# EvolBioInf/andi

Measured on AMD Instinct MI355X. Metric: genome-pairs/sec (ordered pairs, n^2-n) over the N x N anchor-distance loop, higher is better.
Workload: dtype u8

## Files before the change

andi_amd/csrc/api.hip:

```cpp
#include <hip/hip_runtime.h>

#include <algorithm>
#include <atomic>
#include <chrono>
#include <cstdarg>
#include <cstdio>
#include <cstdlib>
#include <cstring>
#include <mutex>
#include <string>
#include <thread>
#include <sys/mman.h>
#include <vector>

#include "api_internal.h"
#include "andi_dev.h"
#include "andi_hip.h"
#include "bootstrap.h"
#include "dev_arena.h"
#include "esa_build.h"
#include "knobs.h"
#include "sa_device.h"
#include "scan.h"

// ... 196 lines not shown
	if (hipMalloc(&p, bytes) != hipSuccess) {
		(void)hipGetLastError();
		return nullptr;
	}
	return p;
}
void scratch_put(int device, void *p, size_t bytes) {
	if (!p) return;
	{
		std::lock_guard<std::mutex> lk(state().mu);
		auto &v = state().scratch;
		bool have = false;
		for (const IdleScratch &x : v) have = have || x.device == device;
		if (!have) {
			v.push_back({device, p, bytes});
			return;
		}
	}
	(void)hipFree(p);
}
static bool any() {
	std::lock_guard<std::mutex> lk(state().mu);
	return !state().streams.empty() || !state().pinned.empty() || !state().scratch.empty() || !state().slabs.empty();
}
static size_t trim() {
	std::vector<IdleStream> st;
	std::vector<IdlePinned> pb;
	std::vector<IdleScratch> sc;
	{
		std::lock_guard<std::mutex> lk(state().mu);
		st.swap(state().streams), pb.swap(state().pinned), sc.swap(state().scratch);
		if (state().words_out == 0) {
			for (char *slab : state().slabs) pb.push_back({slab, SLAB_BYTES});
			state().slabs.clear(), state().free_words.clear();
		}
	}
	for (const IdleStream &x : st)
		if (hipSetDevice(x.device) == hipSuccess) (void)hipStreamDestroy(x.s);
	for (const IdlePinned &b : pb) (void)hipHostFree(b.p);
	size_t freed = 0;
	for (const IdleScratch &x : sc)
		if (hipSetDevice(x.device) == hipSuccess && hipFree(x.p) == hipSuccess) freed += x.bytes;
	return freed;
}
}

int andi_hip_abi_version(void) {
	return ANDI_HIP_ABI_VERSION;
}

size_t andi_hip_trim(void) {
	if (!andi_arena::any_chunks() && !host_pool::any()) return 0;
	int ndev = 0, cur = 0;
	if (hipGetDeviceCount(&ndev) != hipSuccess) {
		(void)hipGetLastError();
		return 0;
	}
	(void)hipGetDevice(&cur);
	size_t freed = 0;
	for (int d = 0; d < ndev && d < 64; ++d) {
		if (!andi_arena::has_chunks(d)) continue;
		if (hipSetDevice(d) != hipSuccess) continue;
		freed += andi_arena::trim(d);
	}
	freed += host_pool::trim();
	(void)hipSetDevice(cur);
	return freed;
}

void andi_hip_default_opts(andi_hip_opts *o) {
	if (!o) return;
	memset(o, 0, sizeof *o);
	o->p_value = 0.025;
	o->model = ANDI_M_JC;
	o->device = 0;
	o->host_threads = 0;
	o->low_memory = 0;
	o->segment = 0;
	o->sa_on_host = 0;
	o->num_gpus = 1;
	o->devices = NULL;
}

int andi_hip_device_count(void) {
	int count = 0;
	return hipGetDeviceCount(&count) == hipSuccess && count > 0 ? count : 0;
}

int ctx_create(andi_hip_ctx **out, int device, char *errbuf, size_t errlen, bool high_priority) {
	if (!out) return 1;
	*out = nullptr;
	int count = 0;
	hipError_t e = hipGetDeviceCount(&count);
	if (e != hipSuccess || count <= 0) {
		set_err(errbuf, errlen, "no HIP device available (%s); the anchor-distance engine has no CPU path",
				e != hipSuccess ? hipGetErrorString(e) : "device count 0");
		return 1;
	}
	if (device < 0 || device >= count) {
		set_err(errbuf, errlen, "HIP device %d out of range (have %d)", device, count);
		return 1;
	}
	e = hipSetDevice(device);
	if (e != hipSuccess) {
		set_err(errbuf, errlen, "hipSetDevice(%d): %s", device, hipGetErrorString(e));
		return 1;
	}
	auto *ctx = new andi_hip_ctx;
	ctx->device = device;
	andi_arena::retain(device);
	int prio = 0;
	if (high_priority) {
		int least = 0, greatest = 0;
		if (hipDeviceGetStreamPriorityRange(&least, &greatest) == hipSuccess) prio = greatest;
	}
	ctx->stream_prio = prio;
	e = host_pool::stream_get(&ctx->stream, device, prio);
	if (e == hipSuccess) e = hipEventCreateWithFlags(&ctx->side_fork, hipEventDisableTiming);
	if (e == hipSuccess) e = hipEventCreateWithFlags(&ctx->side_join, hipEventDisableTiming);
	if (e == hipSuccess) e = hipEventCreateWithFlags(&ctx->desc_done, hipEventDisableTiming);
	if (e == hipSuccess) e = hipEventCreateWithFlags(&ctx->built, hipEventDisableTiming);
	if (e == hipSuccess) e = hipMalloc((void **)&ctx->d_fixups, sizeof(unsigned long long));
	if (e == hipSuccess) e = hipMemset(ctx->d_fixups, 0, sizeof(unsigned long long));
	if (e == hipSuccess && !(ctx->h_quad_waves = (uint32_t *)host_pool::word_get())) e = hipErrorOutOfMemory;
	if (e == hipSuccess) e = hipEventCreateWithFlags(&ctx->coop_fork, hipEventDisableTiming);
	if (e == hipSuccess) e = hipEventCreateWithFlags(&ctx->coop_join, hipEventDisableTiming);
	if (e == hipSuccess) e = hipEventCreateWithFlags(&ctx->l2_fork, hipEventDisableTiming);
	if (e == hipSuccess) e = hipEventCreateWithFlags(&ctx->l2_join, hipEventDisableTiming);
	if (e == hipSuccess && !(ctx->h_any_left = (uint32_t *)host_pool::word_get())) e = hipErrorOutOfMemory;
	if (e == hipSuccess) e = hipMalloc((void **)&ctx->d_route, 4 * sizeof(unsigned long long));
	if (e == hipSuccess) e = hipMemset(ctx->d_route, 0, 4 * sizeof(unsigned long long));
	if (e != hipSuccess) {
		set_err(errbuf, errlen, "context setup: %s", hipGetErrorString(e));
		andi_hip_ctx_destroy(ctx);
		return 1;
	}
	*out = ctx;
	return 0;
}

int andi_hip_ctx_create(andi_hip_ctx **out, int device, char *errbuf, size_t errlen) {
	return ctx_create(out, device, errbuf, errlen, false);
}

void andi_hip_ctx_expect_queries(andi_hip_ctx *ctx, size_t queries) {
	if (ctx) ctx->queries_hint = queries;
}

void andi_hip_ctx_destroy(andi_hip_ctx *ctx) {
	if (!ctx) return;
	(void)hipSetDevice(ctx->device);
	if (ctx->stream) (void)hipStreamSynchronize(ctx->stream);
	resolve_events(ctx);
	if (ctx->scratch) (void)andi_arena::dev_free(ctx->scratch);
	if (ctx->desc_dev) (void)andi_arena::dev_free(ctx->desc_dev);
	if (ctx->desc_host) host_pool::pinned_put(ctx->desc_host, ctx->desc_bytes);
	if (ctx->d_fixups) (void)andi_arena::dev_free(ctx->d_fixups);
	if (ctx->ib_dev) (void)andi_arena::dev_free(ctx->ib_dev);
	if (ctx->ib_host) host_pool::pinned_put(ctx->ib_host, ctx->ib_cap * sizeof(AndiIndexBatchItem));
	if (ctx->ib_done) (void)hipEventDestroy(ctx->ib_done);
	if (ctx->built) (void)hipEventDestroy(ctx->built);
	if (ctx->sa_ws) (void)andi_arena::dev_free(ctx->sa_ws);
	host_pool::word_put(ctx->sa_pinned);
	host_pool::word_put(ctx->h_quad_waves);
	if (ctx->d_route) (void)andi_arena::dev_free(ctx->d_route);
	if (ctx->scratch2) (void)andi_arena::dev_free(ctx->scratch2);
	if (ctx->pool_scratch) {
		(void)hipDeviceSynchronize();
		host_pool::scratch_put(ctx->device, ctx->pool_scratch, ctx->pool_bytes + 4096);
	}
	host_pool::word_put(ctx->h_any_left);
	if (ctx->coop_stream) {
		(void)hipStreamSynchronize(ctx->coop_stream);
		host_pool::stream_put(ctx->coop_stream, ctx->device, 0);
	}
	if (ctx->coop_fork) (void)hipEventDestroy(ctx->coop_fork);
	if (ctx->coop_join) (void)hipEventDestroy(ctx->coop_join);
	if (ctx->l2_fork) (void)hipEventDestroy(ctx->l2_fork);
	if (ctx->l2_join) (void)hipEventDestroy(ctx->l2_join);
	if (ctx->desc_done) (void)hipEventDestroy(ctx->desc_done);
	if (ctx->side_stream) {
		(void)hipStreamSynchronize(ctx->side_stream);
		host_pool::stream_put(ctx->side_stream, ctx->device, ctx->stream_prio);
	}
	if (ctx->side_fork) (void)hipEventDestroy(ctx->side_fork);
	if (ctx->side_join) (void)hipEventDestroy(ctx->side_join);
	if (ctx->stream) {
		(void)hipStreamSynchronize(ctx->stream);
		host_pool::stream_put(ctx->stream, ctx->device, ctx->stream_prio);
	}
	andi_arena::release(ctx->device);
	delete ctx;
}

const char *andi_hip_last_error(const andi_hip_ctx *ctx) {
	return ctx ? ctx->err.c_str() : "no context";
}

int andi_hip_sync(andi_hip_ctx *ctx) {
	if (!ctx) return 1;
	HIP_TRY(ctx, hipStreamSynchronize(ctx->stream));
	return 0;
}

int andi_hip_dev_alloc(andi_hip_ctx *ctx, size_t bytes, void **dptr) {
	if (!ctx || !dptr) return 1;
	HIP_TRY(ctx, hipSetDevice(ctx->device));
	HIP_TRY(ctx, hipMalloc(dptr, bytes ? bytes : 1));
	return 0;
}

void andi_hip_dev_free(andi_hip_ctx *ctx, void *dptr) {
	if (!ctx || !dptr) return;
	(void)hipSetDevice(ctx->device);
	(void)andi_arena::dev_free(dptr);
}

int andi_hip_copy_to_host(andi_hip_ctx *ctx, void *dst, const void *src, size_t bytes) {
	if (!ctx) return 1;
	HIP_TRY(ctx, hipMemcpyAsync(dst, src, bytes, hipMemcpyDeviceToHost, ctx->stream));
	HIP_TRY(ctx, hipStreamSynchronize(ctx->stream));
	return 0;
}

int esa_reserve(andi_hip_ctx *ctx, size_t cap, andi_hip_esa **out) {
	auto *e = new andi_hip_esa;
	e->cap = cap;
	hipError_t err = hipSuccess;
	auto chk = [&](hipError_t x) {
		if (err == hipSuccess) err = x;
	};
	e->deepK_cap = pick_deep_k(cap, ctx->queries_hint);
	const size_t deep_entries = (size_t)1 << (2 * e->deepK_cap);
	chk(dmalloc(&e->S, cap + 1 + ANDI_PAD));
	chk(dmalloc(&e->SA, cap + 8));
	chk(dmalloc(&e->deep, deep_entries + 2));
	const size_t nib_part = (cap / 2 + 1 + ANDI_NIB_BACK + 255) & ~(size_t)255;
	chk(dmalloc(&e->Nraw, 2 * (ANDI_NIB_FRONT + nib_part)));
	if (err == hipSuccess) {
		e->N0 = e->Nraw + ANDI_NIB_FRONT, e->N1 = e->Nraw + ANDI_NIB_FRONT + nib_part + ANDI_NIB_FRONT;
		chk(hipMemsetAsync(e->Nraw, 0x77, 2 * (ANDI_NIB_FRONT + nib_part), ctx->stream));
	}
	{
		const size_t blocks = (cap + 1 + 4096) / 32 + 4;
		chk(dmalloc(&e->Praw, 3 * blocks));
		if (err == hipSuccess) {
			e->P = e->Praw + 3;
			chk(hipMemsetAsync(e->Praw, 0xff, 3 * blocks * sizeof(uint32_t), ctx->stream));
		}
	}
	if (!(e->h_flags = (int32_t *)host_pool::word_get())) chk(hipErrorOutOfMemory);
	if (err == hipSuccess) chk(hipHostGetDevicePointer((void **)&e->flags, e->h_flags, 0));
	e->bytes = (cap + 1 + ANDI_PAD) + 4 * cap + 8 * deep_entries + 80 +
			   2 * (ANDI_NIB_FRONT + nib_part);
	if (err != hipSuccess) {
		andi_hip_esa_free(ctx, e);
		return fail(ctx, "allocating a subject", err);
	}
	*out = e;
	return 0;
}

int esa_upload(andi_hip_ctx *ctx, andi_hip_esa *e, const char *RS, const int32_t *SA, size_t n,
					  size_t threshold, hipEvent_t done) {
	if (n > e->cap) {
		ctx->err = "subject does not fit its slot";
		return 1;
	}
	e->n = (int32_t)n;
	e->thr = (int32_t)threshold;
	e->deepK = std::min(pick_deep_k(n, ctx->queries_hint), e->deepK_cap);
	e->ref_built = e->index_built = false;
	e->rec_valid = false;
	hipError_t err = done ? hipSuccess : hipStreamSynchronize(ctx->stream);
	memset(e->h_flags, 0, 4 * sizeof(int32_t));
	if (err == hipSuccess) err = hipMemsetAsync(e->S + n, 0, 1 + ANDI_PAD, ctx->stream);
	if (err == hipSuccess) err = hipMemcpyAsync(e->S, RS, n, hipMemcpyHostToDevice, ctx->stream);
	if (err == hipSuccess && SA)
		err = hipMemcpyAsync(e->SA, SA, n * sizeof(int32_t), hipMemcpyHostToDevice, ctx->stream);
	if (err == hipSuccess) err = done ? hipEventRecord(done, ctx->stream) : hipStreamSynchronize(ctx->stream);
	if (err != hipSuccess) return fail(ctx, "uploading a subject", err);
	return 0;
}

int esa_from_query(andi_hip_ctx *ctx, andi_hip_esa *e, const andi_hip_queries *Q, size_t i, size_t threshold) {
	const size_t len = Q->len[i], n = 2 * len + 1;
	if (n > e->cap) {
		ctx->err = "subject does not fit its slot";
		return 1;
	}
	e->n = (int32_t)n;
	e->thr = (int32_t)threshold;
	e->deepK = std::min(pick_deep_k(n, ctx->queries_hint), e->deepK_cap);
	e->ref_built = e->index_built = false;
	e->rec_valid = false;
	memset(e->h_flags, 0, 4 * sizeof(int32_t));
	hipError_t err = hipMemsetAsync(e->S + (n & ~(size_t)3), 0, (n & 3) + 1 + ANDI_PAD, ctx->stream);
	if (err == hipSuccess) err = andi_launch_rs_from_query(e->S, Q->pool + Q->off[i], (uint32_t)len, ctx->stream);
	if (err != hipSuccess) return fail(ctx, "writing a subject from its resident sequence", err);
	return 0;
}

int queries_gc_counts(andi_hip_ctx *ctx, const andi_hip_queries *Q, std::vector<unsigned long long> &out) {
	HIP_TRY(ctx, hipSetDevice(ctx->device));
	unsigned long long *d = nullptr;
	HIP_TRY(ctx, dmalloc(&d, Q->nq));
// ... 92 lines not shown
	const size_t tab_entries = (size_t)1 << (2 * ANDI_CACHE_K);
	const size_t mins = andi_min_tree_entries((int32_t)n);
	hipError_t err = hipSuccess;
	auto chk = [&](hipError_t x) {
		if (err == hipSuccess) err = x;
	};
	chk(dmalloc(&e->LCP, n + 1));
	chk(dmalloc(&e->CLD, n + 1));
	chk(dmalloc(&e->FVC, n + ANDI_PAD));
	chk(dmalloc(&e->tab, tab_entries));
	chk(dmalloc(&e->min_scratch, mins));
	if (err != hipSuccess) return fail(ctx, "allocating the reference arrays", err);
	e->bytes += 8 * (n + 1) + n + ANDI_PAD + 16 * tab_entries + 4 * mins;
	return 0;
}

int andi_hip_esa_build(andi_hip_ctx *ctx, andi_hip_esa *e) {
	if (!ctx || !e) return 1;
	HIP_TRY(ctx, hipSetDevice(ctx->device));
	if (ensure_reference_buffers(ctx, e)) return 1;
	Timed t(ctx, 0);
	hipError_t err = andi_launch_esa_build(build_args(e), ctx->stream);
	t.stop();
	if (err == hipSuccess) err = hipEventRecord(ctx->built, ctx->stream);
	if (err != hipSuccess) return fail(ctx, "andi_hip_esa_build", err);
	e->ref_built = true, ctx->builds_pending = true;
	return 0;
}

int andi_hip_esa_build_index(andi_hip_ctx *ctx, andi_hip_esa *e) {
	if (!ctx || !e) return 1;
	HIP_TRY(ctx, hipSetDevice(ctx->device));
	Timed t(ctx, 0);
	const int ext = andi_index_single_ext(ctx->queries_hint, e->rec_valid);
	hipError_t err = andi_launch_index_build(build_args(e), ext, ctx->stream);
	t.stop();
	if (err == hipSuccess) err = hipEventRecord(ctx->built, ctx->stream);
	if (err != hipSuccess) return fail(ctx, "andi_hip_esa_build_index", err);
	e->index_built = true, e->deep_ext = (ext == 2 && !e->rec_valid) ? 0 : ext, ctx->builds_pending = true;
	return 0;
}

int andi_hip_esa_build_index_batch(andi_hip_ctx *ctx, andi_hip_esa *const *esas, size_t count) {
	if (!ctx || !esas || count == 0 || count > 65535) {
		if (ctx) ctx->err = "andi_hip_esa_build_index_batch: bad arguments";
		return 1;
	}
	HIP_TRY(ctx, hipSetDevice(ctx->device));
	if (ctx->ib_cap < count) {
		HIP_TRY(ctx, hipStreamSynchronize(ctx->stream));
		if (ctx->ib_dev) (void)andi_arena::dev_free(ctx->ib_dev);
		if (ctx->ib_host) host_pool::pinned_put(ctx->ib_host, ctx->ib_cap * sizeof(AndiIndexBatchItem));
		ctx->ib_dev = ctx->ib_host = nullptr, ctx->ib_cap = 0;
		const size_t cap = std::max<size_t>(count, 64);
		HIP_TRY(ctx, andi_arena::dev_malloc(&ctx->ib_dev, cap * sizeof(AndiIndexBatchItem)));
		HIP_TRY(ctx, host_pool::pinned_get(&ctx->ib_host, cap * sizeof(AndiIndexBatchItem)));
		if (!ctx->ib_done) HIP_TRY(ctx, hipEventCreateWithFlags(&ctx->ib_done, hipEventDisableTiming));
		ctx->ib_cap = cap;
	} else {
		HIP_TRY(ctx, hipEventSynchronize(ctx->ib_done));
	}
	auto *items = (AndiIndexBatchItem *)ctx->ib_host;
	int32_t max_n = 0, max_n_shallow = 0;
	for (size_t k = 0; k < count; ++k) {
		andi_hip_esa *e = esas[k];
		if (!e) {
			ctx->err = "andi_hip_esa_build_index_batch: null subject";
			return 1;
		}
		items[k].S = e->S, items[k].SA = e->SA, items[k].deep = e->deep, items[k].N0 = e->N0, items[k].N1 = e->N1, items[k].P = e->P;
		items[k].flags = e->flags, items[k].n = e->n, items[k].deepK = e->deepK;
		items[k].rec = e->rec_valid ? e->rec : nullptr;
		items[k].rec2 = e->rec_valid ? e->rec2 : nullptr;
		items[k].single_ext = andi_index_single_ext(ctx->queries_hint, e->rec_valid);
		max_n = std::max(max_n, e->n);
		if (e->deepK < ANDI_CLOSED_RUN_K) max_n_shallow = std::max(max_n_shallow, e->n);
	}
	Timed t(ctx, 0);
	hipError_t err = hipMemcpyAsync(ctx->ib_dev, ctx->ib_host, count * sizeof(AndiIndexBatchItem), hipMemcpyHostToDevice, ctx->stream);
	if (err == hipSuccess) err = hipEventRecord(ctx->ib_done, ctx->stream);
	if (err == hipSuccess) err = andi_launch_index_build_batch((const AndiIndexBatchItem *)ctx->ib_dev, (uint32_t)count, max_n, max_n_shallow, ctx->stream);
	t.stop();
	if (err == hipSuccess) err = hipEventRecord(ctx->built, ctx->stream);
	if (err != hipSuccess) return fail(ctx, "andi_hip_esa_build_index_batch", err);
	for (size_t k = 0; k < count; ++k) {
		const int ext = items[k].single_ext;
		esas[k]->index_built = true, esas[k]->deep_ext = (ext == 2 && !esas[k]->rec_valid) ? 0 : ext;
	}
	ctx->builds_pending = true;
	return 0;
}

int andi_hip_esa_flags(andi_hip_ctx *ctx, const andi_hip_esa *e, int32_t *out4) {
	if (!ctx || !e || !out4) return 1;
	HIP_TRY(ctx, hipStreamSynchronize(ctx->stream));
	memcpy(out4, e->h_flags, 4 * sizeof(int32_t));
	return 0;
}

int andi_hip_esa_download(andi_hip_ctx *ctx, const andi_hip_esa *e, int32_t *LCP, int32_t *CLD,
						  uint8_t *FVC, andi_hip_interval *cache) {
	if (!ctx || !e) return 1;
	if (!e->ref_built) {
		ctx->err = "andi_hip_esa_download: reference arrays not built (call andi_hip_esa_build)";
		return 1;
	}
	const size_t n = (size_t)e->n;
	HIP_TRY(ctx, hipStreamSynchronize(ctx->stream));
	if (LCP) HIP_TRY(ctx, hipMemcpy(LCP, e->LCP, (n + 1) * 4, hipMemcpyDeviceToHost));
	if (CLD) HIP_TRY(ctx, hipMemcpy(CLD, e->CLD, (n + 1) * 4, hipMemcpyDeviceToHost));
	if (FVC) HIP_TRY(ctx, hipMemcpy(FVC, e->FVC, n, hipMemcpyDeviceToHost));
	if (cache)
		HIP_TRY(ctx, hipMemcpy(cache, e->tab, ((size_t)16 << (2 * ANDI_CACHE_K)), hipMemcpyDeviceToHost));
	return 0;
}

int andi_hip_esa_download_index(andi_hip_ctx *ctx, const andi_hip_esa *e, uint32_t *table, int *K) {
	if (!ctx || !e) return 1;
	if (!e->index_built) {
		ctx->err = "andi_hip_esa_download_index: scan index not built (call andi_hip_esa_build_index)";
		return 1;
	}
	if (K) *K = e->deepK;
	HIP_TRY(ctx, hipStreamSynchronize(ctx->stream));
	if (table) HIP_TRY(ctx, hipMemcpy(table, e->deep, (size_t)8 << (2 * e->deepK), hipMemcpyDeviceToHost));
	return 0;
}

#ifdef ANDI_TEST_HOOKS
extern "C" int andi_hip_test_download_text(andi_hip_ctx *ctx, const andi_hip_esa *e, uint8_t *N0, uint8_t *N1, size_t nib_bytes, uint32_t *P,
										   size_t p_words) {
	if (!ctx || !e) return 1;
	if (nib_bytes > e->cap / 2 + 1 + ANDI_NIB_BACK || p_words > 3 * ((e->cap + 1 + 4096) / 32 + 4)) {
		ctx->err = "andi_hip_test_download_text: more than the buffers hold";
		return 1;
	}
	HIP_TRY(ctx, hipStreamSynchronize(ctx->stream));
	if (N0) HIP_TRY(ctx, hipMemcpy(N0, e->N0, nib_bytes, hipMemcpyDeviceToHost));
	if (N1) HIP_TRY(ctx, hipMemcpy(N1, e->N1, nib_bytes, hipMemcpyDeviceToHost));
	if (P) HIP_TRY(ctx, hipMemcpy(P, e->Praw, p_words * sizeof(uint32_t), hipMemcpyDeviceToHost));
	return 0;
}
extern "C" int andi_hip_test_coop_items(andi_hip_ctx *ctx, uint32_t *items, size_t items_cap, uint8_t *pair_class, uint8_t *pair_cost, size_t pairs_cap,
										uint32_t *info) {
	if (!ctx) return 1;
	const auto &l = ctx->last_items;
	HIP_TRY(ctx, hipSetDevice(ctx->device));
	HIP_TRY(ctx, hipStreamSynchronize(ctx->stream));
	if (info) info[0] = l.n_items, info[1] = l.pairs, info[2] = l.total_segs, info[3] = l.items ? 1u : 0u;
	const size_t ni = std::min<size_t>(items_cap, l.n_items), np = std::min<size_t>(pairs_cap, l.pairs);
	if (items && l.items && ni) HIP_TRY(ctx, hipMemcpy(items, l.items, ni * sizeof(uint32_t), hipMemcpyDeviceToHost));
	if (pair_class && l.pair_class && np) HIP_TRY(ctx, hipMemcpy(pair_class, l.pair_class, np, hipMemcpyDeviceToHost));
	if (pair_cost && l.pair_cost && np) HIP_TRY(ctx, hipMemcpy(pair_cost, l.pair_cost, np, hipMemcpyDeviceToHost));
	return 0;
}
extern "C" int andi_hip_test_stitch_slots(andi_hip_ctx *ctx, ChainState *cold_exit, ChainState *true_exit, ChainState *used_entry, uint32_t *cold_counts,
										  uint32_t *owned, ColdMark *marks, size_t slots, uint32_t *restitch_count, uint32_t *info) {
	if (!ctx) return 1;
	const auto &l = ctx->last_slots;
	const bool have = l.cold_exit != nullptr;
	if (info) info[0] = l.nsub, info[1] = l.total_segs, info[2] = l.seg, info[3] = have ? 1u : 0u;
	const bool wants = cold_exit || true_exit || used_entry || cold_counts || owned || marks || restitch_count;
	if (!wants) return 0;
	if (!have || slots > (size_t)l.nsub * l.total_segs) {
		ctx->err = have ? "andi_hip_test_stitch_slots: more slots than the call had" : "andi_hip_test_stitch_slots: no scan call with one segment length on record";
		return 1;
	}
	HIP_TRY(ctx, hipSetDevice(ctx->device));
	HIP_TRY(ctx, hipStreamSynchronize(ctx->stream));
	if (cold_exit && slots) HIP_TRY(ctx, hipMemcpy(cold_exit, l.cold_exit, slots * sizeof(ChainState), hipMemcpyDeviceToHost));
	if (true_exit && slots) HIP_TRY(ctx, hipMemcpy(true_exit, l.true_exit, slots * sizeof(ChainState), hipMemcpyDeviceToHost));
	if (used_entry && slots) HIP_TRY(ctx, hipMemcpy(used_entry, l.used_entry, slots * sizeof(ChainState), hipMemcpyDeviceToHost));
	if (cold_counts && slots) HIP_TRY(ctx, hipMemcpy(cold_counts, l.cold_counts, slots * 16 * sizeof(uint32_t), hipMemcpyDeviceToHost));
	if (owned && slots) HIP_TRY(ctx, hipMemcpy(owned, l.owned, slots * 16 * sizeof(uint32_t), hipMemcpyDeviceToHost));
	if (marks && slots) HIP_TRY(ctx, hipMemcpy(marks, l.marks, slots * ANDI_COLD_MARKS * sizeof(ColdMark), hipMemcpyDeviceToHost));
	if (restitch_count) HIP_TRY(ctx, hipMemcpy(restitch_count, l.restitch_count, 16 * sizeof(uint32_t), hipMemcpyDeviceToHost));
	return 0;
}
extern "C" int andi_hip_test_pack_text(andi_hip_ctx *ctx, andi_hip_esa *e, int forms) {
	if (!ctx || !e) return 1;
	HIP_TRY(ctx, hipSetDevice(ctx->device));
	HIP_TRY(ctx, andi_launch_pack_text(e->S, (size_t)e->n + 1 + 64, e->N0, (forms & 1) ? e->N1 : nullptr, (forms & 2) ? e->P : nullptr, e->flags + 1,
									   ctx->stream));
	return 0;
}
extern "C" int andi_hip_test_query_codes(andi_hip_ctx *ctx, const andi_hip_queries *q, size_t qidx, uint32_t *out, size_t words) {
	if (!ctx || !q || !out || qidx >= q->nq || !q->codes || words > 2 * (((size_t)q->len[qidx] + 1 + 255) / 256 * 8)) {
		if (ctx) ctx->err = "andi_hip_test_query_codes: bad arguments, or more than the query's blocks hold";
		return 1;
	}
	HIP_TRY(ctx, hipSetDevice(ctx->device));
	HIP_TRY(ctx, hipStreamSynchronize(ctx->stream));
	if (words) HIP_TRY(ctx, hipMemcpy(out, q->codes + 2 * (q->off[qidx] / 32), words * sizeof(uint32_t), hipMemcpyDeviceToHost));
	return 0;
}
#endif

int andi_hip_esa_single_form(const andi_hip_esa *e) { return e && e->index_built ? e->deep_ext : 0; }

void andi_hip_esa_free(andi_hip_ctx *ctx, andi_hip_esa *e) {
	if (!e) return;
	if (ctx) (void)hipSetDevice(ctx->device);
	(void)hipDeviceSynchronize();
	void *bufs[] = {e->S, e->SA, e->LCP, e->CLD, e->FVC, e->tab, e->deep, e->Nraw, e->Praw, e->rec, e->rec2, e->min_scratch};
	for (void *b : bufs) (void)andi_arena::dev_free(b, false);
	host_pool::word_put(e->h_flags);
	delete e;
}

size_t andi_hip_esa_bytes(const andi_hip_esa *e) {
	return e ? e->bytes : 0;
}

static hipError_t queries_count_separators(andi_hip_ctx *ctx, andi_hip_queries *q) {
	hipError_t err = dmalloc(&q->d_sep, q->nq);
	if (err != hipSuccess) return err;
	uint32_t longest = 0;
	for (uint32_t l : q->len) longest = std::max(longest, l);
	err = hipMemsetAsync(q->d_sep, 0, q->nq * sizeof(uint32_t), ctx->stream);
	if (err == hipSuccess) err = andi_launch_sep_counts(q->pool, q->d_off, q->d_len, (uint32_t)q->nq, longest, q->d_sep, ctx->stream);
	return err;
}

int andi_hip_queries_stage(andi_hip_ctx *ctx, const andi_hip_seq *seqs, size_t n,
						   andi_hip_queries **out) {
	if (!ctx || !seqs || !out || n == 0 || n >= (size_t)UINT32_MAX) {
		if (ctx) ctx->err = "andi_hip_queries_stage: bad arguments";
		return 1;
	}
	HIP_TRY(ctx, hipSetDevice(ctx->device));
	auto *q = new andi_hip_queries;
	q->nq = n;
	q->off.resize(n);
	q->len.resize(n);
	uint64_t cursor = 0;
	for (size_t i = 0; i < n; ++i) {
		if (!seqs[i].seq || seqs[i].len == 0 || seqs[i].len > (size_t)(INT32_MAX - 1) / 2) {
			ctx->err = "andi_hip_queries_stage: empty or oversized sequence";
			delete q;
			return 1;
		}
		q->off[i] = cursor;
		q->len[i] = (uint32_t)seqs[i].len;
		q->total_nt += seqs[i].len;
		cursor += (seqs[i].len + 1 + 255) & ~(uint64_t)255;
	}
	const size_t pool_bytes = cursor + ANDI_PAD;
	hipError_t err = hipSuccess;
	auto chk = [&](hipError_t x) {
		if (err == hipSuccess) err = x;
	};
	chk(dmalloc(&q->pool, pool_bytes));
	chk(dmalloc(&q->nib, pool_bytes / 2 + 64));
	chk(dmalloc(&q->planes, 3 * (pool_bytes / 32) + 16));
	chk(dmalloc(&q->codes, 2 * (pool_bytes / 32) + 16));
	if (!(q->h_foreign = (int32_t *)host_pool::word_get())) chk(hipErrorOutOfMemory);
	int32_t *d_foreign = nullptr;
	chk(dmalloc(&d_foreign, 1));
	chk(dmalloc(&q->d_off, n));
	chk(dmalloc(&q->d_len, n));
	if (err == hipSuccess) err = hipMemsetAsync(q->pool, 0, pool_bytes, ctx->stream);
	uint64_t threaded_from = (uint64_t)1 << 31;
	if (const char *um = andi_knob(KNOB_UPLOAD_MIN_MB))
		if (atoi(um) >= 0) threaded_from = (uint64_t)atoi(um) << 20;
	if (err == hipSuccess && q->total_nt >= threaded_from) {
		err = hipStreamSynchronize(ctx->stream);
		constexpr size_t CHUNK = (size_t)8 << 20;
		const int nt = 4;
		std::atomic<size_t> next_seq{0};
		std::atomic<int> bad{0};
		auto work = [&]() {
			(void)hipSetDevice(ctx->device);
			hipStream_t st = nullptr;
			void *pin = nullptr;
			hipEvent_t ev[2] = {nullptr, nullptr};
			bool ok = host_pool::stream_get(&st, ctx->device, 0) == hipSuccess && host_pool::pinned_get(&pin, 2 * CHUNK) == hipSuccess &&
					  hipEventCreateWithFlags(&ev[0], hipEventDisableTiming) == hipSuccess && hipEventCreateWithFlags(&ev[1], hipEventDisableTiming) == hipSuccess;
			size_t k = 0;
			while (ok && !bad.load()) {
				const size_t i = next_seq.fetch_add(1);
				if (i >= n) break;
				for (size_t o = 0; o < seqs[i].len && ok; o += CHUNK, ++k) {
					const size_t len = std::min(CHUNK, seqs[i].len - o);
					char *buf = (char *)pin + (k & 1) * CHUNK;
					if (k >= 2) ok = hipEventSynchronize(ev[k & 1]) == hipSuccess;
					memcpy(buf, seqs[i].seq + o, len);
					ok = ok && hipMemcpyAsync(q->pool + q->off[i] + o, buf, len, hipMemcpyHostToDevice, st) == hipSuccess && hipEventRecord(ev[k & 1], st) == hipSuccess;
				}
			}
			if (st) ok = hipStreamSynchronize(st) == hipSuccess && ok;
			if (!ok) bad.store(1);
			for (hipEvent_t e : ev)
				if (e) (void)hipEventDestroy(e);
			if (pin) host_pool::pinned_put(pin, 2 * CHUNK);
			if (st) host_pool::stream_put(st, ctx->device, 0);
		};
		std::vector<std::thread> ts;
		for (int t = 1; t < nt; ++t) ts.emplace_back(work);
		work();
		for (auto &t : ts) t.join();
		if (bad.load() && err == hipSuccess) err = hipErrorUnknown;
	} else {
		for (size_t i = 0; i < n && err == hipSuccess; ++i)
			err = hipMemcpyAsync(q->pool + q->off[i], seqs[i].seq, seqs[i].len, hipMemcpyHostToDevice,
								 ctx->stream);
	}
// ... 316 lines not shown
```

andi_amd/csrc/api_internal.h:

```cpp
#pragma once
#include <hip/hip_runtime.h>

#include <atomic>
#include <cstdarg>
#include <cstdio>
#include <cstdlib>
#include <cstdint>
#include <string>
#include <vector>

#include "andi_dev.h"
#include "andi_hip.h"
#include "dev_arena.h"
#include "esa_build.h"
#include "knobs.h"
#include "scan.h"

#define ANDI_SLOT_BYTES (3 * sizeof(ChainState) + 2 * 16 * sizeof(uint32_t) + ANDI_COLD_MARKS * sizeof(ColdMark) + 4 + 8 + 8)

struct EventPair {
	hipEvent_t a, b;
	int kind;
};

struct andi_hip_ctx {
	int device = 0;
	size_t queries_hint = 0;
	hipStream_t stream = nullptr;
	hipStream_t side_stream = nullptr;
	hipEvent_t side_fork = nullptr, side_join = nullptr;
	std::string err;
	void *scratch = nullptr;
	size_t scratch_bytes = 0;
	void *desc_host = nullptr;
	void *desc_dev = nullptr;
	size_t desc_bytes = 0;
	hipEvent_t desc_done = nullptr;
	unsigned long long *d_fixups = nullptr;
	void *ib_host = nullptr, *ib_dev = nullptr;
	size_t ib_cap = 0;
	hipEvent_t ib_done = nullptr;
	hipEvent_t built = nullptr;
	bool builds_pending = false;
	void *sa_ws = nullptr;
	size_t sa_ws_bytes = 0;
	int32_t *sa_pinned = nullptr;
	int stream_prio = 0;
	uint32_t *h_quad_waves = nullptr;
	hipStream_t coop_stream = nullptr;
	hipEvent_t coop_fork = nullptr, coop_join = nullptr, l2_fork = nullptr, l2_join = nullptr;
	uint32_t *h_any_left = nullptr;
	void *pool_scratch = nullptr;
	size_t pool_bytes = 0;
	uint32_t pool_waves = 0;
	bool pool_failed = false;
	void *scratch2 = nullptr;
	size_t scratch2_bytes = 0;
	uint32_t round_waves = 0;
	struct {
		const uint32_t *items = nullptr;
		const uint8_t *pair_class = nullptr, *pair_cost = nullptr;
		uint32_t n_items = 0, pairs = 0, total_segs = 0;
	} last_items;
	unsigned long long *d_route = nullptr;
	std::vector<EventPair> pending;
	andi_hip_timings acc{};
#ifdef ANDI_TEST_HOOKS
	struct {
		const ChainState *cold_exit = nullptr, *true_exit = nullptr, *used_entry = nullptr;
		const uint32_t *cold_counts = nullptr, *owned = nullptr, *restitch_count = nullptr;
		const ColdMark *marks = nullptr;
		uint32_t nsub = 0, total_segs = 0, seg = 0;
	} last_slots;
#endif
};

struct andi_hip_esa {
	uint8_t *S = nullptr;
	int32_t *SA = nullptr, *LCP = nullptr, *CLD = nullptr;
	uint8_t *FVC = nullptr;
	int4 *tab = nullptr;
	int32_t *min_scratch = nullptr;
	uint2 *deep = nullptr;
	uint8_t *Nraw = nullptr;
	uint8_t *N0 = nullptr, *N1 = nullptr;
	uint32_t *Praw = nullptr, *P = nullptr;
	uint32_t *rec = nullptr;
	bool rec_valid = false;
	uint16_t *rec2 = nullptr;
	int32_t *flags = nullptr;
	int32_t *h_flags = nullptr;
	int32_t deepK = 0;
	int32_t deepK_cap = 0;
	int32_t n = 0;
	int32_t thr = 0;
	size_t cap = 0;
	size_t ref_cap = 0;
	bool ref_built = false;
	bool index_built = false;
	int deep_ext = 0;
	size_t bytes = 0;
};

struct andi_hip_queries {
	bool owns_pool = true;
	uint8_t *pool = nullptr;
	uint8_t *nib = nullptr;
	uint32_t *planes = nullptr;
	uint32_t *codes = nullptr;
	int32_t *h_foreign = nullptr;
	uint64_t *d_off = nullptr;
	uint32_t *d_len = nullptr;
	uint32_t *d_sep = nullptr;
	std::vector<uint64_t> off;
	std::vector<uint32_t> len;
	size_t nq = 0;
	uint64_t total_nt = 0;
	uint32_t seg = 0;
	uint32_t *d_qseg_start = nullptr;
	uint32_t *d_seg2query = nullptr;
	uint32_t total_segs = 0;
	uint32_t c_seg = 0;
	uint32_t *c_qseg_start = nullptr;
	uint32_t *c_seg2query = nullptr;
	uint32_t c_total_segs = 0;
};

namespace {

void set_err(char *buf, size_t len, const char *fmt, ...) {
	if (!buf || !len) return;
	va_list ap;
	va_start(ap, fmt);
	vsnprintf(buf, len, fmt, ap);
	va_end(ap);
}

int fail(andi_hip_ctx *ctx, const char *what, hipError_t e) {
	if (ctx) {
		ctx->err = std::string(what) + ": " + hipGetErrorString(e);
	}
	return 1;
}

#define HIP_TRY(ctx, call)                                                                         \
	do {                                                                                           \
		hipError_t e__ = (call);                                                                   \
		if (e__ != hipSuccess) return fail((ctx), #call, e__);                                     \
	} while (0)

template <typename T>
hipError_t dmalloc(T **p, size_t count) {
	return andi_arena::dev_malloc((void **)p, count * sizeof(T));
}

struct DevScope {
	hipStream_t stream;
	hipError_t err = hipSuccess;
	std::vector<void *> held;
	explicit DevScope(hipStream_t st) : stream(st) {}
	template <typename T>
	void alloc(T **p, size_t count) {
		if (err == hipSuccess && (err = dmalloc(p, count)) == hipSuccess) held.push_back(*p);
	}
	void release() {
		(void)hipStreamSynchronize(stream);
		for (void *p : held) (void)andi_arena::dev_free(p, false);
		held.clear();
		err = hipSuccess;
	}
	~DevScope() { release(); }
	DevScope(const DevScope &) = delete;
	DevScope &operator=(const DevScope &) = delete;
};

size_t nj_group_size(AndiKnob knob, size_t max, size_t budget, size_t each) {
	size_t G = budget / each;
	if (const char *v = andi_knob(knob))
		if (atoll(v) >= 1) G = (size_t)atoll(v);
	return G < 1 ? 1 : G > max ? max : G;
}

void resolve_events(andi_hip_ctx *ctx) {
	for (auto &ev : ctx->pending) {
		float ms = 0.f;
		if (hipEventSynchronize(ev.b) == hipSuccess && hipEventElapsedTime(&ms, ev.a, ev.b) == hipSuccess) {
			if (ev.kind == 0) {
				ctx->acc.build_ms += ms;
				ctx->acc.build_launches++;
			} else if (ev.kind == 1) {
				ctx->acc.scan_ms += ms;
				ctx->acc.scan_launches++;
			} else {
				ctx->acc.stitch_ms += ms;
				ctx->acc.stitch_launches++;
			}
		}
		(void)hipEventDestroy(ev.a);
		(void)hipEventDestroy(ev.b);
	}
	ctx->pending.clear();
}

struct Timed {
	andi_hip_ctx *ctx;
	EventPair ev;
	bool ok;
	Timed(andi_hip_ctx *c, int kind) : ctx(c), ok(false) {
		ev.kind = kind;
		if (hipEventCreate(&ev.a) != hipSuccess) return;
		if (hipEventCreate(&ev.b) != hipSuccess) {
			(void)hipEventDestroy(ev.a);
			return;
		}
		ok = hipEventRecord(ev.a, c->stream) == hipSuccess;
	}
	void stop() {
		if (!ok) return;
		(void)hipEventRecord(ev.b, ctx->stream);
		ctx->pending.push_back(ev);
		ok = false;
		if (ctx->pending.size() > 256) resolve_events(ctx);
	}
	~Timed() {
		if (!ok) return;
		(void)hipEventDestroy(ev.a);
		(void)hipEventDestroy(ev.b);
	}
	Timed(const Timed &) = delete;
	Timed &operator=(const Timed &) = delete;
};

}

struct PackedQueries {
	std::vector<uint64_t> off;
	std::vector<uint32_t> len;
	uint64_t total_nt = 0;
	size_t pool_bytes = 0;
	uint8_t *nib = nullptr;
	int foreign = 0;
	std::string err;
	std::atomic<int> users{0};
	void release() {
		free(nib);
		nib = nullptr;
	}
	~PackedQueries() { release(); }
};

#pragma GCC visibility push(hidden)

EsaDev esa_view(const andi_hip_esa *e, int mode);
int pick_deep_k(size_t n, size_t queries);
int ctx_create(andi_hip_ctx **out, int device, char *errbuf, size_t errlen, bool high_priority);
int esa_reserve(andi_hip_ctx *ctx, size_t cap, andi_hip_esa **out);
int esa_upload(andi_hip_ctx *ctx, andi_hip_esa *e, const char *RS, const int32_t *SA, size_t n,
			   size_t threshold, hipEvent_t done = nullptr);
int esa_from_query(andi_hip_ctx *ctx, andi_hip_esa *e, const andi_hip_queries *Q, size_t i, size_t threshold);
int queries_gc_counts(andi_hip_ctx *ctx, const andi_hip_queries *Q, std::vector<unsigned long long> &out);
int esa_sort_suffixes(andi_hip_ctx *ctx, andi_hip_esa *e);

int pack_queries_host(const andi_hip_seq *seqs, size_t n, int threads, PackedQueries &P);
int queries_stage_packed(andi_hip_ctx *ctx, const PackedQueries &P, andi_hip_queries **out);

namespace host_pool {
hipError_t stream_get(hipStream_t *out, int device, int prio);
void stream_put(hipStream_t s, int device, int prio);
hipError_t pinned_get(void **out, size_t bytes);
void pinned_put(void *p, size_t bytes);
void *word_get();
void word_put(void *p);
void *scratch_get(int device, size_t bytes);
void scratch_put(int device, void *p, size_t bytes);
}

#pragma GCC visibility pop
```

andi_amd/csrc/scan.h:

```cpp
#pragma once
#include <hip/hip_runtime.h>
#include <stdint.h>

#include "andi_dev.h"
#include "andi_hip.h"

struct __attribute__((aligned(16))) ChainState {
	uint32_t p;
	uint32_t lastS;
	uint32_t lastQ;
	uint32_t lastLen;
	uint32_t lwra;
	uint32_t pad[3];
};
#define ANDI_ANCHORS_UNKNOWN 0xffffffffu

#define ANDI_COLD_MARKS 1
struct __attribute__((aligned(16))) ColdMark {
	ChainState st;
	uint32_t counts[16];
	uint32_t first[4];
};

struct ScanArgs {
	const EsaDev *subjects;
	const int64_t *self;
	uint32_t nsub;
	const uint8_t *qpool;
	const uint8_t *qnib;
	const uint32_t *qplanes;
	const uint32_t *qcodes;
	const uint64_t *qoff;
	const uint32_t *qlen;
	const uint32_t *qsep;
	uint32_t nq;
	const uint32_t *qseg_start;
	const uint32_t *seg2query;
	uint32_t total_segs;
	uint32_t seg;
	ChainState *cold_exit;
	uint32_t *exit_p;
	uint32_t *cold_counts;
	ColdMark *marks;
	ChainState *true_exit;
	ChainState *used_entry;
	uint32_t *restitch_count;
	uint32_t restitch_round;
	uint32_t stitch_lanes;
	unsigned long long *defer_list;
	uint32_t *defer_count;
	uint32_t defer_base;
	unsigned long long *first_pub;
	uint8_t *stretch_bad;
	uint32_t *owned;
	andi_hip_model *M;
	unsigned long long *fixups;
	int exact_equal;
	int any_reference;
	int adaptive;
	uint32_t seg0;
	uint32_t seg_factor;
	uint32_t max_class;
	uint8_t *pair_class;
	uint32_t *pair_waves;
	uint32_t *pair_wave0;
	uint32_t *pair_bsum;
	uint32_t max_waves;
	uint8_t *pair_cost;
	uint32_t *coop_items;
	uint32_t n_items;
	uint32_t *item_hist;
	uint32_t items_order;
	const uint32_t *layout_count;
	float *sub_cost;
	uint32_t *sub_order;
	uint32_t quad_min_match;
	uint32_t quad_listed;
	uint32_t *h_quad_waves;
	hipStream_t side_stream;
	hipEvent_t side_fork, side_join;
	int route;
	uint32_t route_seg;
	uint32_t reduce_threads;
	uint32_t route_all_few;
	uint32_t route_giveup;
	unsigned long long *route_nt;
	int coop;
	void *pool_scratch;
	uint32_t *pool_ticket;
	uint32_t pool_waves;
	size_t pool_bytes;
	uint32_t pool_maxchunks, pool_hc;
	uint32_t pool_match;
	int pool_use;
	uint32_t pool_first;
	uint32_t knock;
};

hipError_t andi_launch_unpack_symbols(const uint8_t *N0, size_t bytes, uint8_t *dst, hipStream_t st);
hipError_t andi_launch_pack_symbols(const uint8_t *src, size_t bytes, uint8_t *N0, uint8_t *N1,
									int32_t *foreign, hipStream_t st);
hipError_t andi_launch_pack_planes(const uint8_t *N0, size_t symbols, uint32_t *planes, uint32_t *codes, hipStream_t st);
hipError_t andi_launch_pair_layout(const ScanArgs &a, hipStream_t st);
hipError_t andi_launch_pair_leftover(const ScanArgs &a2, hipStream_t st);
hipError_t andi_launch_route_count(const ScanArgs &a, hipStream_t st);
hipError_t andi_launch_coop_items(const ScanArgs &b, hipStream_t st);
hipError_t andi_launch_lane_cold(const ScanArgs &a, hipStream_t st);
int andi_coop_enabled(void);
hipError_t andi_launch_coop_cold(const ScanArgs &a, hipStream_t st);
int andi_coop_wants_pool(const ScanArgs &a);
int andi_coop_will_pool(const ScanArgs &a);
size_t andi_pool_scratch_bytes(int device, uint32_t *waves);
hipError_t andi_launch_lane_stitch(const ScanArgs &a, hipStream_t st);
hipError_t andi_launch_lane_quad_small(const ScanArgs &a, uint32_t count, hipStream_t st);
#ifndef ANDI_RESTITCH_ROUNDS
#define ANDI_RESTITCH_ROUNDS 3
#endif
#ifndef ANDI_STITCH_FIRST
#define ANDI_STITCH_FIRST 12
#endif
#ifndef ANDI_STITCH_FEW
#define ANDI_STITCH_FEW 12
#endif
#ifndef ANDI_STITCH_MANY
#define ANDI_STITCH_MANY 4096
#endif
static_assert(ANDI_RESTITCH_ROUNDS < 8, "restitch_count[]: rounds 0 .. ROUNDS at the front, defer_count at 8, ANDI_ROUTE_ANY_LEFT at 11, ANDI_STRAGGLERS at 12, ANDI_QUAD_WAVES at 13, ANDI_SPARSE_WAVES at 14, ANDI_ALL_WAVES at 15");
#define ANDI_ROUTE_COOP 0x40u
#define ANDI_ROUTE_LEFT 0x20u
#define ANDI_ROUTE_SOFT 0x10u
#define ANDI_ROUTE_GUESS 0x04u
#define ANDI_ROUTE_L2 0x08u
#define ANDI_ROUTE_POOLCAND 0x08u
#define ANDI_STRUCT_WAVES 4
#define ANDI_POOL_SEGS 6
#define ANDI_COOP_SEGS 7
#define ANDI_COST_CLASSES 64u
#define ANDI_ITEMS_ROUNDS 8u
#define ANDI_ITEMS_GRID 0
#define ANDI_ITEMS_HEAVY 1
#define ANDI_ITEMS_LIGHT 2
#define ANDI_LAYOUT_LANES 1
#define ANDI_LAYOUT_LANES2 2
#define ANDI_LAYOUT_COOP 3
#define ANDI_ROUTE_ANY_LEFT 11
#define ANDI_ROUTE_MIN_QLEN 8192u
#define ANDI_HARD_WAVES 9
#define ANDI_ISLAND_WAVES 11
#define ANDI_LANE_WAVES 10
#define ANDI_ALL_WAVES 15
#define ANDI_QUAD_WAVES 13
#define ANDI_SPARSE_WAVES 14
#define ANDI_SPARSE_MATCH 19u
#define ANDI_STRAGGLERS 12
#ifndef ANDI_STITCH_BUDGET
#define ANDI_STITCH_BUDGET 48
#endif
#ifndef ANDI_LISTED_LANES
#define ANDI_LISTED_LANES 2
#endif
#ifndef ANDI_LISTED_BLOCKS
#define ANDI_LISTED_BLOCKS 1024
#endif
#ifndef ANDI_STITCH_TOGETHER
#define ANDI_STITCH_TOGETHER 40
#endif
hipError_t andi_launch_scan_cold(const ScanArgs &a, hipStream_t st);
hipError_t andi_launch_scan_stitch(const ScanArgs &a, hipStream_t st);
hipError_t andi_launch_scan_reduce(const ScanArgs &a, hipStream_t st);
hipError_t andi_launch_match_positions(const EsaDev &E, const uint8_t *q, uint32_t qlen,
									   uint32_t first, uint32_t count, int cached,
									   andi_hip_interval *out, hipStream_t st);
```

andi_amd/csrc/scan.hip:

```cpp
#include "scan_dev.h"
#include "knobs.h"

#include <cstdlib>

template <int G>
struct Window {
	uint32_t q0, s0;
	uint32_t qc;
	uint32_t mask;
	uint4 sb;
};

__device__ __forceinline__ uint32_t diff_bits4(uint32_t x) {
	x |= x >> 4;
	x |= x >> 2;
	x |= x >> 1;
	x &= 0x01010101u;
	return ((x * 0x01020408u) >> 24) & 0xfu;
}

__device__ __forceinline__ void codes16(uint4 v, uint32_t &code, uint32_t &valid) {
	auto pack4 = [](uint32_t x) {
		x &= 0x06060606u;
		x ^= x >> 1;
// ... 322 lines not shown
	for (uint32_t t = lane; t < 16; t += G) a.owned[slot * 16 + t] = histT[t * hist_stride<G>()];
}

__global__ __launch_bounds__(BLOCK) void k_scan_reduce(ScanArgs a) {
	__shared__ uint32_t s_hist[3][16];
	const uint32_t sub = blockIdx.y, qidx = blockIdx.x;
	const uint32_t lane = __lane_id();
	andi_hip_model *out = a.M + (size_t)sub * a.nq + qidx;

	if (a.self[sub] == (int64_t)qidx) {
		if (threadIdx.x < 17) {
			uint32_t *o = (uint32_t *)out;
			o[threadIdx.x] = (threadIdx.x == 0 || threadIdx.x == 16) ? 9u : 0u;
		}
		return;
	}

	if (a.route) {
		const uint32_t cls = a.pair_class[sub * a.nq + qidx];
		const bool mine = a.route == ANDI_LAYOUT_COOP ? (cls & (ANDI_ROUTE_COOP | ANDI_ROUTE_LEFT)) == ANDI_ROUTE_COOP
						: a.route == ANDI_LAYOUT_LANES2 ? (cls & ANDI_ROUTE_L2) != 0
						: !(cls & (ANDI_ROUTE_COOP | ANDI_ROUTE_L2));
		if (!mine) return;
	}
	uint32_t *total = s_hist[0];
	uint32_t *histT = s_hist[1], *histC = s_hist[2];
	if (threadIdx.x < 16) total[threadIdx.x] = 0;
	__syncthreads();

	uint32_t nseg, seg;
	size_t row;
	if (a.adaptive) {
		const PairGeom g = pair_geometry(a, sub, qidx);
		nseg = g.nseg, seg = g.seg, row = g.slot0;
	} else {
		const uint32_t base = a.qseg_start[qidx];
		nseg = a.qseg_start[qidx + 1] - base, seg = a.seg;
		row = (size_t)sub * a.total_segs + base;
	}
	PairCtx c = make_ctx(a, sub, qidx);

	bool ok = true;
	for (uint32_t k = 1 + threadIdx.x; k < nseg; k += blockDim.x)
		ok = ok && same_state(a.true_exit[row + k - 1], a.used_entry[row + k]);
	const bool all_ok = __syncthreads_and(ok);
	{
		uint32_t sum[16];
#pragma unroll
		for (int t = 0; t < 16; ++t) sum[t] = 0;
		for (uint32_t k = threadIdx.x; k < nseg; k += blockDim.x) {
			const uint4 *o = (const uint4 *)(a.owned + (row + k) * 16);
#pragma unroll
			for (int t = 0; t < 4; ++t) {
				const uint4 v = o[t];
				sum[4 * t] += v.x, sum[4 * t + 1] += v.y, sum[4 * t + 2] += v.z, sum[4 * t + 3] += v.w;
			}
		}
#pragma unroll
		for (int t = 0; t < 16; ++t) {
			uint32_t v = sum[t];
			for (int d = 32; d; d >>= 1) v += (uint32_t)__shfl_xor((int)v, d);
			if (lane == 0) atomicAdd(&total[t], v);
		}
	}
	__syncthreads();
	if (threadIdx.x >= 64) return;
	ChainState fin = a.true_exit[row + nseg - 1];
	if (!all_ok) {
		uint32_t next = 1;
		for (uint32_t base = 1; base < nseg; base += 64) {
			const uint32_t kk = base + lane;
			uint64_t bad = __ballot(kk < nseg && !same_state(a.true_exit[row + kk - 1], a.used_entry[row + kk]));
			for (; bad; bad &= bad - 1) {
				uint32_t k = base + (uint32_t)__builtin_ctzll(bad);
				if (k < next) continue;
				ChainState st = a.true_exit[row + k - 1];
				while (k < nseg && !same_state(st, a.used_entry[row + k])) {
					if (lane == 0) atomicAdd(a.fixups, 1ull);
					const uint32_t start = k * seg, e = start + seg, end = e < c.qlen ? e : c.qlen;
					if (c.E.mode == ANDI_MODE_REFERENCE) {
						if (c.exact)
							stitch_segment<64, ANDI_MODE_REFERENCE, true>(c, st, start, end, a.cold_exit[row + k],
																		  a.cold_counts + (row + k) * 16, histT, histC);
						else
							stitch_segment<64, ANDI_MODE_REFERENCE, false>(c, st, start, end, a.cold_exit[row + k],
																		   a.cold_counts + (row + k) * 16, histT, histC);
					} else {
						if (c.exact)
							stitch_segment<64, ANDI_MODE_PROBE, true>(c, st, start, end, a.cold_exit[row + k],
																	  a.cold_counts + (row + k) * 16, histT, histC);
						else
							stitch_segment<64, ANDI_MODE_PROBE, false>(c, st, start, end, a.cold_exit[row + k],
																	   a.cold_counts + (row + k) * 16, histT, histC);
					}
					if (lane < 16) total[lane] += histT[lane] - a.owned[(row + k) * 16 + lane];
					++k;
				}
				if (k == nseg) fin = st;
				next = k + 1;
			}
		}
	}

	Tally last;
	last.hist = (lds_u32 *)total, last.hs = 1, last.quarter = 0, last.rest = 0;
	last.same[0] = last.same[1] = last.same[2] = last.same[3] = 0;
	if (fin.lastLen >= c.qlen || fin.lwra || fin.lastLen >= 2 * c.thr) {
		const bool whole = fin.lastLen >= c.qlen;
		const uint32_t from = whole ? 0u : fin.lastQ, len = whole ? c.qlen : fin.lastLen;
		if (c.exact)
			count_anchor<64, true>(c, last, from, len);
		else
			count_anchor<64, false>(c, last, from, len);
	}
	tally_finish<64>(last);
	if (lane < 16) out->counts[lane] = total[lane];
	if (lane == 0) out->seq_len = c.qlen;
}

__global__ __launch_bounds__(256) void k_match_positions(EsaDev Ed, const uint8_t *qd, uint32_t qlen,
														 uint32_t first, uint32_t count, int cached,
														 andi_hip_interval *out) {
	uint32_t k = blockIdx.x * blockDim.x + threadIdx.x;
	if (k >= count) return;
	const EsaG E = esa_global(Ed);
	g_u8p q = (g_u8p)qd;
	uint32_t pos = first + k;
	Ival r = cached ? esa_match_cached<1>(E, q + pos, qlen - pos)
					: esa_match<1>(E, q + pos, qlen - pos);
	andi_hip_interval o;
	o.l = r.l, o.i = r.i, o.j = r.j;
	o.m = r.i >= 0 ? E.SA[r.i] : -1;
	out[k] = o;
}

template <bool EXACT>
static hipError_t launch_reference(const ScanArgs &a, hipStream_t st, bool stitch) {
	const uint32_t per_block = BLOCK / SCAN_G;
	dim3 grid((a.total_segs + per_block - 1) / per_block, a.nsub);
	if (stitch)
		k_scan_stitch<SCAN_G, ANDI_MODE_REFERENCE, EXACT><<<grid, BLOCK, 0, st>>>(a);
	else
		k_scan_cold<SCAN_G, ANDI_MODE_REFERENCE, EXACT><<<grid, BLOCK, 0, st>>>(a);
	CHECK_LAUNCH();
	return hipSuccess;
}

hipError_t andi_launch_scan_cold(const ScanArgs &a, hipStream_t st) {
	hipError_t e = a.coop ? andi_launch_coop_cold(a, st) : andi_launch_lane_cold(a, st);
	if (e != hipSuccess || !a.any_reference) return e;
	return a.exact_equal ? launch_reference<true>(a, st, false) : launch_reference<false>(a, st, false);
}

hipError_t andi_launch_scan_stitch(const ScanArgs &a, hipStream_t st) {
	hipError_t e = andi_launch_lane_stitch(a, st);
	if (e != hipSuccess || !a.any_reference) return e;
	return a.exact_equal ? launch_reference<true>(a, st, true) : launch_reference<false>(a, st, true);
}

hipError_t andi_launch_scan_reduce(const ScanArgs &a, hipStream_t st) {
	dim3 grid(a.nq, a.nsub);
	k_scan_reduce<<<grid, a.reduce_threads == 64 ? 64 : BLOCK, 0, st>>>(a);
	CHECK_LAUNCH();
	return hipSuccess;
}

hipError_t andi_launch_match_positions(const EsaDev &E, const uint8_t *q, uint32_t qlen,
									   uint32_t first, uint32_t count, int cached,
									   andi_hip_interval *out, hipStream_t st) {
	if (count == 0) return hipSuccess;
	k_match_positions<<<(count + 255) / 256, 256, 0, st>>>(E, q, qlen, first, count, cached, out);
	CHECK_LAUNCH();
	return hipSuccess;
}
```

andi_amd/csrc/scan_call.hip:

```cpp
#include <hip/hip_runtime.h>

#include <algorithm>
#include <cstdio>
#include <cstdlib>
#include <vector>

#include "api_internal.h"

#define ANDI_MIN_SEGMENT 4096u
#define ANDI_MAX_SEGMENT 65536u
#define ANDI_TARGET_CHAINS (1u << 22)
#define ANDI_MIN_CHAINS (1u << 19)
#define ANDI_ADAPTIVE_MAX_PAIRS (1u << 22)
#define ANDI_ROUTE_MIN_NT (1u << 18)
#define ANDI_ROUTE_TINY_NT (1u << 25)
#define ANDI_ROUTE_SMALL_NT (1ull << 30)

static int ensure_segmentation(andi_hip_ctx *ctx, andi_hip_queries *q, uint32_t seg, bool coop = false) {
	uint32_t &have = coop ? q->c_seg : q->seg, &total_out = coop ? q->c_total_segs : q->total_segs;
	uint32_t *&d_start = coop ? q->c_qseg_start : q->d_qseg_start, *&d_s2q = coop ? q->c_seg2query : q->d_seg2query;
	if (have == seg && d_start) return 0;
	HIP_TRY(ctx, hipStreamSynchronize(ctx->stream));
	(void)andi_arena::dev_free(d_start);
	(void)andi_arena::dev_free(d_s2q);
// ... 33 lines not shown
	int coop = 0;
	bool want_adaptive = false;
	bool adaptive = false;
	uint32_t segment = 0;
	uint32_t coop_seg = 0;
	uint32_t seg0 = 0;
	uint32_t max_class = 0;
	uint64_t max_waves = 0;
	uint32_t seg_factor = 0, quad_min_match = 0, knock = 0, pool_match = 0, route_all_few = 0, route_giveup = 0;
	uint32_t items_order = ANDI_ITEMS_HEAVY;
	uint32_t longest_q = 0, reduce_threads = 0, coop_reduce_threads = 0;
	int exact_equal = 0;
	bool force_reference = false, force_adaptive = false;
};

uint32_t reduce_threads(uint32_t longest_q, uint32_t seg) { return (longest_q + seg - 1) / seg <= 64 ? 64u : 0u; }

ScanPlan plan_call(andi_hip_esa *const *subjects, size_t nsub, const andi_hip_queries *q, int model, uint32_t segment) {
	ScanPlan P;
	P.force_reference = andi_knob(KNOB_FORCE_REFERENCE) != nullptr;
	P.force_adaptive = andi_knob(KNOB_FORCE_ADAPTIVE) != nullptr;
	const bool uniform = andi_knob(KNOB_UNIFORM_SEGMENTS) != nullptr;
	const int coop_mode = andi_coop_enabled();
	int coop_ok = coop_mode != 0 && !P.force_reference;
	for (size_t s = 0; s < nsub && coop_ok; ++s)
		if (!subjects[s] || subjects[s]->thr < 2 || subjects[s]->thr > 30) coop_ok = 0;
	const uint64_t call_nt = q->total_nt * (uint64_t)nsub;
	const bool engine = coop_ok && coop_mode < 0 && segment == 0 && call_nt >= ANDI_ROUTE_MIN_NT && !uniform && !P.force_adaptive;
	const int tiny_log = knob_int(KNOB_ROUTE_TINY, 1, 62, 0);
	bool tiny = engine && call_nt < (tiny_log ? 1ull << tiny_log : ANDI_ROUTE_TINY_NT);
	uint32_t coop_seg = 524288;
	while (coop_seg > 32768 && call_nt / coop_seg < 24576) coop_seg /= 2;
	while (coop_seg > 2048 && call_nt / coop_seg < 12000u) coop_seg /= 2;
	P.coop_seg = coop_seg = (uint32_t)knob_int(KNOB_COOP_SEG, 64, INT32_MAX, (int)coop_seg);
	bool routed = engine && nsub * q->nq <= ANDI_ADAPTIVE_MAX_PAIRS;
	if (routed || tiny) {
		uint64_t cand_nt = 0;
		for (size_t i = 0; i < q->nq; ++i)
			if (q->len[i] >= std::min(coop_seg, ANDI_ROUTE_MIN_QLEN)) cand_nt += q->len[i];
		if (2 * cand_nt < q->total_nt) routed = tiny = false;
	}
	P.routed = routed && !tiny;
	P.coop = coop_ok && (coop_mode > 0 || tiny);
	P.want_adaptive = !P.coop && segment == 0 && nsub * q->nq <= ANDI_ADAPTIVE_MAX_PAIRS && !uniform;
	if (segment == 0 && P.coop) segment = coop_seg;
	if (segment == 0) {
		segment = ANDI_MIN_SEGMENT;
		while (segment < ANDI_MAX_SEGMENT && call_nt / segment > ANDI_TARGET_CHAINS) segment *= 2;
	}
	P.segment = segment;
	P.seg0 = (uint32_t)knob_int(KNOB_SEG0, 64, INT32_MAX, (int)(segment / 2));
	P.seg_factor = (uint32_t)knob_int(KNOB_SEG_FACTOR, 1, INT32_MAX, 16);
	P.quad_min_match = (uint32_t)knob_int(KNOB_QUAD_MATCH, INT32_MIN, INT32_MAX, 128);
	P.knock = (uint32_t)knob_int(KNOB_KNOCK, INT32_MIN, INT32_MAX, 0);
	P.pool_match = (uint32_t)knob_int(KNOB_POOL_MATCH, 0, INT32_MAX, 48);
	const int small_log = knob_int(KNOB_ROUTE_SMALL, 1, 62, 0);
	P.route_all_few = call_nt < (small_log ? 1ull << small_log : ANDI_ROUTE_SMALL_NT) ? 1u : 0u;
	P.route_giveup = (uint32_t)knob_int(KNOB_COOP_GIVEUP, 1, INT32_MAX, P.route_all_few ? 256 : 1024);
	if (const char *o = andi_knob(KNOB_COOP_ORDER)) P.items_order = o[0] == 'G' ? ANDI_ITEMS_GRID : o[0] == 'R' ? ANDI_ITEMS_LIGHT : ANDI_ITEMS_HEAVY;
	for (size_t i = 0; i < q->nq; ++i) P.longest_q = std::max(P.longest_q, (uint32_t)q->len[i]);
	P.coop_reduce_threads = reduce_threads(P.longest_q, coop_seg);
	P.exact_equal = (model == ANDI_M_LOGDET || model == ANDI_M_ANI) ? 1 : 0;
	return P;
}

void plan_layout(andi_hip_ctx *ctx, ScanPlan &P, const int64_t *h_self, size_t nsub, const andi_hip_queries *q,
				 int any_reference, uint64_t nt) {
	if (any_reference) P.routed = false;
	P.adaptive = P.want_adaptive && !any_reference;
	if (P.adaptive) {
		for (size_t s = 0; s < nsub; ++s)
			for (size_t i = 0; i < q->nq; ++i) {
				if (h_self[s] == (int64_t)i) continue;
				P.max_waves += ((q->len[i] + (uint64_t)P.seg0 - 1) / P.seg0 + 63) / 64;
			}
		uint64_t used = 0;
		for (size_t i = 0; i < q->nq; ++i) used += (q->len[i] + (uint64_t)P.seg0 - 1) / P.seg0;
		used *= nsub;
		size_t free_b = 0, total_b = 0;
		const size_t want_b = (size_t)64 * P.max_waves * ANDI_SLOT_BYTES * (P.routed ? 2 : 1);
		const bool fits = P.max_waves < (1u << 26) &&
						  (want_b <= ctx->scratch_bytes || hipMemGetInfo(&free_b, &total_b) != hipSuccess || want_b < free_b / 2 + ctx->scratch_bytes);
		if (!fits || (10 * used < 7 * 64 * P.max_waves && !P.force_adaptive)) P.adaptive = false, P.max_waves = 0;
	}
	P.max_class = 0;
	while (P.max_class < 3 && nt / ((uint64_t)P.seg0 << (P.max_class + 1)) >= ANDI_MIN_CHAINS) P.max_class++;
	P.reduce_threads = reduce_threads(P.longest_q, P.adaptive ? P.seg0 : P.segment);
}

size_t carve_layout(ScanArgs &x, char *base, size_t off, size_t n, size_t pairs, bool cls, size_t nsub, size_t items = 0) {
	uintptr_t p = (uintptr_t)base + off;
	auto take = [&p](size_t bytes, size_t align = 1) {
		p = (p + align - 1) & ~(uintptr_t)(align - 1);
		const uintptr_t at = p;
		p += bytes;
		return (void *)at;
	};
	x.cold_exit = (ChainState *)take(n * sizeof(ChainState));
	x.true_exit = (ChainState *)take(n * sizeof(ChainState));
	x.used_entry = (ChainState *)take(n * sizeof(ChainState));
	x.cold_counts = (uint32_t *)take(n * 16 * sizeof(uint32_t));
	x.owned = (uint32_t *)take(n * 16 * sizeof(uint32_t));
	x.marks = (ColdMark *)take(n * ANDI_COLD_MARKS * sizeof(ColdMark));
	x.exit_p = (uint32_t *)take(n * sizeof(uint32_t));
	x.restitch_count = (uint32_t *)take(64, 16);
	x.restitch_round = 0;
	x.defer_count = x.restitch_count + 8;
	x.defer_list = (unsigned long long *)take(n * sizeof(unsigned long long));
	x.first_pub = (unsigned long long *)take(n * sizeof(unsigned long long));
	x.stretch_bad = (uint8_t *)x.first_pub;
	if (pairs) {
		x.pair_waves = (uint32_t *)take(pairs * sizeof(uint32_t));
		x.pair_wave0 = (uint32_t *)take((pairs + 1) * sizeof(uint32_t));
		x.pair_bsum = (uint32_t *)take((pairs / 1024 + 2) * sizeof(uint32_t));
		if (cls) x.pair_class = (uint8_t *)take(pairs);
	}
	if (nsub) {
		x.sub_cost = (float *)take(nsub * sizeof(float), 16);
		x.sub_order = (uint32_t *)take(nsub * sizeof(uint32_t));
	}
	if (items) {
		x.pair_cost = (uint8_t *)take(pairs);
		x.item_hist = (uint32_t *)take(ANDI_COST_CLASSES * ((pairs + 1023) / 1024) * sizeof(uint32_t), 16);
		x.coop_items = (uint32_t *)take(items * sizeof(uint32_t));
	}
	return (size_t)(p - (uintptr_t)base);
}

int carve_scratch(andi_hip_ctx *ctx, const ScanPlan &P, ScanArgs &a, size_t slots, size_t slots2, size_t nsub, size_t pairs_all, size_t *b_off) {
	const size_t pairs = P.adaptive || P.routed ? pairs_all : 0, subs = P.routed ? nsub : 0;
	if (!ctx->round_waves) {
		int cus = 0;
		if (hipDeviceGetAttribute(&cus, hipDeviceAttributeMultiprocessorCount, ctx->device) != hipSuccess || cus <= 0) cus = 256;
		ctx->round_waves = (uint32_t)cus * 4u * 8u;
	}
	const bool listed = P.routed && !P.route_all_few && P.items_order != ANDI_ITEMS_GRID && slots2 <= (size_t)ANDI_ITEMS_ROUNDS * ctx->round_waves;
	const size_t items = listed ? slots2 : 0;
	ScanArgs m = a;
	*b_off = (carve_layout(m, nullptr, 0, slots, pairs, true, subs, items) + 15) & ~(size_t)15;
	const size_t need = (P.routed ? carve_layout(m, nullptr, *b_off, slots2, 0, false, 0) : *b_off) + 256;
	if (ctx->scratch_bytes < need) {
		HIP_TRY(ctx, hipStreamSynchronize(ctx->stream));
		if (ctx->scratch) (void)andi_arena::dev_free(ctx->scratch);
		ctx->scratch = nullptr;
		ctx->scratch_bytes = 0;
		HIP_TRY(ctx, andi_arena::dev_malloc(&ctx->scratch, need));
		ctx->scratch_bytes = need;
	}
	carve_layout(a, (char *)ctx->scratch, 0, slots, pairs, true, subs, items);
	return 0;
}

int upload_descriptors(andi_hip_ctx *ctx, andi_hip_esa *const *subjects, const int64_t *self, size_t nsub, const andi_hip_queries *q,
					   bool force_reference, int &any_reference, uint64_t &pairs, uint64_t &nt) {
	const size_t desc_need = nsub * (sizeof(EsaDev) + sizeof(int64_t));
	if (ctx->desc_bytes < desc_need) {
		HIP_TRY(ctx, hipStreamSynchronize(ctx->stream));
		if (ctx->desc_dev) (void)andi_arena::dev_free(ctx->desc_dev);
		if (ctx->desc_host) host_pool::pinned_put(ctx->desc_host, ctx->desc_bytes);
		ctx->desc_dev = ctx->desc_host = nullptr;
		ctx->desc_bytes = 0;
		const size_t desc_cap = std::max<size_t>(desc_need, 4096);
		HIP_TRY(ctx, andi_arena::dev_malloc(&ctx->desc_dev, desc_cap));
		HIP_TRY(ctx, host_pool::pinned_get(&ctx->desc_host, desc_cap));
		ctx->desc_bytes = desc_cap;
	} else {
		HIP_TRY(ctx, hipEventSynchronize(ctx->desc_done));
	}
	auto *h_esa = (EsaDev *)ctx->desc_host;
	auto *h_self = (int64_t *)(h_esa + nsub);
	pairs = 0, nt = 0, any_reference = 0;
	if (ctx->builds_pending) {
		HIP_TRY(ctx, hipEventSynchronize(ctx->built));
		ctx->builds_pending = false;
	}
	for (size_t s = 0; s < nsub; ++s) {
		andi_hip_esa *e = subjects[s];
		if (!e || (!e->index_built && !e->ref_built)) {
			ctx->err = "andi_hip_scan_rows: subject index not built";
			return 1;
		}
		int mode = ANDI_MODE_PROBE;
		if (!e->index_built || e->h_flags[0] != 0 || force_reference) {
			mode = ANDI_MODE_REFERENCE;
			if (!e->ref_built && andi_hip_esa_build(ctx, e)) return 1;
			ctx->acc.reference_subjects++;
			any_reference = 1;
		}
		if (e->index_built && e->h_flags[1]) {
			ctx->err = "andi_hip_scan_rows: a subject holds a byte outside {A,C,G,T,!,;,#}";
			return 1;
		}
		h_esa[s] = esa_view(e, mode);
		h_self[s] = self ? self[s] : -1;
		bool has_self = h_self[s] >= 0 && (size_t)h_self[s] < q->nq;
		pairs += q->nq - (has_self ? 1 : 0);
		nt += q->total_nt - (has_self ? q->len[(size_t)h_self[s]] : 0);
	}
	HIP_TRY(ctx, hipMemcpyAsync(ctx->desc_dev, ctx->desc_host, desc_need, hipMemcpyHostToDevice,
								ctx->stream));
	HIP_TRY(ctx, hipEventRecord(ctx->desc_done, ctx->stream));
	return 0;
}

ScanArgs scan_args(andi_hip_ctx *ctx, const ScanPlan &P, size_t nsub, const andi_hip_queries *q, andi_hip_model *M_dev, int any_reference) {
	ScanArgs a;
	a.subjects = (const EsaDev *)ctx->desc_dev;
	a.self = (const int64_t *)((const EsaDev *)ctx->desc_dev + nsub);
	a.nsub = (uint32_t)nsub;
	a.qpool = q->pool, a.qnib = q->nib, a.qplanes = q->planes, a.qcodes = q->codes, a.qoff = q->d_off, a.qlen = q->d_len, a.qsep = q->d_sep, a.nq = (uint32_t)q->nq;
	a.qseg_start = q->d_qseg_start, a.seg2query = q->d_seg2query;
	a.total_segs = q->total_segs, a.seg = P.segment;
	a.adaptive = P.adaptive ? 1 : 0;
	a.seg0 = P.seg0, a.max_waves = (uint32_t)P.max_waves, a.max_class = P.max_class;
	a.pair_waves = a.pair_wave0 = a.pair_bsum = nullptr, a.pair_class = nullptr;
	a.sub_cost = nullptr, a.sub_order = nullptr;
	a.pair_cost = nullptr, a.coop_items = nullptr, a.item_hist = nullptr, a.layout_count = nullptr;
	a.n_items = 0, a.items_order = ANDI_ITEMS_GRID;
	a.seg_factor = P.seg_factor;
	a.M = M_dev;
	a.fixups = ctx->d_fixups;
	a.any_reference = any_reference;
	a.quad_min_match = P.quad_min_match;
	a.quad_listed = 0;
	a.side_stream = ctx->side_stream, a.side_fork = ctx->side_fork, a.side_join = ctx->side_join;
	a.h_quad_waves = ctx->h_quad_waves;
	a.knock = P.knock;
	a.coop = P.coop && !a.adaptive;
	a.pool_scratch = nullptr, a.pool_ticket = nullptr, a.pool_waves = 0, a.pool_bytes = 0;
	a.pool_maxchunks = a.pool_hc = 0, a.pool_first = 0, a.pool_use = 0;
	a.pool_match = P.pool_match;
	a.route = P.routed ? ANDI_LAYOUT_LANES : 0, a.route_seg = P.coop_seg, a.route_nt = ctx->d_route;
	a.reduce_threads = P.reduce_threads;
	a.route_all_few = P.route_all_few;
	a.route_giveup = P.route_giveup;
	a.exact_equal = P.exact_equal;
	return a;
}

void give_pool_scratch(andi_hip_ctx *ctx, ScanArgs &x) {
	if (!andi_coop_wants_pool(x)) return;
	if (!ctx->pool_scratch && !ctx->pool_failed) {
		uint32_t waves = 0;
		const size_t bytes = andi_pool_scratch_bytes(ctx->device, &waves);
		if (bytes && (ctx->pool_scratch = host_pool::scratch_get(ctx->device, bytes)))
			ctx->pool_waves = waves, ctx->pool_bytes = bytes - 4096;
		else
			ctx->pool_failed = true;
	}
	if (!ctx->pool_scratch) return;
	x.pool_ticket = (uint32_t *)ctx->pool_scratch, x.pool_scratch = (char *)ctx->pool_scratch + 4096, x.pool_waves = ctx->pool_waves, x.pool_bytes = ctx->pool_bytes;
}

hipError_t launch_direct(andi_hip_ctx *ctx, ScanArgs &a, const char *&what) {
	hipError_t e = hipSuccess;
	if (a.adaptive) {
		Timed t(ctx, 2);
		e = andi_launch_pair_layout(a, ctx->stream);
		t.stop();
		if (e != hipSuccess) return what = "scan layout", e;
	}
	give_pool_scratch(ctx, a);
	{
		Timed t(ctx, 1);
		e = andi_launch_scan_cold(a, ctx->stream);
		t.stop();
		if (e != hipSuccess) return what = "scan pass A", e;
		if (a.coop) ctx->acc.coop_calls++;
		if (a.coop && andi_coop_will_pool(a)) ctx->acc.pool_calls++;
	}
	Timed t(ctx, 2);
	e = andi_launch_scan_stitch(a, ctx->stream);
	if (e == hipSuccess) e = andi_launch_scan_reduce(a, ctx->stream);
	t.stop();
	if (e != hipSuccess) what = "scan passes B/C";
#ifdef ANDI_TEST_HOOKS
	if (e == hipSuccess && !a.adaptive) {
		auto &l = ctx->last_slots;
		l.cold_exit = a.cold_exit, l.true_exit = a.true_exit, l.used_entry = a.used_entry, l.cold_counts = a.cold_counts, l.owned = a.owned;
		l.marks = a.marks, l.restitch_count = a.restitch_count, l.nsub = a.nsub, l.total_segs = a.total_segs, l.seg = a.seg;
	}
#endif
	return e;
}

hipError_t launch_routed(andi_hip_ctx *ctx, const ScanPlan &P, ScanArgs &a, size_t b_off, const andi_hip_queries *q,
						 size_t slots, size_t slots2, const char *&what) {
	const size_t nsub = a.nsub, pairs_all = nsub * q->nq;
	ScanArgs b = a;
	b.adaptive = 0, b.coop = 1, b.route = ANDI_LAYOUT_COOP;
	b.qseg_start = q->c_qseg_start, b.seg2query = q->c_seg2query, b.total_segs = q->c_total_segs, b.seg = P.coop_seg;
	b.reduce_threads = P.coop_reduce_threads;
	carve_layout(b, (char *)ctx->scratch, b_off, slots2, 0, false, 0);
	const bool look = !a.route_all_few;
	const bool listed = b.coop_items != nullptr;
	b.items_order = listed ? P.items_order : (uint32_t)ANDI_ITEMS_GRID;
	b.layout_count = a.restitch_count;
	hipError_t e;
	{
		Timed t(ctx, 2);
		e = hipMemsetAsync(b.restitch_count, 0, 16 * sizeof(uint32_t), ctx->stream);
		if (e == hipSuccess) e = andi_launch_pair_layout(a, ctx->stream);
		if (e == hipSuccess && listed) e = andi_launch_coop_items(b, ctx->stream);
		t.stop();
		if (e != hipSuccess) return what = "scan layout", e;
	}
	Timed t(ctx, 1);
	for (int k = 0; k < 16; ++k) ctx->h_any_left[1 + k] = 0;
	ctx->h_any_left[1 + ANDI_LANE_WAVES] = 1;
	e = hipSuccess;
	if (look) e = hipMemcpyAsync(ctx->h_any_left + 1, a.restitch_count, 16 * sizeof(uint32_t), hipMemcpyDeviceToHost, ctx->stream);
	if (look && e == hipSuccess) e = hipStreamSynchronize(ctx->stream);
	const bool lanes_first = look && e == hipSuccess && (uint64_t)ctx->h_any_left[1 + ANDI_LANE_WAVES] * 20 < ctx->h_any_left[1 + ANDI_ALL_WAVES];
	b.pool_use = look && e == hipSuccess && 2 * (uint64_t)ctx->h_any_left[1 + ANDI_POOL_SEGS] >= ctx->h_any_left[1 + ANDI_COOP_SEGS] && ctx->h_any_left[1 + ANDI_COOP_SEGS] != 0;
	give_pool_scratch(ctx, b);
	b.n_items = ctx->h_any_left[1 + ANDI_COOP_SEGS];
	if (andi_coop_will_pool(b)) b.coop_items = nullptr;
	ctx->last_items.items = b.coop_items, ctx->last_items.pair_class = b.pair_class, ctx->last_items.pair_cost = b.pair_cost;
	ctx->last_items.n_items = b.n_items, ctx->last_items.pairs = (uint32_t)pairs_all, ctx->last_items.total_segs = b.total_segs;
	if (e == hipSuccess) e = hipEventRecord(ctx->coop_fork, ctx->stream);
	if (e == hipSuccess) e = hipStreamWaitEvent(ctx->coop_stream, ctx->coop_fork, 0);
	if (e == hipSuccess && lanes_first) e = andi_launch_scan_cold(a, ctx->stream);
	if (e == hipSuccess) e = andi_launch_coop_cold(b, ctx->coop_stream);
	if (andi_coop_will_pool(b)) ctx->acc.pool_calls++;
	if (e == hipSuccess) e = hipEventRecord(ctx->coop_join, ctx->coop_stream);
	if (e == hipSuccess && !lanes_first) e = andi_launch_scan_cold(a, ctx->stream);
	if (e == hipSuccess) e = hipStreamWaitEvent(ctx->stream, ctx->coop_join, 0);
	if (e == hipSuccess) e = hipMemcpyAsync(ctx->h_any_left, b.restitch_count + ANDI_ROUTE_ANY_LEFT, sizeof(uint32_t), hipMemcpyDeviceToHost, ctx->stream);
	if (e == hipSuccess) e = hipStreamSynchronize(ctx->stream);
	if (e != hipSuccess) return what = "scan pass A", e;
	const bool any_left = ctx->h_any_left[0] != 0;
	const bool any_lanes = ctx->h_any_left[1 + ANDI_LANE_WAVES] != 0;
	ScanArgs a2 = a;
	if (any_left) {
		const size_t need2 = carve_layout(a2, nullptr, 0, slots, pairs_all, false, 0) + 256;
		if (ctx->scratch2_bytes < need2) {
			if (ctx->scratch2) (void)andi_arena::dev_free(ctx->scratch2);
			ctx->scratch2 = nullptr, ctx->scratch2_bytes = 0;
			e = andi_arena::dev_malloc(&ctx->scratch2, need2);
			if (e != hipSuccess) return what = "scratch of the second lane layout", e;
			ctx->scratch2_bytes = need2;
		}
		carve_layout(a2, (char *)ctx->scratch2, 0, slots, pairs_all, false, 0);
		a2.route = ANDI_LAYOUT_LANES2;
		a2.side_stream = nullptr;
	}
	t.stop();
	Timed t2(ctx, 2);
	e = hipEventRecord(ctx->l2_fork, ctx->stream);
	if (e == hipSuccess) e = hipStreamWaitEvent(ctx->coop_stream, ctx->l2_fork, 0);
	if (e == hipSuccess) e = andi_launch_scan_stitch(b, ctx->coop_stream);
	if (e == hipSuccess) e = andi_launch_scan_reduce(b, ctx->coop_stream);
	if (e == hipSuccess) e = hipEventRecord(ctx->coop_join, ctx->coop_stream);
	if (e == hipSuccess && any_left) {
		e = hipStreamWaitEvent(ctx->side_stream, ctx->l2_fork, 0);
		if (e == hipSuccess) e = andi_launch_pair_leftover(a2, ctx->side_stream);
		if (e == hipSuccess) e = andi_launch_scan_cold(a2, ctx->side_stream);
		if (e == hipSuccess) e = andi_launch_scan_stitch(a2, ctx->side_stream);
		if (e == hipSuccess) e = andi_launch_scan_reduce(a2, ctx->side_stream);
		if (e == hipSuccess) e = hipEventRecord(ctx->l2_join, ctx->side_stream);
	}
	if (e == hipSuccess && any_lanes) e = andi_launch_scan_stitch(a, ctx->stream);
	if (e == hipSuccess && any_lanes) e = andi_launch_scan_reduce(a, ctx->stream);
	if (e == hipSuccess) e = hipStreamWaitEvent(ctx->stream, ctx->coop_join, 0);
	if (e == hipSuccess && any_left) e = hipStreamWaitEvent(ctx->stream, ctx->l2_join, 0);
	if (e == hipSuccess) e = andi_launch_route_count(a, ctx->stream);
	t2.stop();
	if (e != hipSuccess) return what = "scan passes B/C", e;
	ctx->acc.coop_calls++;
	ctx->acc.routed_calls++;
	return hipSuccess;
}

}

int andi_hip_scan_rows(andi_hip_ctx *ctx, andi_hip_esa *const *subjects, const int64_t *self,
					   size_t nsub, const andi_hip_queries *q_const, int model, uint32_t segment,
					   andi_hip_model *M_dev) {
	if (!ctx || !subjects || !q_const || !M_dev || nsub == 0 || nsub > 65535) {
		if (ctx) ctx->err = "andi_hip_scan_rows: bad arguments";
		return 1;
	}
	if (model < ANDI_M_RAW || model > ANDI_M_ANI) {
		ctx->err = "andi_hip_scan_rows: unknown model";
		return 1;
	}
	auto *q = const_cast<andi_hip_queries *>(q_const);
	if (*q->h_foreign) {
		ctx->err = "andi_hip_scan_rows: a query holds a byte outside {A,C,G,T,!}";
		return 1;
	}
	HIP_TRY(ctx, hipSetDevice(ctx->device));
	if (!ctx->side_stream) HIP_TRY(ctx, host_pool::stream_get(&ctx->side_stream, ctx->device, ctx->stream_prio));
	if (!ctx->coop_stream) HIP_TRY(ctx, host_pool::stream_get(&ctx->coop_stream, ctx->device, 0));

	ctx->last_items = {};
#ifdef ANDI_TEST_HOOKS
	ctx->last_slots = {};
#endif
	ScanPlan P = plan_call(subjects, nsub, q, model, segment);
	if (ensure_segmentation(ctx, q, P.segment)) return 1;
	int any_reference = 0;
	uint64_t pairs = 0, nt = 0;
	if (upload_descriptors(ctx, subjects, self, nsub, q, P.force_reference, any_reference, pairs, nt)) return 1;
	const int64_t *h_self = (const int64_t *)((const EsaDev *)ctx->desc_host + nsub);
	plan_layout(ctx, P, h_self, nsub, q, any_reference, nt);
	if (P.routed && ensure_segmentation(ctx, q, P.coop_seg, true)) return 1;
	const size_t slots = P.adaptive ? (size_t)64 * P.max_waves : nsub * (size_t)q->total_segs;
	const size_t slots2 = P.routed ? nsub * (size_t)q->c_total_segs : 0;
	ScanArgs a = scan_args(ctx, P, nsub, q, M_dev, any_reference);
	size_t b_off = 0;
	if (carve_scratch(ctx, P, a, slots, slots2, nsub, nsub * q->nq, &b_off)) return 1;

	const char *what = nullptr;
	const hipError_t e = P.routed ? launch_routed(ctx, P, a, b_off, q, slots, slots2, what) : launch_direct(ctx, a, what);
	if (e != hipSuccess) {
		(void)hipStreamSynchronize(ctx->coop_stream);
		(void)hipStreamSynchronize(ctx->side_stream);
		(void)hipStreamSynchronize(ctx->stream);
		return fail(ctx, what, e);
	}
	(P.adaptive ? ctx->acc.adaptive_calls : ctx->acc.uniform_calls)++;
	ctx->acc.scan_pairs += pairs;
	ctx->acc.scan_query_nt += nt;
	return 0;
}
```

andi_amd/csrc/scan_lane.hip:

```cpp
#include "lane_chain.h"
#include "knobs.h"

#include <algorithm>

namespace {

[[maybe_unused]] constexpr uint32_t EST_WAVES = 4;
constexpr uint32_t EST_WAVES_FEW = 8;
__device__ __forceinline__ uint32_t cost_class(uint32_t mean) {
	const uint32_t m = mean < 1u ? 1u : mean, e = 31u - (uint32_t)__builtin_clz(m);
	const uint32_t lg = 4u * e + (((m << 2) >> e) & 3u);
	return lg < ANDI_COST_CLASSES ? ANDI_COST_CLASSES - 1u - lg : 0u;
}

__global__ __launch_bounds__(64 * EST_WAVES_FEW) void k_pair_estimate(ScanArgs a, bool many) {
	__shared__ uint32_t s_shorts, s_runs;
	const uint32_t est_waves = many ? 1u : blockDim.x >> 6;
	const uint32_t pair = many ? blockIdx.x * (blockDim.x >> 6) + (threadIdx.x >> 6) : blockIdx.x, wave = many ? 0u : threadIdx.x >> 6;
	const uint32_t lane = threadIdx.x & 63u;
	if (pair >= a.nsub * a.nq) return;
	const uint32_t sub = pair / a.nq, qidx = pair % a.nq;
	const bool first = many ? lane == 0 : threadIdx.x == 0;
	if (a.self[sub] == (int64_t)qidx) {
		if (first) a.pair_class[pair] = 0, a.pair_waves[pair] = 0;
		if (first && a.pair_cost) a.pair_cost[pair] = 0;
		return;
	}
	if (!many) {
		if (threadIdx.x == 0) s_shorts = 0, s_runs = 0;
		__syncthreads();
	}
	PairCtx c = make_ctx(a, sub, qidx);
	const uint32_t nl_shift = !a.route || c.qlen >= 32768u ? 6u : c.qlen >= 16384u ? 5u : 4u, nl = 1u << nl_shift;
	const uint32_t p = (uint32_t)(((uint64_t)(2 * lane + 1) * c.qlen) >> (nl_shift + 1));
	LWin w;
	w.q0 = EMPTY, w.dg = NO_DIAG;
	const uint32_t cap = a.adaptive ? 16 * a.seg0 / (a.seg_factor ? a.seg_factor : 1) / 2 + 32 : 96u;
	Probe r;
	r.len = 0;
	if (lane < nl) r = lane_probe(c, p, w, cap);
	uint32_t sum = r.len < cap ? r.len : cap;
#pragma unroll
	for (int d = 32; d; d >>= 1) sum += (uint32_t)__shfl_xor((int)sum, d);
	sum <<= 6u - nl_shift;
	bool islands = false, guess = false, far_clean = false;
	const bool quad_cand = (sum >> 6) >= a.quad_min_match && (sum >> 6) < ANDI_ISLAND_MEAN_MAX && a.quad_min_match != 0;
	uint32_t break_dist = ~0u;
	if (a.qsep && a.self[sub] >= 0) {
		const uint32_t ends = a.qsep[qidx] + a.qsep[(uint32_t)a.self[sub]];
		if (ends) break_dist = c.qlen / ends;
	}
	const bool coop_cand = a.route && (sum >> 6) < 512u && c.qlen >= (a.route_seg < ANDI_ROUTE_MIN_QLEN ? a.route_seg : ANDI_ROUTE_MIN_QLEN) && break_dist >= 20480u;
	if (coop_cand) {
		const uint32_t T = c.thr + 3;
		uint32_t nrounds = est_waves > 1 ? 8u : 4u;
		while (nrounds > 1 && c.qlen < nrounds * (64u * 2048u)) nrounds >>= 1;
		const uint32_t nsamples = nl * nrounds;
		uint32_t shorts = 0, runs = 0;
		for (uint32_t k = wave; k < nrounds; k += est_waves) {
			const uint32_t pk = (uint32_t)(((uint64_t)(2 * nrounds * lane + 2 * k + 1) * c.qlen) / (2u * nl * nrounds));
			bool all_short = lane < nl;
			for (uint32_t j = 0; j < 5 && all_short; ++j) {
				const uint32_t pj = pk + 128 * j;
				LWin wk;
				wk.q0 = EMPTY, wk.dg = NO_DIAG;
				all_short = pj + T < c.qlen && lane_probe(c, pj, wk, T + 1).len < T;
				if (j == 0 && all_short) ++shorts;
			}
			if (all_short) ++runs;
		}
#pragma unroll
		for (int d = 32; d; d >>= 1) shorts += (uint32_t)__shfl_xor((int)shorts, d), runs += (uint32_t)__shfl_xor((int)runs, d);
		if (!many) {
			if (lane == 0) atomicAdd(&s_shorts, shorts), atomicAdd(&s_runs, runs);
			__syncthreads();
			shorts = s_shorts, runs = s_runs;
		}
		const float ns = (float)nsamples;
		float g = (float)(shorts - runs) / ns, f0;
		if (g > 0.53f) g = 0.53f;
		f0 = g;
		for (int it = 0; it < 5; ++it) {
			const float f4 = f0 * f0 * f0 * f0;
			f0 -= (f0 - f0 * f4 - g) / (1.f - 5.f * f4);
		}
		const float f5 = f0 * f0 * f0 * f0 * f0, expect = ns * f5;
		islands = (float)runs > expect + 3.f * sqrtf(expect * (1.f - f5)) + 3.f;
		if (islands) {
			const float fa = (float)shorts / ns, fa5 = fa * fa * fa * fa * fa, most = ns * fa5;
			far_clean = (float)runs <= 2.f * most + 10.f;
		}
		if (a.route_all_few && ((sum >> 6) < ANDI_SPARSE_MATCH || (float)(shorts - runs) >= 0.45f * ns)) {
			const float fa = (float)shorts / ns, fa5 = fa * fa * fa * fa * fa, most = ns * fa5;
			islands = (float)runs > most + 3.f * sqrtf(most * (1.f - fa5)) + 3.f;
			guess = !islands;
		}
	} else if (quad_cand && nl == 64) {
		uint32_t shorts = r.len < c.thr ? 1u : 0u;
		for (uint32_t k = 1; k < 4; ++k) {
			const uint32_t pk = (uint32_t)(((uint64_t)(8 * lane + 2 * k + 1) * c.qlen) >> 9);
			LWin wk;
			wk.q0 = EMPTY, wk.dg = NO_DIAG;
			const Probe rk = lane_probe(c, pk, wk, c.thr + 1);
			shorts += rk.len < c.thr ? 1u : 0u;
		}
#pragma unroll
		for (int d = 32; d; d >>= 1) shorts += (uint32_t)__shfl_xor((int)shorts, d);
		const float expect = 256.f * (1.f - __expf(-(float)c.thr / (float)(sum >> 6)));
		islands = (float)shorts > expect + 2.f * sqrtf(expect * (1.f - expect / 256.f)) + 2.f;
	}
	if (first) {
		const uint32_t want = (sum >> 6) * a.seg_factor;
		uint32_t cls = 0;
		while (cls < a.max_class && (a.seg0 << cls) < want) ++cls;
		const uint32_t seg = a.seg0 << cls, nseg = (c.qlen + seg - 1) / seg;
		const bool far = islands && far_clean;
		const bool soft = (sum >> 6) < ANDI_SPARSE_MATCH || (sum >> 6) >= 512u || far;
		if (far) islands = false, guess = true;
		const bool quad = (sum >> 6) >= a.quad_min_match && !(islands && (sum >> 6) < ANDI_ISLAND_MEAN_MAX);
		a.pair_class[pair] = (uint8_t)(cls | (quad ? 0x80u : 0u) | (coop_cand && !islands ? ANDI_ROUTE_COOP : 0u) | (soft ? ANDI_ROUTE_SOFT : 0u) |
										 (coop_cand && islands ? ANDI_ROUTE_LEFT : 0u) | (coop_cand && guess ? ANDI_ROUTE_GUESS : 0u) |
										 (a.route && (sum >> 6) >= a.pool_match && (sum >> 6) < 4096u && break_dist >= 262144u ? ANDI_ROUTE_POOLCAND : 0u));
		a.pair_waves[pair] = (nseg + 63) / 64;
		if (a.pair_cost) a.pair_cost[pair] = (uint8_t)cost_class(sum >> 6);
		if (a.sub_cost && !many) atomicAdd(&a.sub_cost[sub], (float)c.qlen / (float)((sum >> 6) < 8u ? 8u : (sum >> 6)));
		if (islands) atomicAdd(&a.restitch_count[ANDI_STRUCT_WAVES], (nseg + 63) / 64);
	}
}

__device__ __forceinline__ uint32_t block_scan_1024(uint32_t v, uint32_t *s_part) {
	s_part[threadIdx.x] = v;
	__syncthreads();
	for (uint32_t d = 1; d < 1024; d <<= 1) {
		const uint32_t o = threadIdx.x >= d ? s_part[threadIdx.x - d] : 0;
		__syncthreads();
		s_part[threadIdx.x] += o;
		__syncthreads();
	}
	return s_part[threadIdx.x];
}

__global__ __launch_bounds__(1024) void k_pair_block_sums(ScanArgs a) {
	__shared__ uint32_t s_part[1024];
	const uint32_t P = a.nsub * a.nq, i = blockIdx.x * 1024 + threadIdx.x;
	const uint32_t incl = block_scan_1024(i < P ? a.pair_waves[i] : 0u, s_part);
	if (threadIdx.x == 1023) a.pair_bsum[blockIdx.x] = incl;
}

__global__ __launch_bounds__(1024) void k_pair_block_offsets(ScanArgs a) {
	__shared__ uint32_t s_part[1024];
	const uint32_t P = a.nsub * a.nq, nb = (P + 1023) / 1024, per = (nb + 1023) / 1024;
	const uint32_t first = threadIdx.x * per, last = first + per < nb ? first + per : nb;
	uint32_t sum = 0;
	for (uint32_t i = first; i < last; ++i) sum += a.pair_bsum[i];
	uint32_t run = block_scan_1024(sum, s_part) - sum;
	for (uint32_t i = first; i < last; ++i) {
		const uint32_t v = a.pair_bsum[i];
		a.pair_bsum[i] = run;
		run += v;
	}
	if (threadIdx.x == 1023) a.pair_wave0[P] = s_part[1023];
}

__global__ __launch_bounds__(1024) void k_pair_offsets(ScanArgs a) {
	__shared__ uint32_t s_part[1024];
	const uint32_t P = a.nsub * a.nq, i = blockIdx.x * 1024 + threadIdx.x;
	const uint32_t v = i < P ? a.pair_waves[i] : 0u;
	const uint32_t incl = block_scan_1024(v, s_part);
	if (i < P) {
		const uint32_t w0 = a.pair_bsum[blockIdx.x] + incl - v;
		a.pair_wave0[i] = w0;
		if ((a.pair_class[i] & 0x80u) && v) {
			uint32_t *list = (uint32_t *)a.defer_list;
			const uint32_t base = atomicAdd(&a.restitch_count[ANDI_QUAD_WAVES], v);
			for (uint32_t k = 0; k < v; ++k) list[base + k] = w0 + k;
		}
	}
}

__global__ __launch_bounds__(1024) void k_pair_totals(ScanArgs a) {
	__shared__ uint32_t s_sum[4];
	const uint32_t P = a.nsub * a.nq, pair = blockIdx.x * 1024 + threadIdx.x;
	if (threadIdx.x < 4) s_sum[threadIdx.x] = 0;
	__syncthreads();
	uint32_t all = 0, sparse = 0, hard = 0, isl = 0;
	if (pair < P) {
		const uint32_t cls = a.pair_class[pair];
		all = a.pair_waves[pair];
		hard = (cls & ANDI_ROUTE_COOP) ? 0u : all;
		sparse = (cls & ANDI_ROUTE_SOFT) ? all : hard;
		isl = (cls & ANDI_ROUTE_LEFT) ? all : 0u;
	}
#pragma unroll
	for (int d = 32; d; d >>= 1) {
		all += (uint32_t)__shfl_xor((int)all, d);
		sparse += (uint32_t)__shfl_xor((int)sparse, d);
		hard += (uint32_t)__shfl_xor((int)hard, d);
		isl += (uint32_t)__shfl_xor((int)isl, d);
	}
	if ((threadIdx.x & 63u) == 0) atomicAdd(&s_sum[0], all), atomicAdd(&s_sum[1], sparse), atomicAdd(&s_sum[2], hard), atomicAdd(&s_sum[3], isl);
	__syncthreads();
	if (threadIdx.x == 0) {
		if (s_sum[0]) atomicAdd(&a.restitch_count[ANDI_ALL_WAVES], s_sum[0]);
		if (s_sum[1]) atomicAdd(&a.restitch_count[ANDI_SPARSE_WAVES], s_sum[1]);
		if (s_sum[2]) atomicAdd(&a.restitch_count[ANDI_HARD_WAVES], s_sum[2]);
		if (s_sum[3]) atomicAdd(&a.restitch_count[ANDI_ISLAND_WAVES], s_sum[3]);
	}
}

__device__ __forceinline__ uint32_t route_pair(const ScanArgs &a, uint32_t pair, uint32_t &pool_segs, uint32_t &coop_segs) {
	uint32_t cls = a.pair_class[pair];
	const bool lanes_few = 10 * a.restitch_count[ANDI_SPARSE_WAVES] <= a.restitch_count[ANDI_ALL_WAVES];
	if ((cls & ANDI_ROUTE_COOP) && (cls & ANDI_ROUTE_SOFT) && !lanes_few && !a.route_all_few) cls &= ~ANDI_ROUTE_COOP;
	if ((cls & ANDI_ROUTE_GUESS) && 20 * a.restitch_count[ANDI_ISLAND_WAVES] > a.restitch_count[ANDI_ALL_WAVES]) cls &= ~ANDI_ROUTE_COOP;
	if ((cls & (ANDI_ROUTE_LEFT | ANDI_ROUTE_GUESS)) && !(cls & ANDI_ROUTE_COOP) && (cls & 3u) < a.max_class && 3 * a.restitch_count[ANDI_STRUCT_WAVES] >= a.restitch_count[ANDI_ALL_WAVES]) {
		++cls;
		const uint32_t seg = a.seg0 << (cls & 3u);
		a.pair_waves[pair] = ((a.qlen[pair % a.nq] + seg - 1) / seg + 63) / 64;
	}
	const bool pool = (cls & ANDI_ROUTE_POOLCAND) != 0;
	cls &= ~(ANDI_ROUTE_SOFT | ANDI_ROUTE_LEFT | ANDI_ROUTE_GUESS | ANDI_ROUTE_POOLCAND);
	if (a.route_all_few && 20 * a.restitch_count[ANDI_HARD_WAVES] <= a.restitch_count[ANDI_ALL_WAVES] && a.self[pair / a.nq] != (int64_t)(pair % a.nq))
		cls |= ANDI_ROUTE_COOP;
	if (cls & ANDI_ROUTE_COOP) {
		const uint32_t segs = (a.qlen[pair % a.nq] + a.route_seg - 1) / a.route_seg;
		coop_segs += segs, pool_segs += pool ? segs : 0u;
	}
	a.pair_class[pair] = (uint8_t)cls;
	if (cls & ANDI_ROUTE_COOP) a.pair_waves[pair] = 0;
	return a.pair_waves[pair];
}

__global__ __launch_bounds__(256) void k_pair_route(ScanArgs a) {
	const uint32_t P = a.nsub * a.nq, pair = blockIdx.x * 256 + threadIdx.x;
	uint32_t mine = 0, pool_segs = 0, coop_segs = 0;
	if (pair < P) mine = route_pair(a, pair, pool_segs, coop_segs);
#pragma unroll
	for (int d = 32; d; d >>= 1)
		mine += (uint32_t)__shfl_xor((int)mine, d), pool_segs += (uint32_t)__shfl_xor((int)pool_segs, d), coop_segs += (uint32_t)__shfl_xor((int)coop_segs, d);
	if ((threadIdx.x & 63u) == 0 && mine) atomicAdd(&a.restitch_count[ANDI_LANE_WAVES], mine);
	if ((threadIdx.x & 63u) == 0 && coop_segs) atomicAdd(&a.restitch_count[ANDI_COOP_SEGS], coop_segs), atomicAdd(&a.restitch_count[ANDI_POOL_SEGS], pool_segs);
}
__global__ __launch_bounds__(1024) void k_sub_order(ScanArgs a) {
	for (uint32_t s = threadIdx.x; s < a.nsub; s += 1024) {
		if (a.nsub > 8192u) {
			a.sub_order[s] = s;
			continue;
		}
		const float c = a.sub_cost[s];
		uint32_t rank = 0;
		for (uint32_t t = 0; t < a.nsub; ++t) {
			const float o = a.sub_cost[t];
			rank += (o > c || (o == c && t < s)) ? 1u : 0u;
		}
		a.sub_order[rank] = s;
	}
}

enum { ITEMS_ALL, ITEMS_HIST, ITEMS_PLACE };
static_assert(ANDI_COST_CLASSES * 16 == 1024, "k_items: the table [class][wavefront] is one entry per thread of the block");

template <int MODE>
__global__ __launch_bounds__(1024) void k_items(ScanArgs a, uint32_t nblocks) {
	__shared__ uint32_t s_cnt[1024], s_part[1024];
	const uint32_t t = threadIdx.x, lane = t & 63u, wave = t >> 6, pair = blockIdx.x * 1024 + t;
	uint32_t segs = 0, first = 0, key = 0;
	if (pair < a.nsub * a.nq && (a.pair_class[pair] & ANDI_ROUTE_COOP)) {
		const uint32_t sub = pair / a.nq, q = pair % a.nq, w0 = a.qseg_start[q];
		segs = a.qseg_start[q + 1] - w0, first = sub * a.total_segs + w0;
		const uint32_t cost = a.pair_cost[pair] < ANDI_COST_CLASSES ? a.pair_cost[pair] : ANDI_COST_CLASSES - 1u;
		key = a.items_order == ANDI_ITEMS_LIGHT ? cost : ANDI_COST_CLASSES - 1u - cost;
	}
	s_cnt[t] = 0;
	__syncthreads();
	uint32_t place = 0;
	for (uint64_t todo = __ballot(segs != 0); todo;) {
		const uint32_t k = (uint32_t)__shfl((int)key, (int)__builtin_ctzll(todo));
		const bool same = segs != 0 && key == k;
		uint32_t incl = same ? segs : 0u;
#pragma unroll
		for (int d = 1; d < 64; d <<= 1) {
			const uint32_t o = (uint32_t)__shfl_up((int)incl, d);
			incl += lane >= (uint32_t)d ? o : 0u;
		}
		if (same) place = incl - segs;
		if (lane == 63) s_cnt[16 * k + wave] = incl;
		todo &= ~__ballot(same);
	}
	__syncthreads();
	const uint32_t cnt = s_cnt[t], incl = block_scan_1024(cnt, s_part);
	s_cnt[t] = incl - cnt;
	__syncthreads();
	if (MODE == ITEMS_HIST) {
		if (t < ANDI_COST_CLASSES) a.item_hist[(size_t)t * nblocks + blockIdx.x] = s_part[16 * t + 15] - s_cnt[16 * t];
		return;
	}
	place += s_cnt[16 * key + wave];
	if (MODE == ITEMS_PLACE) place += a.item_hist[(size_t)key * nblocks + blockIdx.x] - s_cnt[16 * key];
	const uint32_t n_items = a.layout_count[ANDI_COOP_SEGS];
	if (place >= n_items || segs > n_items - place) segs = 0;
	if (segs <= 8)
		for (uint32_t i = 0; i < segs; ++i) a.coop_items[place + i] = first + i;
	for (uint64_t big = __ballot(segs > 8); big; big &= big - 1) {
		const int l = __builtin_ctzll(big);
		const uint32_t p = (uint32_t)__shfl((int)place, l), s = (uint32_t)__shfl((int)segs, l), f = (uint32_t)__shfl((int)first, l);
		for (uint32_t i = lane; i < s; i += 64) a.coop_items[p + i] = f + i;
	}
}

__global__ __launch_bounds__(1024) void k_items_scan(ScanArgs a, uint32_t n) {
	__shared__ uint32_t s_part[1024];
	const uint32_t per = (n + 1023) / 1024;
	const uint32_t first = threadIdx.x * per < n ? threadIdx.x * per : n, last = first + per < n ? first + per : n;
	uint32_t sum = 0;
	for (uint32_t i = first; i < last; ++i) sum += a.item_hist[i];
	uint32_t run = block_scan_1024(sum, s_part) - sum;
	for (uint32_t i = first; i < last; ++i) {
		const uint32_t v = a.item_hist[i];
		a.item_hist[i] = run;
		run += v;
	}
}

__global__ __launch_bounds__(256) void k_pair_leftover(ScanArgs a) {
	const uint32_t P = a.nsub * a.nq, pair = blockIdx.x * 256 + threadIdx.x;
	if (pair >= P) return;
	const uint32_t sub = pair / a.nq, qidx = pair % a.nq;
	uint32_t cls = a.pair_class[pair], waves = 0;
	if (a.self[sub] != (int64_t)qidx && (cls & ANDI_ROUTE_COOP) && (cls & ANDI_ROUTE_LEFT)) {
		cls = (cls & ~(ANDI_ROUTE_COOP | ANDI_ROUTE_LEFT)) | ANDI_ROUTE_L2;
		const uint32_t seg = a.seg0 << (cls & 3u), nseg = (a.qlen[qidx] + seg - 1) / seg;
		a.pair_class[pair] = (uint8_t)cls;
		waves = (nseg + 63) / 64;
	}
	a.pair_waves[pair] = waves;
}

__global__ __launch_bounds__(256) void k_route_count(ScanArgs a) {
	const uint32_t P = a.nsub * a.nq, pair = blockIdx.x * 256 + threadIdx.x;
	unsigned long long nt[2] = {0, 0};
	uint32_t back = 0;
	if (pair < P && a.self[pair / a.nq] != (int64_t)(pair % a.nq)) {
		const uint32_t cls = a.pair_class[pair];
		nt[(cls & ANDI_ROUTE_COOP) ? 0 : 1] = a.qlen[pair % a.nq];
		back = (cls & ANDI_ROUTE_L2) ? 1u : 0u;
	}
#pragma unroll
	for (int d = 32; d; d >>= 1) {
		nt[0] += (unsigned long long)__shfl_xor((long long)nt[0], d);
		nt[1] += (unsigned long long)__shfl_xor((long long)nt[1], d);
		back += (uint32_t)__shfl_xor((int)back, d);
	}
	if ((threadIdx.x & 63u) == 0) {
		if (nt[0]) atomicAdd(&a.route_nt[0], nt[0]);
		if (nt[1]) atomicAdd(&a.route_nt[1], nt[1]);
		if (back) atomicAdd(&a.route_nt[2], (unsigned long long)back);
	}
}


__device__ __forceinline__ uint32_t dpp_quad_floor(uint32_t v, int ctrl) {
	switch (ctrl) {
		case 0: return (uint32_t)__builtin_amdgcn_update_dpp(0, (int)v, 0x00, 0xF, 0xF, true);
		case 1: return (uint32_t)__builtin_amdgcn_update_dpp(0, (int)v, 0x55, 0xF, 0xF, true);
		case 2: return (uint32_t)__builtin_amdgcn_update_dpp(0, (int)v, 0xAA, 0xF, 0xF, true);
		case 3: return (uint32_t)__builtin_amdgcn_update_dpp(0, (int)v, 0xFF, 0xF, 0xF, true);
		case 4: return (uint32_t)__builtin_amdgcn_update_dpp(0, (int)v, 0xB1, 0xF, 0xF, true);
		default: return (uint32_t)__builtin_amdgcn_update_dpp(0, (int)v, 0x4E, 0xF, 0xF, true);
	}
}


__device__ __forceinline__ bool pos_in(const LWin &w, uint32_t p) {
	return w.q0 != EMPTY && p >= w.q0 && p - w.q0 < WNT;
}

__device__ __forceinline__ void lane_note_anchor(const ScanArgs &a, size_t slot, uint32_t anchors, const ChainState &st, const Tally &tally) {
	ColdMark *marks = a.marks + slot * ANDI_COLD_MARKS;
	if (anchors == 1) *(uint4 *)marks[0].first = make_uint4(st.lastQ, st.lastS, st.lastLen, 0);
	if (anchors >= 2 && anchors < 2 + ANDI_COLD_MARKS) {
		ColdMark *m = marks + (anchors - 2);
		ChainState ms = st;
		ms.pad[0] = 1;
		m->st = ms;
		uint32_t v[16];
#pragma unroll
		for (int t = 0; t < 16; ++t) v[t] = tally.hist[t * BLOCK];
		v[0] += tally.quarter + tally.same[0], v[5] += tally.quarter + tally.same[1];
		v[10] += tally.quarter + tally.same[2], v[15] += tally.quarter + tally.rest + tally.same[3];
		uint4 *mc = (uint4 *)m->counts;
#pragma unroll
		for (int t = 0; t < 4; ++t) mc[t] = make_uint4(v[4 * t], v[4 * t + 1], v[4 * t + 2], v[4 * t + 3]);
	}
}
__device__ __forceinline__ void lane_finish(const ScanArgs &a, size_t slot, uint32_t anchors, ChainState &st, Tally &tally) {
	ColdMark *marks = a.marks + slot * ANDI_COLD_MARKS;
	for (uint32_t k = anchors < 2 ? 0 : anchors - 1; k < ANDI_COLD_MARKS; ++k) marks[k].st.pad[0] = 0;
	st.pad[1] = anchors < 255 ? anchors : 255;
	a.cold_exit[slot] = st;
	a.exit_p[slot] = st.p;
	tally_finish<1>(tally);
	uint32_t out[16];
#pragma unroll
	for (int t = 0; t < 16; ++t) out[t] = tally.hist[t * BLOCK];
	uint4 *dst = (uint4 *)(a.cold_counts + slot * 16);
#pragma unroll
	for (int t = 0; t < 4; ++t) dst[t] = make_uint4(out[4 * t], out[4 * t + 1], out[4 * t + 2], out[4 * t + 3]);
}
// ... 585 lines not shown
			x = (x | (x << 2)) & 0x33333333u;
			return (x | (x << 1)) & 0x55555555u;
		};
		*(uint2 *)(codes + 2 * j) = make_uint2(spread(o[0]) | (spread(o[1]) << 1), spread(o[0] >> 16) | (spread(o[1] >> 16) << 1));
	}
}

__device__ __forceinline__ void pack_text_block(const uint8_t *__restrict__ src, int64_t symbols, uint8_t *__restrict__ N0,
												uint8_t *__restrict__ N1, uint32_t *__restrict__ P, int32_t *__restrict__ foreign) {
	__shared__ uint8_t lut[256];
	lut[threadIdx.x] = (uint8_t)(symbol_of((uint8_t)threadIdx.x) | (in_alphabet((uint8_t)threadIdx.x) ? 0u : 0x80u));
	__syncthreads();
	const int64_t j = (int64_t)blockIdx.x * blockDim.x + threadIdx.x;
	if (32 * j >= symbols) return;
	const bool whole = 32 * j + 16 < symbols;
	const uint4 lo = ld_u128_unaligned((g_u8p)src + 32 * j), hi = ld_u128_unaligned((g_u8p)src + 32 * j + 16);
	const uint32_t in[8] = {lo.x, lo.y, lo.z, lo.w, hi.x, hi.y, hi.z, hi.w};
	uint32_t w[4] = {0, 0, 0, 0}, bad = 0, bad_hi = 0;
#pragma unroll
	for (int k = 0; k < 32; ++k) {
		const uint32_t e = lut[(in[k >> 2] >> (8 * (k & 3))) & 0xffu];
		w[k >> 3] |= (e & 7u) << (4 * (k & 7));
		if (k < 16) bad |= e; else bad_hi |= e;
	}
	if (whole) bad |= bad_hi;
	if ((bad & 0x80u) && foreign) *foreign = 1;
	const uint32_t prev = j ? (lut[src[32 * j - 1]] & 7u) : 7u;
	const uint2 a0 = make_uint2(w[0], w[1]), a1 = make_uint2((w[0] << 4) | prev, (w[1] << 4) | (w[0] >> 28));
	if (whole) {
		((uint4 *)N0)[j] = make_uint4(a0.x, a0.y, w[2], w[3]);
		if (N1) ((uint4 *)N1)[j] = make_uint4(a1.x, a1.y, (w[2] << 4) | (w[1] >> 28), (w[3] << 4) | (w[2] >> 28));
	} else {
		((uint2 *)N0)[2 * j] = a0;
		if (N1) ((uint2 *)N1)[2 * j] = a1;
	}
	if (P) {
		uint32_t o[3];
		planes_of(make_uint4(w[0], w[1], w[2], w[3]), o);
		P[3 * j] = o[0], P[3 * j + 1] = o[1], P[3 * j + 2] = o[2];
	}
}

__global__ __launch_bounds__(256) void k_pack_text(const uint8_t *__restrict__ src, int64_t symbols, uint8_t *__restrict__ N0,
												   uint8_t *__restrict__ N1, uint32_t *__restrict__ P, int32_t *__restrict__ foreign) {
	pack_text_block(src, symbols, N0, N1, P, foreign);
}

__global__ __launch_bounds__(256) void k_pack_text_batch(const AndiIndexBatchItem *__restrict__ items) {
	const AndiIndexBatchItem it = items[blockIdx.y];
	pack_text_block(it.S, (int64_t)it.n + 1 + 64, it.N0, it.N1, it.P, it.flags + 1);
}

}

#ifdef ANDI_QUAD_TU
hipError_t andi_launch_lane_quad_small(const ScanArgs &a0, uint32_t count, hipStream_t st) {
	if (count == 0) return hipSuccess;
	ScanArgs a = a0;
	a.quad_listed = 1;
	if (a.exact_equal)
		k_lane_quad<true><<<count, BLOCK, 0, st>>>(a);
	else
		k_lane_quad<false><<<count, BLOCK, 0, st>>>(a);
	return hipGetLastError();
}
#else

hipError_t andi_launch_pack_text_batch(const AndiIndexBatchItem *d_items, uint32_t count, size_t max_n, hipStream_t st) {
	const int64_t blocks = (int64_t)((max_n + 1 + 64 + 31) / 32);
	if (count == 0) return hipSuccess;
	k_pack_text_batch<<<dim3((unsigned)((blocks + 255) / 256), count), 256, 0, st>>>(d_items);
	CHECK_LAUNCH();
	return hipSuccess;
}

hipError_t andi_launch_pack_text(const uint8_t *src, size_t symbols, uint8_t *N0, uint8_t *N1, uint32_t *P, int32_t *foreign,
								 hipStream_t st) {
	const int64_t blocks = (int64_t)((symbols + 31) / 32);
	if (blocks == 0) return hipSuccess;
	k_pack_text<<<(unsigned)((blocks + 255) / 256), 256, 0, st>>>(src, (int64_t)symbols, N0, N1, P, foreign);
	CHECK_LAUNCH();
	return hipSuccess;
}

hipError_t andi_launch_unpack_symbols(const uint8_t *N0, size_t bytes, uint8_t *dst, hipStream_t st) {
	const int64_t pairs = (int64_t)(bytes / 16);
	if (pairs == 0) return hipSuccess;
	k_unpack_symbols<<<(unsigned)((pairs + 255) / 256), 256, 0, st>>>((const uint2 *)N0, pairs, (uint4 *)dst);
	CHECK_LAUNCH();
	return hipSuccess;
}

hipError_t andi_launch_pack_planes(const uint8_t *N0, size_t symbols, uint32_t *planes, uint32_t *codes, hipStream_t st) {
	const int64_t blocks = (int64_t)((symbols + 31) / 32);
	if (blocks == 0) return hipSuccess;
	k_pack_planes<<<(unsigned)((blocks + 255) / 256), 256, 0, st>>>((const uint4 *)N0, blocks, planes, codes);
	CHECK_LAUNCH();
	return hipSuccess;
}

hipError_t andi_launch_pack_symbols(const uint8_t *src, size_t bytes, uint8_t *N0, uint8_t *N1,
									int32_t *foreign, hipStream_t st) {
	const int64_t pairs = (int64_t)((bytes + 15) / 16);
	if (pairs == 0) return hipSuccess;
	k_pack_symbols<<<(unsigned)((pairs + 255) / 256), 256, 0, st>>>(src, pairs, (uint2 *)N0, (uint2 *)N1, foreign);
	CHECK_LAUNCH();
	return hipSuccess;
}

template <bool EXACT>
static hipError_t lane_cold(const ScanArgs &a, dim3 grid, hipStream_t st) {
	const bool blocks4 = andi_knob(KNOB_QUAD_UNLISTED) != nullptr;
	const bool quads = a.adaptive && a.quad_min_match != 0xffffffffu;
	const bool side = quads && a.side_stream && !andi_knob(KNOB_NO_SIDE_STREAM);
	const bool counted = side && a.h_quad_waves && !blocks4 && !andi_knob(KNOB_QUAD_BLOCKS4);
	if (quads) {
		(void)hipMemsetAsync(a.first_pub, 0xff, (size_t)64 * a.max_waves * sizeof(unsigned long long), st);
		if (side) {
			(void)hipEventRecord(a.side_fork, st);
			(void)hipStreamWaitEvent(a.side_stream, a.side_fork, 0);
		}
		if (!counted) {
			ScanArgs b = a;
			b.quad_listed = blocks4 ? 0 : 1;
			k_lane_quad<EXACT><<<grid, BLOCK, 0, side ? a.side_stream : st>>>(b);
			if (side) (void)hipEventRecord(a.side_join, a.side_stream);
		}
	}
	if (a.adaptive) k_lane_cold<EXACT, true><<<grid, BLOCK, 0, st>>>(a);
	else k_lane_cold<EXACT, false><<<grid, BLOCK, 0, st>>>(a);
	hipError_t e = hipSuccess;
	if (counted) {
		(void)hipMemcpyAsync(a.h_quad_waves, a.restitch_count + ANDI_QUAD_WAVES, sizeof(uint32_t), hipMemcpyDeviceToHost, a.side_stream);
		e = hipStreamSynchronize(a.side_stream);
		if (e == hipSuccess) e = andi_launch_lane_quad_small(a, *a.h_quad_waves, a.side_stream);
		(void)hipEventRecord(a.side_join, a.side_stream);
	}
	if (side) (void)hipStreamWaitEvent(st, a.side_join, 0);
	return e != hipSuccess ? e : hipGetLastError();
}

static hipError_t pair_offsets(const ScanArgs &a, hipStream_t st) {
	const uint32_t P = a.nsub * a.nq;
	const unsigned nb = (P + 1023) / 1024;
	k_pair_block_sums<<<nb, 1024, 0, st>>>(a);
	CHECK_LAUNCH();
	k_pair_block_offsets<<<1, 1024, 0, st>>>(a);
	CHECK_LAUNCH();
	k_pair_offsets<<<nb, 1024, 0, st>>>(a);
	CHECK_LAUNCH();
	return hipSuccess;
}

hipError_t andi_launch_pair_layout(const ScanArgs &a, hipStream_t st) {
	const uint32_t P = a.nsub * a.nq;
	(void)hipMemsetAsync(a.restitch_count, 0, 16 * sizeof(uint32_t), st);
	if (a.sub_cost) (void)hipMemsetAsync(a.sub_cost, 0, a.nsub * sizeof(float), st);
	if (P <= 4096) k_pair_estimate<<<P, P <= 1024 ? 64 * EST_WAVES_FEW : 64 * EST_WAVES, 0, st>>>(a, false);
	else k_pair_estimate<<<(P + 3) / 4, 256, 0, st>>>(a, true);
	CHECK_LAUNCH();
	if (a.route) {
		k_pair_totals<<<(P + 1023) / 1024, 1024, 0, st>>>(a);
		CHECK_LAUNCH();
		k_pair_route<<<(P + 255) / 256, 256, 0, st>>>(a);
		CHECK_LAUNCH();
		if (a.sub_order) {
			k_sub_order<<<1, 1024, 0, st>>>(a);
			CHECK_LAUNCH();
		}
	}
	return a.adaptive ? pair_offsets(a, st) : hipSuccess;
}

hipError_t andi_launch_coop_items(const ScanArgs &b, hipStream_t st) {
	const uint32_t P = b.nsub * b.nq, nblocks = (P + 1023) / 1024;
	if (nblocks == 1) {
		k_items<ITEMS_ALL><<<1, 1024, 0, st>>>(b, 1);
	} else {
		k_items<ITEMS_HIST><<<nblocks, 1024, 0, st>>>(b, nblocks);
		k_items_scan<<<1, 1024, 0, st>>>(b, ANDI_COST_CLASSES * nblocks);
		k_items<ITEMS_PLACE><<<nblocks, 1024, 0, st>>>(b, nblocks);
	}
	CHECK_LAUNCH();
	return hipSuccess;
}

hipError_t andi_launch_pair_leftover(const ScanArgs &a2, hipStream_t st) {
	const uint32_t P = a2.nsub * a2.nq;
	(void)hipMemsetAsync(a2.restitch_count + ANDI_QUAD_WAVES, 0, 3 * sizeof(uint32_t), st);
	k_pair_leftover<<<(P + 255) / 256, 256, 0, st>>>(a2);
	CHECK_LAUNCH();
	return a2.adaptive ? pair_offsets(a2, st) : hipSuccess;
}

hipError_t andi_launch_route_count(const ScanArgs &a, hipStream_t st) {
	const uint32_t P = a.nsub * a.nq;
	k_route_count<<<(P + 255) / 256, 256, 0, st>>>(a);
	CHECK_LAUNCH();
	return hipSuccess;
}

static dim3 lane_grid(const ScanArgs &a) {
	if (a.adaptive) return dim3((a.max_waves + WAVES_PER_BLOCK - 1) / WAVES_PER_BLOCK, 1);
	return dim3((a.total_segs + BLOCK - 1) / BLOCK, a.nsub);
}

hipError_t andi_launch_lane_cold(const ScanArgs &a, hipStream_t st) {
	dim3 grid = lane_grid(a);
	hipError_t e = a.exact_equal ? lane_cold<true>(a, grid, st) : lane_cold<false>(a, grid, st);
#ifdef ANDI_LANE_STATS
	if (e == hipSuccess && andi_knob(KNOB_LANE_STATS)) {
		static const char *names[24] = {"steps", "lcp_reload", "lcp_slide", "probes", "probe_reload", "table", "final_sa",
										"single", "ext_loop", "multi", "multi_cand", "search", "gap_reload", "gap_words",
										"substitutions", "lucky_tries", "x0", "x1", "x2", "x3", "x4", "x5", "x6", "x7"};
		unsigned long long h[24];
		(void)hipStreamSynchronize(st);
		(void)hipMemcpyFromSymbol(h, HIP_SYMBOL(g_lane_stats), sizeof h);
		for (int k = 0; k < 24; ++k) fprintf(stderr, "lane_stats %-14s %llu\n", names[k], h[k]);
		memset(h, 0, sizeof h);
		(void)hipMemcpyToSymbol(HIP_SYMBOL(g_lane_stats), h, sizeof h);
	}
#endif
	return e;
}

hipError_t andi_launch_lane_stitch(const ScanArgs &a0, hipStream_t st) {
	hipStream_t st_ = st;
	(void)st_;
	dim3 grid = lane_grid(a0);
	ScanArgs a = a0;
	hipError_t e = hipMemsetAsync(a.restitch_count, 0, 16 * sizeof(uint32_t), st);
	if (e != hipSuccess) return e;
	const size_t slots = a.adaptive ? (size_t)64 * a.max_waves : (size_t)a.nsub * a.total_segs;
	const uint32_t per_block = WAVES_PER_BLOCK * ANDI_LISTED_LANES;
	const unsigned lblocks = (unsigned)std::min<size_t>((slots + per_block - 1) / per_block, ANDI_LISTED_BLOCKS);
	static_assert(ANDI_RESTITCH_ROUNDS <= 3, "a list counter per round: restitch_count[13 ... 15]");
	auto stage = [&](auto main_kernel, auto listed_kernel, dim3 main_grid, uint32_t counter) {
		a.defer_count = a.restitch_count + counter;
		main_kernel<<<main_grid, BLOCK, 0, st>>>(a);
		listed_kernel<<<lblocks, BLOCK, 0, st>>>(a);
	};
	dim3 grid0 = grid;
	a.stitch_lanes = 0;
	if (!a.adaptive && slots < (size_t)64 * 8192) {
		uint32_t L = 1;
		while ((size_t)L * 8192 < slots) L *= 2;
		if (L < 64) a.stitch_lanes = L, grid0 = dim3((a.total_segs + WAVES_PER_BLOCK * L - 1) / (WAVES_PER_BLOCK * L), a.nsub);
	}
	if (a.exact_equal)
		stage(k_lane_stitch<true, 0>, k_lane_stitch<true, 1>, grid0, 8);
	else
		stage(k_lane_stitch<false, 0>, k_lane_stitch<false, 1>, grid0, 8);
#ifdef ANDI_LANE_STATS
	if (andi_knob(KNOB_LANE_STATS)) {
		static const char *names[8] = {"entered behind the cold chain's first anchor", "met behind its first anchor", "met at a mark",
									   "met in phase 2", "position-synced", "left on their own", "steps of those that left on their own", "steps of the others"};
		unsigned long long h[24];
		(void)hipStreamSynchronize(st);
		(void)hipMemcpyFromSymbol(h, HIP_SYMBOL(g_lane_stats), sizeof h);
		for (int k = 0; k < 8; ++k) fprintf(stderr, "stitch_stats %-48s %llu\n", names[k], h[ST_X0 + k]);
		fprintf(stderr, "stitch_stats %-48s %llu\n", "reached phase 2", h[ST_SEARCH]);
		memset(h, 0, sizeof h);
		(void)hipMemcpyToSymbol(HIP_SYMBOL(g_lane_stats), h, sizeof h);
	}
#endif
	const bool again = !andi_knob(KNOB_NO_RESTITCH);
	for (uint32_t r = 0; again && r < ANDI_RESTITCH_ROUNDS; ++r) {
		a.restitch_round = r;
		if (a.exact_equal)
			stage(k_stitch_heads, k_lane_stitch<true, 2>, grid, 13 + r);
		else
			stage(k_stitch_heads, k_lane_stitch<false, 2>, grid, 13 + r);
	}
#ifdef ANDI_LANE_STATS
	if (andi_knob(KNOB_LANE_STATS)) {
		static const char *kinds[4] = {"first stage", "first stage, listed", "-", "stretches stitched again (segments)"};
		unsigned long long h[4][16], st[4];
		unsigned int mx[4];
		(void)hipStreamSynchronize(st_);
		(void)hipMemcpyFromSymbol(h, HIP_SYMBOL(g_stitch_hist), sizeof h);
		(void)hipMemcpyFromSymbol(st, HIP_SYMBOL(g_stitch_steps), sizeof st);
		(void)hipMemcpyFromSymbol(mx, HIP_SYMBOL(g_stitch_max), sizeof mx);
		{
			uint32_t rc[16];
			(void)hipMemcpy(rc, a.restitch_count, sizeof rc, hipMemcpyDeviceToHost);
			fprintf(stderr, "stitch_rounds stretches listed per round: %u %u %u; left on their own: %u\n", rc[0], rc[1], rc[2], rc[ANDI_RESTITCH_ROUNDS]);
		}
		{
			static const char *xn[8] = {"left for the list", "shortcut", "first anchor", "mark", "met", "position", "on its own", "-"};
			unsigned long long x[4][8][2];
			(void)hipMemcpyFromSymbol(x, HIP_SYMBOL(g_stitch_exit), sizeof x);
			for (int k = 0; k < 4; ++k)
				for (int e = 0; e < 7; ++e)
					if (x[k][e][0]) fprintf(stderr, "stitch_exit kind %d %-18s %9llu replays %10llu steps\n", k, xn[e], x[k][e][0], x[k][e][1]);
			memset(x, 0, sizeof x);
			(void)hipMemcpyToSymbol(HIP_SYMBOL(g_stitch_exit), x, sizeof x);
			unsigned long long ph[4][8];
			(void)hipMemcpyFromSymbol(ph, HIP_SYMBOL(g_stitch_phase), sizeof ph);
			for (int k = 0; k < 4; ++k)
				fprintf(stderr, "stitch_phase kind %d steps: phase 0 true %llu cold %llu, phase 1 %llu, phase 2 true %llu cold %llu, alone %llu; put at the first anchor %llu\n", k,
						ph[k][0], ph[k][1], ph[k][2], ph[k][3], ph[k][4], ph[k][5], ph[k][6]);
			memset(ph, 0, sizeof ph);
			(void)hipMemcpyToSymbol(HIP_SYMBOL(g_stitch_phase), ph, sizeof ph);
		}
		for (int k = 0; k < 4; ++k) {
			fprintf(stderr, "stitch_len %-22s steps %llu max %u  by log2:", kinds[k], st[k], mx[k]);
			for (int b = 0; b < 16; ++b) fprintf(stderr, " %llu", h[k][b]);
			fprintf(stderr, "\n");
		}
		memset(h, 0, sizeof h), memset(st, 0, sizeof st), memset(mx, 0, sizeof mx);
		(void)hipMemcpyToSymbol(HIP_SYMBOL(g_stitch_hist), h, sizeof h);
		(void)hipMemcpyToSymbol(HIP_SYMBOL(g_stitch_steps), st, sizeof st);
		(void)hipMemcpyToSymbol(HIP_SYMBOL(g_stitch_max), mx, sizeof mx);
	}
#endif
	return hipGetLastError();
}
#endif
```

andi_amd/lib.py:

```python
import ctypes as C
import os

import numpy as np

_HERE = os.path.dirname(os.path.abspath(__file__))
LIB_PATH = os.environ.get("ANDI_HIP_LIB") or os.path.join(_HERE, "libandihip.so")

M_RAW, M_JC, M_KIMURA, M_LOGDET, M_ANI = range(5)
MODEL_NAMES = {"raw": M_RAW, "jc": M_JC, "kimura": M_KIMURA, "logdet": M_LOGDET, "ani": M_ANI}


class AndiHipError(RuntimeError):
    pass


class Seq(C.Structure):
    _fields_ = [("seq", C.c_char_p), ("len", C.c_size_t)]


class Model(C.Structure):
    _fields_ = [("counts", C.c_uint32 * 16), ("seq_len", C.c_uint32)]


class Interval(C.Structure):
# ... 11 lines not shown
        ("host_threads", C.c_int),
        ("low_memory", C.c_int),
        ("segment", C.c_uint32),
        ("progress", PROGRESS_FN),
        ("ud", C.c_void_p),
        ("sa_on_host", C.c_int),
        ("num_gpus", C.c_int),
        ("devices", C.POINTER(C.c_int)),
    ]


class Timings(C.Structure):
    _fields_ = [
        ("build_ms", C.c_double),
        ("build_launches", C.c_uint64),
        ("scan_ms", C.c_double),
        ("scan_launches", C.c_uint64),
        ("stitch_ms", C.c_double),
        ("stitch_launches", C.c_uint64),
        ("scan_query_nt", C.c_uint64),
        ("scan_pairs", C.c_uint64),
        ("fixups", C.c_uint64),
        ("reference_subjects", C.c_uint64),
        ("sa_ms", C.c_double),
        ("sa_builds", C.c_uint64),
        ("sa_rounds", C.c_uint64),
        ("adaptive_calls", C.c_uint64),
        ("uniform_calls", C.c_uint64),
        ("coop_calls", C.c_uint64),
        ("coop_fallbacks", C.c_uint64),
        ("routed_calls", C.c_uint64),
        ("coop_query_nt", C.c_uint64),
        ("lane_query_nt", C.c_uint64),
        ("pool_calls", C.c_uint64),
    ]


_P = C.c_void_p
SYMBOLS = {
    "andi_hip_default_opts": (None, [C.POINTER(Opts)]),
    "andi_hip_abi_version": (C.c_int, []),
    "andi_hip_trim": (C.c_size_t, []),
    "andi_hip_pack_symbols": (C.c_int, [C.c_char_p, C.c_size_t, C.c_void_p]),
    "andi_hip_dist_matrix": (C.c_int, [_P, C.POINTER(Seq), C.c_size_t, C.POINTER(Opts), C.c_char_p, C.c_size_t]),
    "andi_hip_dist_rect": (C.c_int, [_P, _P, C.POINTER(Seq), C.c_size_t, C.POINTER(Seq), C.c_size_t, C.POINTER(Opts),
                                     C.c_char_p, C.c_size_t]),
    "andi_hip_last_gather": (C.c_char_p, []),
    "andi_hip_row_block": (None, [C.c_size_t, C.c_size_t, C.c_size_t, C.POINTER(C.c_size_t), C.POINTER(C.c_size_t)]),
    "andi_hip_copy_ceiling": (C.c_int, [_P, C.c_size_t, C.c_int, C.POINTER(C.c_double)]),
    "andi_hip_subject_prepare": (C.c_int, [C.c_char_p, C.c_size_t, C.c_double, C.POINTER(_P),
                                            C.POINTER(C.c_size_t), C.POINTER(C.c_double),
                                            C.POINTER(C.c_size_t)]),
    "andi_hip_free": (None, [_P]),
    "andi_hip_min_anchor_length": (C.c_size_t, [C.c_double, C.c_double, C.c_size_t]),
    "andi_hip_shustring_cum_prob": (C.c_double, [C.c_size_t, C.c_double, C.c_size_t]),
    "andi_hip_suffix_array": (C.c_int, [_P, _P, C.c_int32]),
    "andi_hip_suffix_sorter": (C.c_char_p, []),
    "andi_hip_model_average": (Model, [C.POINTER(Model), C.POINTER(Model)]),
    "andi_hip_model_coverage": (C.c_double, [C.POINTER(Model)]),
    "andi_hip_estimate": (C.c_double, [C.POINTER(Model), C.c_int]),
    "andi_hip_format_distances": (C.c_size_t, [_P, C.POINTER(C.c_char_p), C.c_size_t, C.c_int, C.c_int,
                                               C.c_int, C.c_int, _P, C.c_size_t, _P, C.c_size_t,
                                               C.POINTER(C.c_int)]),
    "andi_hip_format_distances_rect": (C.c_size_t, [_P, _P, C.POINTER(C.c_char_p), C.c_size_t, C.POINTER(C.c_char_p),
                                                    C.c_size_t, C.c_int, C.c_int, C.c_int, C.c_int, _P, C.c_size_t, _P,
                                                    C.c_size_t, C.POINTER(C.c_int)]),
    "andi_hip_distances": (C.c_int, [_P, C.c_size_t, C.c_int, _P]),
    "andi_hip_format_newick": (C.c_size_t, [_P, C.c_size_t, C.POINTER(C.c_char_p), C.c_int, _P, C.c_size_t]),
    "andi_hip_format_newick_support": (C.c_size_t, [_P, _P, C.c_size_t, C.POINTER(C.c_char_p), C.c_int, _P, C.c_size_t]),
    "andi_hip_format_newick_transfer": (C.c_size_t, [_P, _P, _P, C.c_size_t, C.c_size_t, C.POINTER(C.c_char_p), C.c_int, _P,
                                                     C.c_size_t]),
    "andi_hip_consensus": (C.c_int, [_P, C.c_size_t, C.c_size_t, _P, _P, C.c_size_t, _P, _P, _P, C.POINTER(C.c_size_t)]),
    "andi_hip_format_newick_consensus": (C.c_size_t, [_P, C.c_size_t, C.c_size_t, C.POINTER(C.c_char_p), C.c_int, _P,
                                                      C.c_size_t]),
    "andi_hip_nj": (C.c_int, [_P, _P, C.c_size_t, _P]),
    "andi_hip_nj_batch": (C.c_int, [_P, _P, C.c_size_t, C.c_size_t, _P, _P]),
    "andi_hip_tree": (C.c_int, [_P, _P, C.c_size_t, C.c_int, _P]),
    "andi_hip_tree_batch": (C.c_int, [_P, _P, C.c_size_t, C.c_size_t, C.c_int, _P, _P]),
    "andi_hip_nj_support": (C.c_int, [_P, _P, _P, C.c_size_t, C.c_size_t, _P, _P]),
    "andi_hip_nj_splits": (C.c_int, [_P, _P, C.c_size_t, C.c_size_t, _P, _P, C.POINTER(C.c_size_t), C.POINTER(_P),
                                     C.POINTER(_P)]),
    "andi_hip_nj_transfer": (C.c_int, [_P, _P, _P, C.c_size_t, C.c_size_t, _P, _P, _P, _P]),
    "andi_hip_nj_transfer_taxa": (C.c_int, [_P, _P, _P, C.c_size_t, C.c_size_t, _P, C.c_double, _P, _P, _P, _P]),
    "andi_hip_linkage": (C.c_int, [_P, _P, C.c_size_t, C.c_int, _P]),
    "andi_hip_linkage_batch": (C.c_int, [_P, _P, C.c_size_t, C.c_size_t, C.c_int, _P, _P]),
    "andi_hip_linkage_cut": (C.c_int, [_P, C.c_size_t, C.c_double, _P, C.POINTER(C.c_size_t)]),
    "andi_hip_cluster_medoids": (C.c_int, [_P, C.c_size_t, _P, C.c_size_t, _P]),
    "andi_hip_cluster_stability": (C.c_int, [_P, C.c_size_t, _P, C.c_size_t, C.c_size_t, _P]),
    "andi_hip_format_newick_linkage": (C.c_size_t, [_P, C.c_size_t, C.POINTER(C.c_char_p), C.c_int, _P, C.c_size_t]),
    "andi_hip_complete": (C.c_int, [_P, _P, C.c_size_t, C.c_uint, _P, _P, C.c_size_t, C.POINTER(C.c_size_t),
                                    C.POINTER(C.c_size_t)]),
    "andi_hip_complete_batch": (C.c_int, [_P, _P, C.c_size_t, C.c_size_t, C.c_uint, _P, _P, _P]),
    "andi_hip_delta_scores": (C.c_int, [_P, _P, C.c_size_t, _P]),
    "andi_hip_place": (C.c_int, [_P, _P, C.c_size_t, _P, C.c_size_t, C.c_int, _P, _P, _P, _P]),
    "andi_hip_distances_rect": (C.c_int, [_P, _P, C.c_size_t, C.c_size_t, C.c_int, _P]),
    "andi_hip_root": (C.c_int, [_P, _P, C.c_size_t, C.c_int, _P, _P, _P]),
    "andi_hip_format_newick_rooted": (C.c_size_t, [_P, C.c_size_t, C.POINTER(C.c_char_p), C.c_int, C.c_int32, C.c_double,
                                                   C.POINTER(C.c_char_p), _P, C.c_size_t]),
    "andi_hip_parse_newick": (C.c_int, [C.c_char_p, C.POINTER(C.c_char_p), C.c_size_t, C.c_int, _P, C.c_char_p, C.c_size_t]),
    "andi_hip_format_jplace": (C.c_size_t, [_P, C.c_size_t, C.POINTER(C.c_char_p), C.c_int, _P, C.c_size_t,
                                            C.POINTER(C.c_char_p), C.c_int, _P, C.c_size_t]),
    "andi_hip_sketch": (C.c_int, [_P, C.POINTER(Seq), C.c_size_t, C.c_int, C.c_uint64, C.POINTER(_P)]),
    "andi_hip_sketch_count": (C.c_size_t, [_P]),
    "andi_hip_sketch_sizes": (C.c_int, [_P, _P, _P]),
    "andi_hip_sketch_download": (C.c_int, [_P, _P, C.c_size_t, _P]),
    "andi_hip_sketch_free": (None, [_P, _P]),
    "andi_hip_sketch_timings": (C.c_int, [_P, _P]),
    "andi_hip_sketch_shared": (C.c_int, [_P, _P, _P, _P]),
    "andi_hip_screen_select": (C.c_int, [_P, C.c_size_t, C.c_size_t, C.c_size_t, C.c_uint32, _P, _P]),
    "andi_hip_screen": (C.c_int, [C.POINTER(Seq), C.c_size_t, C.POINTER(Seq), C.c_size_t, C.c_int, C.c_uint64, C.c_int, _P, _P, _P,
                                  C.c_char_p, C.c_size_t]),
    "andi_hip_device_count": (C.c_int, []),
    "andi_hip_reload_knobs": (None, []),
    "andi_hip_ctx_create": (C.c_int, [C.POINTER(_P), C.c_int, C.c_char_p, C.c_size_t]),
    "andi_hip_ctx_destroy": (None, [_P]),
    "andi_hip_ctx_expect_queries": (None, [_P, C.c_size_t]),
    "andi_hip_last_error": (C.c_char_p, [_P]),
    "andi_hip_sync": (C.c_int, [_P]),
    "andi_hip_esa_stage": (C.c_int, [_P, _P, _P, C.c_size_t, C.c_size_t, C.POINTER(_P)]),
    "andi_hip_esa_stage_text": (C.c_int, [_P, _P, C.c_size_t, C.c_size_t, C.POINTER(_P)]),
    "andi_hip_esa_download_sa": (C.c_int, [_P, _P, _P]),
    "andi_hip_esa_build": (C.c_int, [_P, _P]),
    "andi_hip_esa_build_index": (C.c_int, [_P, _P]),
    "andi_hip_esa_build_index_batch": (C.c_int, [_P, C.POINTER(_P), C.c_size_t]),
    "andi_hip_esa_flags": (C.c_int, [_P, _P, _P]),
    "andi_hip_esa_download": (C.c_int, [_P, _P, _P, _P, _P, _P]),
    "andi_hip_esa_download_index": (C.c_int, [_P, _P, _P, C.POINTER(C.c_int)]),
    "andi_hip_esa_single_form": (C.c_int, [_P]),
    "andi_hip_esa_free": (None, [_P, _P]),
    "andi_hip_esa_bytes": (C.c_size_t, [_P]),
    "andi_hip_queries_stage": (C.c_int, [_P, C.POINTER(Seq), C.c_size_t, C.POINTER(_P)]),
    "andi_hip_queries_free": (None, [_P, _P]),
    "andi_hip_queries_view": (C.c_int, [_P, _P, C.c_size_t, C.c_size_t, C.POINTER(_P)]),
    "andi_hip_match_positions": (C.c_int, [_P, _P, _P, C.c_size_t, C.c_size_t, C.c_size_t, C.c_int, _P]),
    "andi_hip_scan_rows": (C.c_int, [_P, C.POINTER(_P), C.POINTER(C.c_int64), C.c_size_t, _P, C.c_int,
                                     C.c_uint32, _P]),
    "andi_hip_bootstrap": (C.c_int, [_P, _P, C.c_size_t, C.c_uint64, C.c_size_t, _P]),
    "andi_hip_bootstrap_range": (C.c_int, [_P, _P, C.c_size_t, C.c_uint64, C.c_size_t, C.c_size_t, _P]),
    "andi_hip_bootstrap_nj": (C.c_int, [_P, _P, C.c_size_t, C.c_int, C.c_uint64, C.c_size_t, C.c_size_t, _P, _P, _P]),
    "andi_hip_bootstrap_tree": (C.c_int, [_P, _P, C.c_size_t, C.c_int, C.c_int, C.c_uint64, C.c_size_t, C.c_size_t, _P, _P,
                                          _P]),
    "andi_hip_estimate_portable": (C.c_int, [_P, C.c_size_t, C.c_int, _P]),
    "andi_hip_dev_alloc": (C.c_int, [_P, C.c_size_t, C.POINTER(_P)]),
    "andi_hip_dev_free": (None, [_P, _P]),
    "andi_hip_copy_to_host": (C.c_int, [_P, _P, _P, C.c_size_t]),
    "andi_hip_timings_get": (C.c_int, [_P, C.POINTER(Timings)]),
    "andi_hip_timings_reset": (None, [_P]),
}

HOOK_SYMBOLS = {
    "andi_hip_test_download_text": (C.c_int, [_P, _P, _P, _P, C.c_size_t, _P, C.c_size_t]),
    "andi_hip_test_pack_text": (C.c_int, [_P, _P, C.c_int]),
    "andi_hip_test_coop_items": (C.c_int, [_P, _P, C.c_size_t, _P, _P, C.c_size_t, _P]),
    "andi_hip_test_query_codes": (C.c_int, [_P, _P, C.c_size_t, _P, C.c_size_t]),
    "andi_hip_test_stitch_slots": (C.c_int, [_P, _P, _P, _P, _P, _P, _P, C.c_size_t, _P, _P]),
}

_lib = None


def load():
    global _lib
    if _lib is None:
        if not os.path.exists(LIB_PATH):
            raise AndiHipError(
                f"{LIB_PATH} not found: build it with `python -c 'import __graft_entry__ as g; g.build()'` "
                "(make -C andi_amd/csrc); there is no CPU fallback")
        L = C.CDLL(LIB_PATH)
        for name, (res, args) in SYMBOLS.items():
            fn = getattr(L, name)
            fn.restype = res
            fn.argtypes = args
        for name, (res, args) in HOOK_SYMBOLS.items():
            fn = getattr(L, name, None)
            if fn is not None:
                fn.restype = res
                fn.argtypes = args
        _lib = L
        import atexit
        atexit.register(L.andi_hip_trim)
    return _lib


def _seq_array(seqs):
    arr = (Seq * len(seqs))()
    for k, s in enumerate(seqs):
        arr[k].seq = s
        arr[k].len = len(s)
    return arr


def subject_prepare(seq: bytes, p_value=0.025):
    L = load()
    rs, n, gc, thr = _P(), C.c_size_t(), C.c_double(), C.c_size_t()
    if L.andi_hip_subject_prepare(seq, len(seq), p_value, C.byref(rs), C.byref(n), C.byref(gc), C.byref(thr)):
        raise AndiHipError("andi_hip_subject_prepare failed")
    try:
        RS = C.string_at(rs, n.value)
    finally:
        L.andi_hip_free(rs)
    return RS, gc.value, thr.value


def min_anchor_length(p, g, l):
    return load().andi_hip_min_anchor_length(p, g, l)


def shustring_cum_prob(x, p, l):
    return load().andi_hip_shustring_cum_prob(x, p, l)


def suffix_array(text: bytes):
    n = len(text)
    buf = C.create_string_buffer(text, n + 1)
    sa = np.empty(n, dtype=np.int32)
    if load().andi_hip_suffix_array(C.cast(buf, _P), sa.ctypes.data, n):
        raise AndiHipError("andi_hip_suffix_array failed")
    return sa


def _model(counts17):
    m = Model()
    for k in range(16):
        m.counts[k] = int(counts17[k])
    m.seq_len = int(counts17[16])
    return m


def estimate(counts17, model=M_JC):
    return load().andi_hip_estimate(C.byref(_model(counts17)), model)


def coverage(counts17):
    return load().andi_hip_model_coverage(C.byref(_model(counts17)))


def format_distances(M, names, model=M_JC, extra_verbose=False, truncate_names=False, warnings=True):
    L = load()
    M = np.ascontiguousarray(M, dtype=np.uint32)
    n = M.shape[0]
    assert M.shape == (n, n, 17)
    cnames = (C.c_char_p * n)(*[s.encode() if isinstance(s, str) else s for s in names])
    cap = 64 + n * (64 + 16 * n)
    warn = C.create_string_buffer(1 << 20)
    flags = C.c_int()
    for _ in range(2):
        out = C.create_string_buffer(cap)
        need = L.andi_hip_format_distances(M.ctypes.data, cnames, n, model, int(extra_verbose), int(truncate_names),
                                           int(warnings), C.cast(out, _P), cap, C.cast(warn, _P), len(warn),
                                           C.byref(flags))
        if need < cap:
            break
        cap = need + 1
    return out.value.decode(), warn.value.decode(), flags.value


def _names(names):
    return (C.c_char_p * len(names))(*[s.encode() if isinstance(s, str) else s for s in names])


def format_distances_rect(MRQ, MQR, ref_names, query_names, model=M_JC, extra_verbose=False, truncate_names=False,
                          warnings=True):
    L = load()
    MRQ = np.ascontiguousarray(MRQ, dtype=np.uint32)
    MQR = np.ascontiguousarray(MQR, dtype=np.uint32)
    nr, nq = MRQ.shape[0], MQR.shape[0]
    assert MRQ.shape == (nr, nq, 17) and MQR.shape == (nq, nr, 17)
    assert len(ref_names) == nr and len(query_names) == nq
    rn, qn = _names(ref_names), _names(query_names)
    cap = 64 + 16 * nr + nq * (64 + 16 * nr) + sum(len(x) for x in ref_names) + sum(len(x) for x in query_names)
    warn = C.create_string_buffer(1 << 20)
    flags = C.c_int()
    for _ in range(2):
        out = C.create_string_buffer(cap)
        need = L.andi_hip_format_distances_rect(MRQ.ctypes.data, MQR.ctypes.data, rn, nr, qn, nq, model,
                                                int(extra_verbose), int(truncate_names), int(warnings),
                                                C.cast(out, _P), cap, C.cast(warn, _P), len(warn), C.byref(flags))
        if need < cap:
            break
        cap = need + 1
    return out.value.decode(), warn.value.decode(), flags.value


NJ_JOIN = np.dtype([("a", "<i4"), ("b", "<i4"), ("c", "<i4"), ("pad", "<i4"), ("la", "<f8"), ("lb", "<f8"),
                    ("lc", "<f8")])


def distances(M, model=M_JC):
    M = np.ascontiguousarray(M, dtype=np.uint32)
    n = M.shape[0]
    assert M.shape == (n, n, 17)
    D = np.empty((n, n), np.float64)
    if load().andi_hip_distances(M.ctypes.data, n, model, D.ctypes.data):
        raise AndiHipError("andi_hip_distances failed")
    return D


def newick(joins, names, truncate_names=False, support=None):
    J = np.ascontiguousarray(joins, dtype=NJ_JOIN)
    n = len(names)
    cn = _names(names)
    cap = 64 + 40 * n + sum(len(x) for x in names)
    if support is not None:
        support = np.ascontiguousarray(support, dtype=np.uint32)
        assert len(support) >= max(n - 3, 0)
        cap += 10 * n
# ... 69 lines not shown
    cap = 64 + 60 * n + sum(len(x) for x in names)
    for _ in range(2):
        out = C.create_string_buffer(cap)
        need = load().andi_hip_format_newick_consensus(nodes.ctypes.data, n, ninner, cn, int(truncate_names),
                                                       C.cast(out, _P), cap)
        if need < cap:
            break
        cap = need + 1
    return out.value.decode()


LINK = np.dtype([("a", "<i4"), ("b", "<i4"), ("size", "<u4"), ("pad", "<u4"), ("height", "<f8")])
LINKAGE_METHODS = {"single": 0, "complete": 1, "average": 2}


def _method(method):
    if method not in LINKAGE_METHODS:
        raise ValueError("linkage method %r: expected single, complete or average" % (method,))
    return LINKAGE_METHODS[method]


def linkage_cut(Z, t):
    Z = np.ascontiguousarray(Z, dtype=LINK)
    n = len(Z) + 1
    labels = np.zeros(n, np.uint32)
    k = C.c_size_t(0)
    if load().andi_hip_linkage_cut(Z.ctypes.data, n, float(t), labels.ctypes.data, C.byref(k)):
        raise AndiHipError("andi_hip_linkage_cut: malformed records")
    return labels


def cluster_medoids(D, labels):
    D = np.ascontiguousarray(D, dtype=np.float64)
    labels = np.ascontiguousarray(labels, dtype=np.uint32)
    n = D.shape[0]
    assert D.shape == (n, n) and labels.shape == (n,)
    k = int(labels.max()) + 1
    medoid = np.zeros(k, np.uint32)
    if load().andi_hip_cluster_medoids(D.ctypes.data, n, labels.ctypes.data, k, medoid.ctypes.data):
        raise AndiHipError("andi_hip_cluster_medoids: bad arguments")
    return medoid


def cluster_stability(labels, rep_labels):
    labels = np.ascontiguousarray(labels, dtype=np.uint32)
    rep_labels = np.ascontiguousarray(rep_labels, dtype=np.uint32)
    n = len(labels)
    assert rep_labels.ndim == 2 and rep_labels.shape[1] == n
    k = int(labels.max()) + 1
    stability = np.zeros(k, np.uint32)
    if load().andi_hip_cluster_stability(labels.ctypes.data, k, rep_labels.ctypes.data, n, rep_labels.shape[0],
                                         stability.ctypes.data):
        raise AndiHipError("andi_hip_cluster_stability: bad arguments")
    return stability


def newick_linkage(Z, names, truncate_names=False):
    Z = np.ascontiguousarray(Z, dtype=LINK)
    n = len(names)
    assert len(Z) == n - 1
    cn = _names(names)
    cap = 64 + 40 * n + sum(len(x) for x in names)
    for _ in range(2):
        out = C.create_string_buffer(cap)
        need = load().andi_hip_format_newick_linkage(Z.ctypes.data, n, cn, int(truncate_names), C.cast(out, _P), cap)
        if need < cap:
            break
        cap = need + 1
    return out.value.decode()


PLACEMENT = np.dtype([("edge", "<i4"), ("used", "<u4"), ("distal", "<f8"), ("pendant", "<f8"), ("err", "<f8")])
PLACE_METHODS = {"ols": 0, "fm": 1}


def _place_method(method):
    if method not in PLACE_METHODS:
        raise ValueError("placement method %r: expected fm or ols" % (method,))
    return PLACE_METHODS[method]


def distances_rect(MRQ, MQR, model=M_JC):
    MRQ = np.ascontiguousarray(MRQ, dtype=np.uint32)
    MQR = np.ascontiguousarray(MQR, dtype=np.uint32)
    nr, nq = MRQ.shape[0], MQR.shape[0]
    assert MRQ.shape == (nr, nq, 17) and MQR.shape == (nq, nr, 17)
    D = np.empty((nq, nr), np.float64)
    if load().andi_hip_distances_rect(MRQ.ctypes.data, MQR.ctypes.data, nr, nq, model, D.ctypes.data):
        raise AndiHipError("andi_hip_distances_rect failed")
    return D


def parse_newick(text, names, truncate_names=False):
    n = len(names)
    J = np.zeros(max(n - 2, 0), NJ_JOIN)
    err = C.create_string_buffer(512)
    raw = text.encode() if isinstance(text, str) else bytes(text)
    if load().andi_hip_parse_newick(raw, _names(names), n, int(truncate_names), J.ctypes.data, err, len(err)):
        raise AndiHipError(err.value.decode(errors="replace"))
    return J


def jplace(J, ref_names, placements, query_names, method="fm", truncate_names=False):
    J = np.ascontiguousarray(J, dtype=NJ_JOIN)
    P = np.ascontiguousarray(placements, dtype=PLACEMENT)
    n, nq = len(ref_names), len(query_names)
    assert len(J) == n - 2 and P.shape == (nq,)
    rn, qn = _names(ref_names), _names(query_names)
    cap = 512 + 64 * n + sum(len(x) for x in ref_names) + 128 * nq + sum(len(x) for x in query_names)
    for _ in range(2):
        out = C.create_string_buffer(cap)
        need = load().andi_hip_format_jplace(J.ctypes.data, n, rn, int(truncate_names), P.ctypes.data, nq, qn,
                                             _place_method(method), C.cast(out, _P), cap)
        if need < cap:
            break
        cap = need + 1
    return out.value.decode()


class Context:
    def __init__(self, device=0):
        L = load()
        self._h = _P()
        err = C.create_string_buffer(512)
        if L.andi_hip_ctx_create(C.byref(self._h), device, err, len(err)):
            raise AndiHipError(err.value.decode())
        self.device = device

    def expect_queries(self, queries):
        load().andi_hip_ctx_expect_queries(self._h, int(queries))

    def _check(self, rc, what):
        if rc:
            raise AndiHipError(f"{what}: {load().andi_hip_last_error(self._h).decode()}")

    def sync(self):
        self._check(load().andi_hip_sync(self._h), "sync")

    def timings(self):
        t = Timings()
        self._check(load().andi_hip_timings_get(self._h, C.byref(t)), "timings")
        return {k: getattr(t, k) for k, _ in Timings._fields_}

    def timings_reset(self):
        load().andi_hip_timings_reset(self._h)

    def coop_items(self):
        hook = _hook("andi_hip_test_coop_items")
        info = np.zeros(4, np.uint32)
        self._check(hook(self._h, None, 0, None, None, 0, info.ctypes.data), "test_coop_items")
        items, cls, cost = np.zeros(int(info[0]), np.uint32), np.zeros(int(info[1]), np.uint8), np.zeros(int(info[1]), np.uint8)
        self._check(hook(self._h, items.ctypes.data, len(items), cls.ctypes.data, cost.ctypes.data, len(cls), info.ctypes.data), "test_coop_items")
        return (items if info[3] else None), cls, cost, int(info[2])

    def stitch_slots(self):
        hook = _hook("andi_hip_test_stitch_slots")
        info = np.zeros(4, np.uint32)
        self._check(hook(self._h, None, None, None, None, None, None, 0, None, info.ctypes.data), "test_stitch_slots")
        if not info[3]:
            raise AndiHipError("test_stitch_slots: no scan call with one segment length on record")
        n = int(info[0]) * int(info[1])
        out = {"cold_exit": np.zeros((n, 8), np.uint32), "true_exit": np.zeros((n, 8), np.uint32), "used_entry": np.zeros((n, 8), np.uint32),
               "cold_counts": np.zeros((n, 16), np.uint32), "owned": np.zeros((n, 16), np.uint32), "marks": np.zeros((n, 28), np.uint32),
               "restitch_count": np.zeros(16, np.uint32)}
        p = {k: v.ctypes.data for k, v in out.items()}
        self._check(hook(self._h, p["cold_exit"], p["true_exit"], p["used_entry"], p["cold_counts"], p["owned"], p["marks"], n,
                         p["restitch_count"], info.ctypes.data), "test_stitch_slots")
        out.update(nsub=int(info[0]), total_segs=int(info[1]), seg=int(info[2]))
        return out

    def alloc(self, nbytes):
        p = _P()
        self._check(load().andi_hip_dev_alloc(self._h, nbytes, C.byref(p)), "dev_alloc")
        return p

    def free(self, p):
        load().andi_hip_dev_free(self._h, p)

    def close(self):
        if self._h:
            load().andi_hip_ctx_destroy(self._h)
            self._h = _P()

    def __del__(self):
        try:
            self.close()
        except Exception:
            pass


class Esa:

    def __init__(self, ctx: Context, seq: bytes, p_value=0.025, sa=None, build="index", prepared=None):
        self.ctx = ctx
        if prepared is not None:
            self.RS, self.gc, self.threshold, sa = prepared
        else:
            self.RS, self.gc, self.threshold = subject_prepare(seq, p_value)
        self.n = len(self.RS)
        self._h = _P()
        L = load()
        if isinstance(sa, str) and sa == "device":
            self._SA = None
            ctx._check(L.andi_hip_esa_stage_text(ctx._h, self.RS, self.n, self.threshold, C.byref(self._h)),
                       "esa_stage_text")
        else:
            self._SA = suffix_array(self.RS) if sa is None else np.ascontiguousarray(sa, dtype=np.int32)
            ctx._check(L.andi_hip_esa_stage(ctx._h, self.RS, self._SA.ctypes.data, self.n, self.threshold,
                                            C.byref(self._h)), "esa_stage")
        self.reference_built = False
        if build in ("index", "both", True):
            self.build()
        if build in ("reference", "both"):
            self.build_reference()

    @property
    def SA(self):
        if self._SA is None:
            sa = np.empty(self.n, np.int32)
            self.ctx._check(load().andi_hip_esa_download_sa(self.ctx._h, self._h, sa.ctypes.data), "esa_download_sa")
            self._SA = sa
        return self._SA

    def build(self):
        self.ctx._check(load().andi_hip_esa_build_index(self.ctx._h, self._h), "esa_build_index")

    def build_reference(self):
        self.ctx._check(load().andi_hip_esa_build(self.ctx._h, self._h), "esa_build")
        self.reference_built = True

    def flags(self):
        out = np.zeros(4, np.int32)
        self.ctx._check(load().andi_hip_esa_flags(self.ctx._h, self._h, out.ctypes.data), "esa_flags")
        return out

    def download(self):
        if not self.reference_built:
            self.build_reference()
        n = self.n
        LCP = np.empty(n + 1, np.int32)
        CLD = np.empty(n + 1, np.int32)
        FVC = np.empty(n, np.uint8)
        cache = np.empty((1 << 20, 4), np.int32)
        self.ctx._check(load().andi_hip_esa_download(self.ctx._h, self._h, LCP.ctypes.data, CLD.ctypes.data,
                                                     FVC.ctypes.data, cache.ctypes.data), "esa_download")
        return LCP, CLD, FVC, cache

    def download_index(self):
        K = C.c_int(0)
        self.ctx._check(load().andi_hip_esa_download_index(self.ctx._h, self._h, None, C.byref(K)), "esa_download_index")
        table = np.empty((1 << (2 * K.value), 2), np.uint32)
        self.ctx._check(load().andi_hip_esa_download_index(self.ctx._h, self._h, table.ctypes.data, C.byref(K)),
                        "esa_download_index")
        return K.value, table

    def pack_text(self, forms=3):
        self.ctx._check(_hook("andi_hip_test_pack_text")(self.ctx._h, self._h, forms), "test_pack_text")

    def download_text(self, beyond=16):
        nib = (self.n + 1 + 64 + 15) // 16 * 8 + beyond
        N0, N1 = np.empty(nib, np.uint8), np.empty(nib, np.uint8)
        P = np.empty(3 + 3 * ((self.n + 1 + 64 + 31) // 32) + beyond // 4, np.uint32)
        self.ctx._check(_hook("andi_hip_test_download_text")(self.ctx._h, self._h, N0.ctypes.data, N1.ctypes.data, nib,
                                                             P.ctypes.data, len(P)), "test_download_text")
        return N0, N1, P

    def single_form(self):
        return load().andi_hip_esa_single_form(self._h)

    def nbytes(self):
        return load().andi_hip_esa_bytes(self._h)

    def close(self):
        if self._h and self.ctx._h:
            load().andi_hip_esa_free(self.ctx._h, self._h)
        self._h = _P()

    def __del__(self):
        try:
            self.close()
        except Exception:
            pass


def prepare_host(seq: bytes, p_value=0.025):
    RS, gc, thr = subject_prepare(seq, p_value)
    return RS, gc, thr, suffix_array(RS)


class Queries:
    def __init__(self, ctx: Context, seqs):
        self.ctx = ctx
        self.seqs = [bytes(s) for s in seqs]
        self._arr = _seq_array(self.seqs)
        self._h = _P()
        ctx._check(load().andi_hip_queries_stage(ctx._h, self._arr, len(self.seqs), C.byref(self._h)),
                   "queries_stage")

    def __len__(self):
        return len(self.seqs)

    def view(self, first, count):
        return QueriesView(self, first, count)

    def codes(self, qidx):
        out = np.zeros(2 * ((len(self.seqs[qidx]) + 1 + 255) // 256 * 8), np.uint32)
# ... 509 lines not shown
```

Measured before the change: 162,200.

## Trim host syncs and launches in routed scan, pool timing events, fuse small layout

Reworks the routed scan call so the host no longer waits after pass A. The coop stage-0 stitch and its count readback are enqueued first, lane stitch/reduce overlap them, and the coop restitch rounds launch only when the readback says they are needed. When there are no lane waves it skips the side-stream fork and join. It also adds a speculative 'ahead' path that skips waiting on pending index builds and reruns if flags are set, replaces memsets with a clear kernel plus a single-block layout kernel for small pair counts, and recycles hipEvents instead of creating and destroying them. These changes cut per-call launch and synchronisation latency, at the cost of more complex control flow and a possible rerun on the speculative path.

```diff
diff --git a/andi_amd/csrc/api.hip b/andi_amd/csrc/api.hip
--- a/andi_amd/csrc/api.hip
+++ b/andi_amd/csrc/api.hip
@@ -372,6 +372,8 @@
 	(void)hipSetDevice(ctx->device);
 	if (ctx->stream) (void)hipStreamSynchronize(ctx->stream);
 	resolve_events(ctx);
+	for (hipEvent_t ev : ctx->idle_events) (void)hipEventDestroy(ev);
+	ctx->idle_events.clear();
 	if (ctx->scratch) (void)andi_arena::dev_free(ctx->scratch);
 	if (ctx->desc_dev) (void)andi_arena::dev_free(ctx->desc_dev);
 	if (ctx->desc_host) host_pool::pinned_put(ctx->desc_host, ctx->desc_bytes);
@@ -770,6 +772,32 @@
 	if (items && l.items && ni) HIP_TRY(ctx, hipMemcpy(items, l.items, ni * sizeof(uint32_t), hipMemcpyDeviceToHost));
 	if (pair_class && l.pair_class && np) HIP_TRY(ctx, hipMemcpy(pair_class, l.pair_class, np, hipMemcpyDeviceToHost));
 	if (pair_cost && l.pair_cost && np) HIP_TRY(ctx, hipMemcpy(pair_cost, l.pair_cost, np, hipMemcpyDeviceToHost));
+	return 0;
+}
+extern "C" int andi_hip_test_call_edges(andi_hip_ctx *ctx, uint32_t *out, uint32_t *count_b) {
+	if (!ctx || !out) return 1;
+	const auto &l = ctx->last_edges;
+	for (int k = 0; k < 3; ++k) out[k] = l.pass_a[k], out[3 + k] = l.rounds[k];
+	out[6] = l.went_ahead, out[7] = l.ran_again;
+	if (!count_b) return 0;
+	for (int k = 0; k < 16; ++k) count_b[k] = 0;
+	if (!l.count_b) return 0;
+	HIP_TRY(ctx, hipSetDevice(ctx->device));
+	HIP_TRY(ctx, hipStreamSynchronize(ctx->stream));
+	HIP_TRY(ctx, hipMemcpy(count_b, l.count_b, 16 * sizeof(uint32_t), hipMemcpyDeviceToHost));
+	return 0;
+}
+extern "C" int andi_hip_test_pair_layout(andi_hip_ctx *ctx, uint32_t *pair_waves, uint32_t *pair_wave0, uint32_t *sub_order, uint32_t *counts, uint32_t *info) {
+	if (!ctx) return 1;
+	const auto &l = ctx->last_items;
+	HIP_TRY(ctx, hipSetDevice(ctx->device));
+	HIP_TRY(ctx, hipStreamSynchronize(ctx->stream));
+	if (info) info[0] = l.pairs, info[1] = l.nsub, info[2] = l.pair_wave0 ? 1u : 0u, info[3] = l.looked;
+	if (pair_waves && l.pair_waves && l.pairs) HIP_TRY(ctx, hipMemcpy(pair_waves, l.pair_waves, l.pairs * sizeof(uint32_t), hipMemcpyDeviceToHost));
+	if (pair_wave0 && l.pair_wave0 && l.pairs) HIP_TRY(ctx, hipMemcpy(pair_wave0, l.pair_wave0, ((size_t)l.pairs + 1) * sizeof(uint32_t), hipMemcpyDeviceToHost));
+	if (sub_order && l.sub_order && l.nsub) HIP_TRY(ctx, hipMemcpy(sub_order, l.sub_order, l.nsub * sizeof(uint32_t), hipMemcpyDeviceToHost));
+	if (counts)
+		for (int k = 0; k < 16; ++k) counts[k] = l.counts[k];
 	return 0;
 }
 extern "C" int andi_hip_test_stitch_slots(andi_hip_ctx *ctx, ChainState *cold_exit, ChainState *true_exit, ChainState *used_entry, uint32_t *cold_counts,
diff --git a/andi_amd/csrc/api_internal.h b/andi_amd/csrc/api_internal.h
--- a/andi_amd/csrc/api_internal.h
+++ b/andi_amd/csrc/api_internal.h
@@ -61,9 +61,12 @@
 		const uint32_t *items = nullptr;
 		const uint8_t *pair_class = nullptr, *pair_cost = nullptr;
 		uint32_t n_items = 0, pairs = 0, total_segs = 0;
+		const uint32_t *pair_waves = nullptr, *pair_wave0 = nullptr, *sub_order = nullptr;
+		uint32_t nsub = 0, looked = 0, counts[16] = {};
 	} last_items;
 	unsigned long long *d_route = nullptr;
 	std::vector<EventPair> pending;
+	std::vector<hipEvent_t> idle_events;
 	andi_hip_timings acc{};
 #ifdef ANDI_TEST_HOOKS
 	struct {
@@ -72,8 +75,14 @@
 		const ColdMark *marks = nullptr;
 		uint32_t nsub = 0, total_segs = 0, seg = 0;
 	} last_slots;
+	struct {
+		uint32_t pass_a[3] = {0, 0, 0}, rounds[3] = {0, 0, 0};
+		uint32_t went_ahead = 0, ran_again = 0;
+		const uint32_t *count_b = nullptr;
+	} last_edges;
 #endif
 };
+#define ANDI_LOOK_B 32
 
 struct andi_hip_esa {
 	uint8_t *S = nullptr;
@@ -196,8 +205,8 @@
 				ctx->acc.stitch_launches++;
 			}
 		}
-		(void)hipEventDestroy(ev.a);
-		(void)hipEventDestroy(ev.b);
+		ctx->idle_events.push_back(ev.a);
+		ctx->idle_events.push_back(ev.b);
 	}
 	ctx->pending.clear();
 }
@@ -206,14 +215,25 @@
 	andi_hip_ctx *ctx;
 	EventPair ev;
 	bool ok;
+	static bool take(andi_hip_ctx *c, hipEvent_t *e) {
+		if (c->idle_events.empty()) return hipEventCreate(e) == hipSuccess;
+		*e = c->idle_events.back();
+		c->idle_events.pop_back();
+		return true;
+	}
+	void give_back() {
+		ctx->idle_events.push_back(ev.a);
+		ctx->idle_events.push_back(ev.b);
+	}
 	Timed(andi_hip_ctx *c, int kind) : ctx(c), ok(false) {
 		ev.kind = kind;
-		if (hipEventCreate(&ev.a) != hipSuccess) return;
-		if (hipEventCreate(&ev.b) != hipSuccess) {
-			(void)hipEventDestroy(ev.a);
+		if (!take(c, &ev.a)) return;
+		if (!take(c, &ev.b)) {
+			c->idle_events.push_back(ev.a);
 			return;
 		}
 		ok = hipEventRecord(ev.a, c->stream) == hipSuccess;
+		if (!ok) give_back();
 	}
 	void stop() {
 		if (!ok) return;
@@ -223,9 +243,7 @@
 		if (ctx->pending.size() > 256) resolve_events(ctx);
 	}
 	~Timed() {
-		if (!ok) return;
-		(void)hipEventDestroy(ev.a);
-		(void)hipEventDestroy(ev.b);
+		if (ok) give_back();
 	}
 	Timed(const Timed &) = delete;
 	Timed &operator=(const Timed &) = delete;
diff --git a/andi_amd/csrc/scan.h b/andi_amd/csrc/scan.h
--- a/andi_amd/csrc/scan.h
+++ b/andi_amd/csrc/scan.h
@@ -101,7 +101,7 @@
 hipError_t andi_launch_pack_symbols(const uint8_t *src, size_t bytes, uint8_t *N0, uint8_t *N1,
 									int32_t *foreign, hipStream_t st);
 hipError_t andi_launch_pack_planes(const uint8_t *N0, size_t symbols, uint32_t *planes, uint32_t *codes, hipStream_t st);
-hipError_t andi_launch_pair_layout(const ScanArgs &a, hipStream_t st);
+hipError_t andi_launch_pair_layout(const ScanArgs &a, hipStream_t st, uint32_t *more = nullptr);
 hipError_t andi_launch_pair_leftover(const ScanArgs &a2, hipStream_t st);
 hipError_t andi_launch_route_count(const ScanArgs &a, hipStream_t st);
 hipError_t andi_launch_coop_items(const ScanArgs &b, hipStream_t st);
@@ -111,7 +111,11 @@
 int andi_coop_wants_pool(const ScanArgs &a);
 int andi_coop_will_pool(const ScanArgs &a);
 size_t andi_pool_scratch_bytes(int device, uint32_t *waves);
-hipError_t andi_launch_lane_stitch(const ScanArgs &a, hipStream_t st);
+#define ANDI_STITCH_CLEAR 1u
+#define ANDI_STITCH_STAGE0 2u
+#define ANDI_STITCH_ROUNDS 4u
+#define ANDI_STITCH_ALL 7u
+hipError_t andi_launch_lane_stitch(const ScanArgs &a, hipStream_t st, unsigned parts = ANDI_STITCH_ALL, uint32_t *rounds = nullptr);
 hipError_t andi_launch_lane_quad_small(const ScanArgs &a, uint32_t count, hipStream_t st);
 #ifndef ANDI_RESTITCH_ROUNDS
 #define ANDI_RESTITCH_ROUNDS 3
@@ -166,7 +170,7 @@
 #define ANDI_STITCH_TOGETHER 40
 #endif
 hipError_t andi_launch_scan_cold(const ScanArgs &a, hipStream_t st);
-hipError_t andi_launch_scan_stitch(const ScanArgs &a, hipStream_t st);
+hipError_t andi_launch_scan_stitch(const ScanArgs &a, hipStream_t st, unsigned parts = ANDI_STITCH_ALL, uint32_t *rounds = nullptr);
 hipError_t andi_launch_scan_reduce(const ScanArgs &a, hipStream_t st);
 hipError_t andi_launch_match_positions(const EsaDev &E, const uint8_t *q, uint32_t qlen,
 									   uint32_t first, uint32_t count, int cached,
diff --git a/andi_amd/csrc/scan.hip b/andi_amd/csrc/scan.hip
--- a/andi_amd/csrc/scan.hip
+++ b/andi_amd/csrc/scan.hip
@@ -498,9 +498,9 @@
 	return a.exact_equal ? launch_reference<true>(a, st, false) : launch_reference<false>(a, st, false);
 }
 
-hipError_t andi_launch_scan_stitch(const ScanArgs &a, hipStream_t st) {
-	hipError_t e = andi_launch_lane_stitch(a, st);
-	if (e != hipSuccess || !a.any_reference) return e;
+hipError_t andi_launch_scan_stitch(const ScanArgs &a, hipStream_t st, unsigned parts, uint32_t *rounds) {
+	hipError_t e = andi_launch_lane_stitch(a, st, parts, rounds);
+	if (e != hipSuccess || !a.any_reference || !(parts & ANDI_STITCH_ROUNDS)) return e;
 	return a.exact_equal ? launch_reference<true>(a, st, true) : launch_reference<false>(a, st, true);
 }
 
diff --git a/andi_amd/csrc/scan_call.hip b/andi_amd/csrc/scan_call.hip
--- a/andi_amd/csrc/scan_call.hip
+++ b/andi_amd/csrc/scan_call.hip
@@ -209,7 +209,7 @@
 }
 
 int upload_descriptors(andi_hip_ctx *ctx, andi_hip_esa *const *subjects, const int64_t *self, size_t nsub, const andi_hip_queries *q,
-					   bool force_reference, int &any_reference, uint64_t &pairs, uint64_t &nt) {
+					   bool force_reference, int &any_reference, uint64_t &pairs, uint64_t &nt, bool *ahead) {
 	const size_t desc_need = nsub * (sizeof(EsaDev) + sizeof(int64_t));
 	if (ctx->desc_bytes < desc_need) {
 		HIP_TRY(ctx, hipStreamSynchronize(ctx->stream));
@@ -227,7 +227,9 @@
 	auto *h_esa = (EsaDev *)ctx->desc_host;
 	auto *h_self = (int64_t *)(h_esa + nsub);
 	pairs = 0, nt = 0, any_reference = 0;
-	if (ctx->builds_pending) {
+	*ahead = *ahead && ctx->builds_pending && !force_reference;
+	for (size_t s = 0; s < nsub && *ahead; ++s) *ahead = subjects[s] && subjects[s]->index_built;
+	if (ctx->builds_pending && !*ahead) {
 		HIP_TRY(ctx, hipEventSynchronize(ctx->built));
 		ctx->builds_pending = false;
 	}
@@ -236,6 +238,14 @@
 		if (!e || (!e->index_built && !e->ref_built)) {
 			ctx->err = "andi_hip_scan_rows: subject index not built";
 			return 1;
+		}
+		if (*ahead) {
+			h_esa[s] = esa_view(e, ANDI_MODE_PROBE);
+			h_self[s] = self ? self[s] : -1;
+			const bool has_self = h_self[s] >= 0 && (size_t)h_self[s] < q->nq;
+			pairs += q->nq - (has_self ? 1 : 0);
+			nt += q->total_nt - (has_self ? q->len[(size_t)h_self[s]] : 0);
+			continue;
 		}
 		int mode = ANDI_MODE_PROBE;
 		if (!e->index_built || e->h_flags[0] != 0 || force_reference) {
@@ -342,7 +352,7 @@
 }
 
 hipError_t launch_routed(andi_hip_ctx *ctx, const ScanPlan &P, ScanArgs &a, size_t b_off, const andi_hip_queries *q,
-						 size_t slots, size_t slots2, const char *&what) {
+						 size_t slots, size_t slots2, andi_hip_esa *const *subjects, bool ahead, bool *again, const char *&what) {
 	const size_t nsub = a.nsub, pairs_all = nsub * q->nq;
 	ScanArgs b = a;
 	b.adaptive = 0, b.coop = 1, b.route = ANDI_LAYOUT_COOP;
@@ -354,10 +364,11 @@
 	b.items_order = listed ? P.items_order : (uint32_t)ANDI_ITEMS_GRID;
 	b.layout_count = a.restitch_count;
 	hipError_t e;
+	const size_t timers_before = ctx->pending.size();
+	uint32_t pass_a[3] = {0, 0, 0}, rounds[3] = {0, 0, 0};
 	{
 		Timed t(ctx, 2);
-		e = hipMemsetAsync(b.restitch_count, 0, 16 * sizeof(uint32_t), ctx->stream);
-		if (e == hipSuccess) e = andi_launch_pair_layout(a, ctx->stream);
+		e = andi_launch_pair_layout(a, ctx->stream, b.restitch_count);
 		if (e == hipSuccess && listed) e = andi_launch_coop_items(b, ctx->stream);
 		t.stop();
 		if (e != hipSuccess) return what = "scan layout", e;
@@ -368,6 +379,18 @@
 	e = hipSuccess;
 	if (look) e = hipMemcpyAsync(ctx->h_any_left + 1, a.restitch_count, 16 * sizeof(uint32_t), hipMemcpyDeviceToHost, ctx->stream);
 	if (look && e == hipSuccess) e = hipStreamSynchronize(ctx->stream);
+	if (ahead && e == hipSuccess) {
+		ctx->builds_pending = false;
+		for (size_t s = 0; s < nsub; ++s)
+			if (subjects[s]->h_flags[0] != 0 || subjects[s]->h_flags[1] != 0) *again = true;
+		if (*again) {
+			while (ctx->pending.size() > timers_before) {
+				ctx->idle_events.push_back(ctx->pending.back().a), ctx->idle_events.push_back(ctx->pending.back().b);
+				ctx->pending.pop_back();
+			}
+			return hipSuccess;
+		}
+	}
 	const bool lanes_first = look && e == hipSuccess && (uint64_t)ctx->h_any_left[1 + ANDI_LANE_WAVES] * 20 < ctx->h_any_left[1 + ANDI_ALL_WAVES];
 	b.pool_use = look && e == hipSuccess && 2 * (uint64_t)ctx->h_any_left[1 + ANDI_POOL_SEGS] >= ctx->h_any_left[1 + ANDI_COOP_SEGS] && ctx->h_any_left[1 + ANDI_COOP_SEGS] != 0;
 	give_pool_scratch(ctx, b);
@@ -375,19 +398,31 @@
 	if (andi_coop_will_pool(b)) b.coop_items = nullptr;
 	ctx->last_items.items = b.coop_items, ctx->last_items.pair_class = b.pair_class, ctx->last_items.pair_cost = b.pair_cost;
 	ctx->last_items.n_items = b.n_items, ctx->last_items.pairs = (uint32_t)pairs_all, ctx->last_items.total_segs = b.total_segs;
-	if (e == hipSuccess) e = hipEventRecord(ctx->coop_fork, ctx->stream);
-	if (e == hipSuccess) e = hipStreamWaitEvent(ctx->coop_stream, ctx->coop_fork, 0);
-	if (e == hipSuccess && lanes_first) e = andi_launch_scan_cold(a, ctx->stream);
-	if (e == hipSuccess) e = andi_launch_coop_cold(b, ctx->coop_stream);
+	ctx->last_items.pair_waves = a.pair_waves, ctx->last_items.pair_wave0 = a.adaptive ? a.pair_wave0 : nullptr, ctx->last_items.sub_order = a.sub_order;
+	ctx->last_items.nsub = a.nsub, ctx->last_items.looked = look ? 1u : 0u;
+	for (int k = 0; k < 16; ++k) ctx->last_items.counts[k] = ctx->h_any_left[1 + k];
+	const bool any_lanes = ctx->h_any_left[1 + ANDI_LANE_WAVES] != 0;
+	const hipStream_t bs = any_lanes ? ctx->coop_stream : ctx->stream;
+	if (e == hipSuccess && any_lanes) e = hipEventRecord(ctx->coop_fork, ctx->stream);
+	if (e == hipSuccess && any_lanes) e = hipStreamWaitEvent(ctx->coop_stream, ctx->coop_fork, 0);
+	if (e == hipSuccess && lanes_first && any_lanes) e = andi_launch_scan_cold(a, ctx->stream), pass_a[0] = 1;
+	if (e == hipSuccess) e = andi_launch_coop_cold(b, bs), pass_a[1] = 1;
 	if (andi_coop_will_pool(b)) ctx->acc.pool_calls++;
-	if (e == hipSuccess) e = hipEventRecord(ctx->coop_join, ctx->coop_stream);
-	if (e == hipSuccess && !lanes_first) e = andi_launch_scan_cold(a, ctx->stream);
-	if (e == hipSuccess) e = hipStreamWaitEvent(ctx->stream, ctx->coop_join, 0);
-	if (e == hipSuccess) e = hipMemcpyAsync(ctx->h_any_left, b.restitch_count + ANDI_ROUTE_ANY_LEFT, sizeof(uint32_t), hipMemcpyDeviceToHost, ctx->stream);
-	if (e == hipSuccess) e = hipStreamSynchronize(ctx->stream);
+	if (e == hipSuccess && any_lanes) e = hipEventRecord(ctx->coop_join, ctx->coop_stream);
+	if (e == hipSuccess && !lanes_first && any_lanes) e = andi_launch_scan_cold(a, ctx->stream), pass_a[0] = 1;
+	if (e == hipSuccess && any_lanes) e = hipStreamWaitEvent(ctx->stream, ctx->coop_join, 0);
 	if (e != hipSuccess) return what = "scan pass A", e;
-	const bool any_left = ctx->h_any_left[0] != 0;
-	const bool any_lanes = ctx->h_any_left[1 + ANDI_LANE_WAVES] != 0;
+	t.stop();
+	Timed t2(ctx, 2);
+	e = andi_launch_scan_stitch(b, bs, ANDI_STITCH_STAGE0);
+	if (e == hipSuccess) e = hipMemcpyAsync(ctx->h_any_left + ANDI_LOOK_B, b.restitch_count, 16 * sizeof(uint32_t), hipMemcpyDeviceToHost, bs);
+	if (e == hipSuccess) e = hipEventRecord(ctx->l2_fork, ctx->stream);
+	if (e == hipSuccess && any_lanes) e = andi_launch_scan_stitch(a, ctx->stream, ANDI_STITCH_ALL, &rounds[0]);
+	if (e == hipSuccess && any_lanes) e = andi_launch_scan_reduce(a, ctx->stream);
+	if (e == hipSuccess) e = hipStreamSynchronize(bs);
+	if (e != hipSuccess) return what = "scan passes B/C", e;
+	const bool any_left = (ctx->h_any_left[0] = ctx->h_any_left[ANDI_LOOK_B + ANDI_ROUTE_ANY_LEFT]) != 0;
+	const bool rounds_b = ctx->h_any_left[ANDI_LOOK_B + ANDI_RESTITCH_ROUNDS] != 0;
 	ScanArgs a2 = a;
 	if (any_left) {
 		const size_t need2 = carve_layout(a2, nullptr, 0, slots, pairs_all, false, 0) + 256;
@@ -402,27 +437,27 @@
 		a2.route = ANDI_LAYOUT_LANES2;
 		a2.side_stream = nullptr;
 	}
-	t.stop();
-	Timed t2(ctx, 2);
-	e = hipEventRecord(ctx->l2_fork, ctx->stream);
-	if (e == hipSuccess) e = hipStreamWaitEvent(ctx->coop_stream, ctx->l2_fork, 0);
-	if (e == hipSuccess) e = andi_launch_scan_stitch(b, ctx->coop_stream);
-	if (e == hipSuccess) e = andi_launch_scan_reduce(b, ctx->coop_stream);
-	if (e == hipSuccess) e = hipEventRecord(ctx->coop_join, ctx->coop_stream);
+	if (rounds_b) e = andi_launch_scan_stitch(b, bs, ANDI_STITCH_ROUNDS, &rounds[1]);
+	if (e == hipSuccess) e = andi_launch_scan_reduce(b, bs);
+	if (e == hipSuccess && any_lanes) e = hipEventRecord(ctx->coop_join, ctx->coop_stream);
 	if (e == hipSuccess && any_left) {
 		e = hipStreamWaitEvent(ctx->side_stream, ctx->l2_fork, 0);
 		if (e == hipSuccess) e = andi_launch_pair_leftover(a2, ctx->side_stream);
-		if (e == hipSuccess) e = andi_launch_scan_cold(a2, ctx->side_stream);
-		if (e == hipSuccess) e = andi_launch_scan_stitch(a2, ctx->side_stream);
+		if (e == hipSuccess) e = andi_launch_scan_cold(a2, ctx->side_stream), pass_a[2] = 1;
+		if (e == hipSuccess) e = andi_launch_scan_stitch(a2, ctx->side_stream, ANDI_STITCH_ALL, &rounds[2]);
 		if (e == hipSuccess) e = andi_launch_scan_reduce(a2, ctx->side_stream);
 		if (e == hipSuccess) e = hipEventRecord(ctx->l2_join, ctx->side_stream);
 	}
-	if (e == hipSuccess && any_lanes) e = andi_launch_scan_stitch(a, ctx->stream);
-	if (e == hipSuccess && any_lanes) e = andi_launch_scan_reduce(a, ctx->stream);
-	if (e == hipSuccess) e = hipStreamWaitEvent(ctx->stream, ctx->coop_join, 0);
+	if (e == hipSuccess && any_lanes) e = hipStreamWaitEvent(ctx->stream, ctx->coop_join, 0);
 	if (e == hipSuccess && any_left) e = hipStreamWaitEvent(ctx->stream, ctx->l2_join, 0);
 	if (e == hipSuccess) e = andi_launch_route_count(a, ctx->stream);
 	t2.stop();
+#ifdef ANDI_TEST_HOOKS
+	for (int k = 0; k < 3; ++k) ctx->last_edges.pass_a[k] = pass_a[k], ctx->last_edges.rounds[k] = rounds[k];
+	ctx->last_edges.count_b = b.restitch_count;
+#else
+	(void)pass_a, (void)rounds;
+#endif
 	if (e != hipSuccess) return what = "scan passes B/C", e;
 	ctx->acc.coop_calls++;
 	ctx->acc.routed_calls++;
@@ -454,31 +489,40 @@
 	ctx->last_items = {};
 #ifdef ANDI_TEST_HOOKS
 	ctx->last_slots = {};
+	ctx->last_edges = {};
 #endif
-	ScanPlan P = plan_call(subjects, nsub, q, model, segment);
-	if (ensure_segmentation(ctx, q, P.segment)) return 1;
-	int any_reference = 0;
-	uint64_t pairs = 0, nt = 0;
-	if (upload_descriptors(ctx, subjects, self, nsub, q, P.force_reference, any_reference, pairs, nt)) return 1;
-	const int64_t *h_self = (const int64_t *)((const EsaDev *)ctx->desc_host + nsub);
-	plan_layout(ctx, P, h_self, nsub, q, any_reference, nt);
-	if (P.routed && ensure_segmentation(ctx, q, P.coop_seg, true)) return 1;
-	const size_t slots = P.adaptive ? (size_t)64 * P.max_waves : nsub * (size_t)q->total_segs;
-	const size_t slots2 = P.routed ? nsub * (size_t)q->c_total_segs : 0;
-	ScanArgs a = scan_args(ctx, P, nsub, q, M_dev, any_reference);
-	size_t b_off = 0;
-	if (carve_scratch(ctx, P, a, slots, slots2, nsub, nsub * q->nq, &b_off)) return 1;
-
-	const char *what = nullptr;
-	const hipError_t e = P.routed ? launch_routed(ctx, P, a, b_off, q, slots, slots2, what) : launch_direct(ctx, a, what);
-	if (e != hipSuccess) {
-		(void)hipStreamSynchronize(ctx->coop_stream);
-		(void)hipStreamSynchronize(ctx->side_stream);
-		(void)hipStreamSynchronize(ctx->stream);
-		return fail(ctx, what, e);
-	}
-	(P.adaptive ? ctx->acc.adaptive_calls : ctx->acc.uniform_calls)++;
-	ctx->acc.scan_pairs += pairs;
-	ctx->acc.scan_query_nt += nt;
-	return 0;
-}
+	for (bool may_go_ahead = true;; may_go_ahead = false) {
+		ScanPlan P = plan_call(subjects, nsub, q, model, segment);
+		if (ensure_segmentation(ctx, q, P.segment)) return 1;
+		int any_reference = 0;
+		uint64_t pairs = 0, nt = 0;
+		bool ahead = may_go_ahead && P.routed && !P.route_all_few;
+		if (upload_descriptors(ctx, subjects, self, nsub, q, P.force_reference, any_reference, pairs, nt, &ahead)) return 1;
+		const int64_t *h_self = (const int64_t *)((const EsaDev *)ctx->desc_host + nsub);
+		plan_layout(ctx, P, h_self, nsub, q, any_reference, nt);
+		if (P.routed && ensure_segmentation(ctx, q, P.coop_seg, true)) return 1;
+		const size_t slots = P.adaptive ? (size_t)64 * P.max_waves : nsub * (size_t)q->total_segs;
+		const size_t slots2 = P.routed ? nsub * (size_t)q->c_total_segs : 0;
+		ScanArgs a = scan_args(ctx, P, nsub, q, M_dev, any_reference);
+		size_t b_off = 0;
+		if (carve_scratch(ctx, P, a, slots, slots2, nsub, nsub * q->nq, &b_off)) return 1;
+
+		const char *what = nullptr;
+		bool again = false;
+		const hipError_t e = P.routed ? launch_routed(ctx, P, a, b_off, q, slots, slots2, subjects, ahead, &again, what) : launch_direct(ctx, a, what);
+		if (e != hipSuccess) {
+			(void)hipStreamSynchronize(ctx->coop_stream);
+			(void)hipStreamSynchronize(ctx->side_stream);
+			(void)hipStreamSynchronize(ctx->stream);
+			return fail(ctx, what, e);
+		}
+#ifdef ANDI_TEST_HOOKS
+		ctx->last_edges.went_ahead |= ahead ? 1u : 0u, ctx->last_edges.ran_again |= again ? 1u : 0u;
+#endif
+		if (again) continue;
+		(P.adaptive ? ctx->acc.adaptive_calls : ctx->acc.uniform_calls)++;
+		ctx->acc.scan_pairs += pairs;
+		ctx->acc.scan_query_nt += nt;
+		return 0;
+	}
+}
diff --git a/andi_amd/csrc/scan_lane.hip b/andi_amd/csrc/scan_lane.hip
--- a/andi_amd/csrc/scan_lane.hip
+++ b/andi_amd/csrc/scan_lane.hip
@@ -33,31 +33,17 @@
 	PairCtx c = make_ctx(a, sub, qidx);
 	const uint32_t nl_shift = !a.route || c.qlen >= 32768u ? 6u : c.qlen >= 16384u ? 5u : 4u, nl = 1u << nl_shift;
 	const uint32_t p = (uint32_t)(((uint64_t)(2 * lane + 1) * c.qlen) >> (nl_shift + 1));
-	LWin w;
-	w.q0 = EMPTY, w.dg = NO_DIAG;
-	const uint32_t cap = a.adaptive ? 16 * a.seg0 / (a.seg_factor ? a.seg_factor : 1) / 2 + 32 : 96u;
-	Probe r;
-	r.len = 0;
-	if (lane < nl) r = lane_probe(c, p, w, cap);
-	uint32_t sum = r.len < cap ? r.len : cap;
-#pragma unroll
-	for (int d = 32; d; d >>= 1) sum += (uint32_t)__shfl_xor((int)sum, d);
-	sum <<= 6u - nl_shift;
-	bool islands = false, guess = false, far_clean = false;
-	const bool quad_cand = (sum >> 6) >= a.quad_min_match && (sum >> 6) < ANDI_ISLAND_MEAN_MAX && a.quad_min_match != 0;
 	uint32_t break_dist = ~0u;
 	if (a.qsep && a.self[sub] >= 0) {
 		const uint32_t ends = a.qsep[qidx] + a.qsep[(uint32_t)a.self[sub]];
 		if (ends) break_dist = c.qlen / ends;
 	}
-	const bool coop_cand = a.route && (sum >> 6) < 512u && c.qlen >= (a.route_seg < ANDI_ROUTE_MIN_QLEN ? a.route_seg : ANDI_ROUTE_MIN_QLEN) && break_dist >= 20480u;
-	if (coop_cand) {
-		const uint32_t T = c.thr + 3;
-		uint32_t nrounds = est_waves > 1 ? 8u : 4u;
-		while (nrounds > 1 && c.qlen < nrounds * (64u * 2048u)) nrounds >>= 1;
-		const uint32_t nsamples = nl * nrounds;
-		uint32_t shorts = 0, runs = 0;
-		for (uint32_t k = wave; k < nrounds; k += est_waves) {
+	const bool pre_cand = a.route && c.qlen >= (a.route_seg < ANDI_ROUTE_MIN_QLEN ? a.route_seg : ANDI_ROUTE_MIN_QLEN) && break_dist >= 20480u;
+	const uint32_t T = c.thr + 3;
+	uint32_t nrounds = est_waves > 1 ? 8u : 4u;
+	while (nrounds > 1 && c.qlen < nrounds * (64u * 2048u)) nrounds >>= 1;
+	auto further_samples = [&](uint32_t first_round, uint32_t step, uint32_t &shorts, uint32_t &runs) {
+		for (uint32_t k = first_round; k < nrounds; k += step) {
 			const uint32_t pk = (uint32_t)(((uint64_t)(2 * nrounds * lane + 2 * k + 1) * c.qlen) / (2u * nl * nrounds));
 			bool all_short = lane < nl;
 			for (uint32_t j = 0; j < 5 && all_short; ++j) {
@@ -71,11 +57,33 @@
 		}
 #pragma unroll
 		for (int d = 32; d; d >>= 1) shorts += (uint32_t)__shfl_xor((int)shorts, d), runs += (uint32_t)__shfl_xor((int)runs, d);
-		if (!many) {
-			if (lane == 0) atomicAdd(&s_shorts, shorts), atomicAdd(&s_runs, runs);
-			__syncthreads();
-			shorts = s_shorts, runs = s_runs;
-		}
+	};
+	if (!many && wave != 0) {
+		uint32_t shorts = 0, runs = 0;
+		if (pre_cand) further_samples(wave - 1, est_waves - 1, shorts, runs);
+		if (pre_cand && lane == 0) atomicAdd(&s_shorts, shorts), atomicAdd(&s_runs, runs);
+		__syncthreads();
+		return;
+	}
+	LWin w;
+	w.q0 = EMPTY, w.dg = NO_DIAG;
+	const uint32_t cap = a.adaptive ? 16 * a.seg0 / (a.seg_factor ? a.seg_factor : 1) / 2 + 32 : 96u;
+	Probe r;
+	r.len = 0;
+	if (lane < nl) r = lane_probe(c, p, w, cap);
+	uint32_t sum = r.len < cap ? r.len : cap;
+#pragma unroll
+	for (int d = 32; d; d >>= 1) sum += (uint32_t)__shfl_xor((int)sum, d);
+	sum <<= 6u - nl_shift;
+	bool islands = false, guess = false, far_clean = false;
+	const bool quad_cand = (sum >> 6) >= a.quad_min_match && (sum >> 6) < ANDI_ISLAND_MEAN_MAX && a.quad_min_match != 0;
+	const bool coop_cand = pre_cand && (sum >> 6) < 512u;
+	if (!many) __syncthreads();
+	if (coop_cand) {
+		const uint32_t nsamples = nl * nrounds;
+		uint32_t shorts = 0, runs = 0;
+		if (many) further_samples(0, 1, shorts, runs);
+		else shorts = s_shorts, runs = s_runs;
 		const float ns = (float)nsamples;
 		float g = (float)(shorts - runs) / ns, f0;
 		if (g > 0.53f) g = 0.53f;
@@ -178,6 +186,13 @@
 	}
 }
 
+__global__ __launch_bounds__(256) void k_layout_clear(ScanArgs a, uint32_t *more) {
+	const uint32_t t = blockIdx.x * 256 + threadIdx.x;
+	if (t < 16) a.restitch_count[t] = 0;
+	if (more && t >= 16 && t < 32) more[t - 16] = 0;
+	if (a.sub_cost && t < a.nsub) a.sub_cost[t] = 0.f;
+}
+
 __global__ __launch_bounds__(1024) void k_pair_totals(ScanArgs a) {
 	__shared__ uint32_t s_sum[4];
 	const uint32_t P = a.nsub * a.nq, pair = blockIdx.x * 1024 + threadIdx.x;
@@ -208,19 +223,22 @@
 	}
 }
 
-__device__ __forceinline__ uint32_t route_pair(const ScanArgs &a, uint32_t pair, uint32_t &pool_segs, uint32_t &coop_segs) {
+struct RouteWaves {
+	uint32_t all, sparse, hard, island, strct;
+};
+__device__ __forceinline__ uint32_t route_pair(const ScanArgs &a, uint32_t pair, const RouteWaves &w, uint32_t &pool_segs, uint32_t &coop_segs) {
 	uint32_t cls = a.pair_class[pair];
-	const bool lanes_few = 10 * a.restitch_count[ANDI_SPARSE_WAVES] <= a.restitch_count[ANDI_ALL_WAVES];
+	const bool lanes_few = 10 * w.sparse <= w.all;
 	if ((cls & ANDI_ROUTE_COOP) && (cls & ANDI_ROUTE_SOFT) && !lanes_few && !a.route_all_few) cls &= ~ANDI_ROUTE_COOP;
-	if ((cls & ANDI_ROUTE_GUESS) && 20 * a.restitch_count[ANDI_ISLAND_WAVES] > a.restitch_count[ANDI_ALL_WAVES]) cls &= ~ANDI_ROUTE_COOP;
-	if ((cls & (ANDI_ROUTE_LEFT | ANDI_ROUTE_GUESS)) && !(cls & ANDI_ROUTE_COOP) && (cls & 3u) < a.max_class && 3 * a.restitch_count[ANDI_STRUCT_WAVES] >= a.restitch_count[ANDI_ALL_WAVES]) {
+	if ((cls & ANDI_ROUTE_GUESS) && 20 * w.island > w.all) cls &= ~ANDI_ROUTE_COOP;
+	if ((cls & (ANDI_ROUTE_LEFT | ANDI_ROUTE_GUESS)) && !(cls & ANDI_ROUTE_COOP) && (cls & 3u) < a.max_class && 3 * w.strct >= w.all) {
 		++cls;
 		const uint32_t seg = a.seg0 << (cls & 3u);
 		a.pair_waves[pair] = ((a.qlen[pair % a.nq] + seg - 1) / seg + 63) / 64;
 	}
 	const bool pool = (cls & ANDI_ROUTE_POOLCAND) != 0;
 	cls &= ~(ANDI_ROUTE_SOFT | ANDI_ROUTE_LEFT | ANDI_ROUTE_GUESS | ANDI_ROUTE_POOLCAND);
-	if (a.route_all_few && 20 * a.restitch_count[ANDI_HARD_WAVES] <= a.restitch_count[ANDI_ALL_WAVES] && a.self[pair / a.nq] != (int64_t)(pair % a.nq))
+	if (a.route_all_few && 20 * w.hard <= w.all && a.self[pair / a.nq] != (int64_t)(pair % a.nq))
 		cls |= ANDI_ROUTE_COOP;
 	if (cls & ANDI_ROUTE_COOP) {
 		const uint32_t segs = (a.qlen[pair % a.nq] + a.route_seg - 1) / a.route_seg;
@@ -234,7 +252,9 @@
 __global__ __launch_bounds__(256) void k_pair_route(ScanArgs a) {
 	const uint32_t P = a.nsub * a.nq, pair = blockIdx.x * 256 + threadIdx.x;
 	uint32_t mine = 0, pool_segs = 0, coop_segs = 0;
-	if (pair < P) mine = route_pair(a, pair, pool_segs, coop_segs);
+	const RouteWaves w = {a.restitch_count[ANDI_ALL_WAVES], a.restitch_count[ANDI_SPARSE_WAVES], a.restitch_count[ANDI_HARD_WAVES],
+						  a.restitch_count[ANDI_ISLAND_WAVES], a.restitch_count[ANDI_STRUCT_WAVES]};
+	if (pair < P) mine = route_pair(a, pair, w, pool_segs, coop_segs);
 #pragma unroll
 	for (int d = 32; d; d >>= 1)
 		mine += (uint32_t)__shfl_xor((int)mine, d), pool_segs += (uint32_t)__shfl_xor((int)pool_segs, d), coop_segs += (uint32_t)__shfl_xor((int)coop_segs, d);
@@ -254,6 +274,76 @@
 			rank += (o > c || (o == c && t < s)) ? 1u : 0u;
 		}
 		a.sub_order[rank] = s;
+	}
+}
+
+__global__ __launch_bounds__(1024) void k_pair_layout_small(ScanArgs a) {
+	__shared__ uint32_t s_part[1024];
+	__shared__ uint32_t s_sum[8];
+	const uint32_t P = a.nsub * a.nq, pair = threadIdx.x;
+	if (threadIdx.x < 8) s_sum[threadIdx.x] = 0;
+	__syncthreads();
+	{
+		uint32_t all = 0, sparse = 0, hard = 0, isl = 0;
+		if (pair < P) {
+			const uint32_t cls = a.pair_class[pair];
+			all = a.pair_waves[pair];
+			hard = (cls & ANDI_ROUTE_COOP) ? 0u : all;
+			sparse = (cls & ANDI_ROUTE_SOFT) ? all : hard;
+			isl = (cls & ANDI_ROUTE_LEFT) ? all : 0u;
+		}
+#pragma unroll
+		for (int d = 32; d; d >>= 1) {
+			all += (uint32_t)__shfl_xor((int)all, d);
+			sparse += (uint32_t)__shfl_xor((int)sparse, d);
+			hard += (uint32_t)__shfl_xor((int)hard, d);
+			isl += (uint32_t)__shfl_xor((int)isl, d);
+		}
+		if ((threadIdx.x & 63u) == 0) atomicAdd(&s_sum[0], all), atomicAdd(&s_sum[1], sparse), atomicAdd(&s_sum[2], hard), atomicAdd(&s_sum[3], isl);
+	}
+	__syncthreads();
+	const RouteWaves w = {s_sum[0], s_sum[1], s_sum[2], s_sum[3], a.restitch_count[ANDI_STRUCT_WAVES]};
+	if (threadIdx.x == 0) {
+		if (w.all) atomicAdd(&a.restitch_count[ANDI_ALL_WAVES], w.all);
+		if (w.sparse) atomicAdd(&a.restitch_count[ANDI_SPARSE_WAVES], w.sparse);
+		if (w.hard) atomicAdd(&a.restitch_count[ANDI_HARD_WAVES], w.hard);
+		if (w.island) atomicAdd(&a.restitch_count[ANDI_ISLAND_WAVES], w.island);
+	}
+	{
+		uint32_t mine = 0, pool_segs = 0, coop_segs = 0;
+		if (pair < P) mine = route_pair(a, pair, w, pool_segs, coop_segs);
+#pragma unroll
+		for (int d = 32; d; d >>= 1)
+			mine += (uint32_t)__shfl_xor((int)mine, d), pool_segs += (uint32_t)__shfl_xor((int)pool_segs, d), coop_segs += (uint32_t)__shfl_xor((int)coop_segs, d);
+		if ((threadIdx.x & 63u) == 0) atomicAdd(&s_sum[4], mine), atomicAdd(&s_sum[5], coop_segs), atomicAdd(&s_sum[6], pool_segs);
+	}
+	if (a.sub_order && threadIdx.x < a.nsub) {
+		const uint32_t s = threadIdx.x;
+		const float c = a.sub_cost[s];
+		uint32_t rank = 0;
+		for (uint32_t t = 0; t < a.nsub; ++t) {
+			const float o = a.sub_cost[t];
+			rank += (o > c || (o == c && t < s)) ? 1u : 0u;
+		}
+		a.sub_order[rank] = s;
+	}
+	__syncthreads();
+	if (threadIdx.x == 0) {
+		if (s_sum[4]) atomicAdd(&a.restitch_count[ANDI_LANE_WAVES], s_sum[4]);
+		if (s_sum[5]) atomicAdd(&a.restitch_count[ANDI_COOP_SEGS], s_sum[5]), atomicAdd(&a.restitch_count[ANDI_POOL_SEGS], s_sum[6]);
+	}
+	if (!a.adaptive) return;
+	const uint32_t v = pair < P ? a.pair_waves[pair] : 0u;
+	const uint32_t incl = block_scan_1024(v, s_part);
+	if (threadIdx.x == 1023) a.pair_bsum[0] = 0, a.pair_wave0[P] = incl;
+	if (pair < P) {
+		const uint32_t w0 = incl - v;
+		a.pair_wave0[pair] = w0;
+		if ((a.pair_class[pair] & 0x80u) && v) {
+			uint32_t *list = (uint32_t *)a.defer_list;
+			const uint32_t base = atomicAdd(&a.restitch_count[ANDI_QUAD_WAVES], v);
+			for (uint32_t k = 0; k < v; ++k) list[base + k] = w0 + k;
+		}
 	}
 }
 
@@ -1145,13 +1235,18 @@
 	return hipSuccess;
 }
 
-hipError_t andi_launch_pair_layout(const ScanArgs &a, hipStream_t st) {
+hipError_t andi_launch_pair_layout(const ScanArgs &a, hipStream_t st, uint32_t *more) {
 	const uint32_t P = a.nsub * a.nq;
-	(void)hipMemsetAsync(a.restitch_count, 0, 16 * sizeof(uint32_t), st);
-	if (a.sub_cost) (void)hipMemsetAsync(a.sub_cost, 0, a.nsub * sizeof(float), st);
+	k_layout_clear<<<((a.sub_cost && a.nsub > 32 ? a.nsub : 32u) + 255) / 256, 256, 0, st>>>(a, more);
+	CHECK_LAUNCH();
 	if (P <= 4096) k_pair_estimate<<<P, P <= 1024 ? 64 * EST_WAVES_FEW : 64 * EST_WAVES, 0, st>>>(a, false);
 	else k_pair_estimate<<<(P + 3) / 4, 256, 0, st>>>(a, true);
 	CHECK_LAUNCH();
+	if (a.route && P <= 1024) {
+		k_pair_layout_small<<<1, 1024, 0, st>>>(a);
+		CHECK_LAUNCH();
+		return hipSuccess;
+	}
 	if (a.route) {
 		k_pair_totals<<<(P + 1023) / 1024, 1024, 0, st>>>(a);
 		CHECK_LAUNCH();
@@ -1217,12 +1312,12 @@
 	return e;
 }
 
-hipError_t andi_launch_lane_stitch(const ScanArgs &a0, hipStream_t st) {
+hipError_t andi_launch_lane_stitch(const ScanArgs &a0, hipStream_t st, unsigned parts, uint32_t *rounds) {
 	hipStream_t st_ = st;
 	(void)st_;
 	dim3 grid = lane_grid(a0);
 	ScanArgs a = a0;
-	hipError_t e = hipMemsetAsync(a.restitch_count, 0, 16 * sizeof(uint32_t), st);
+	hipError_t e = (parts & ANDI_STITCH_CLEAR) ? hipMemsetAsync(a.restitch_count, 0, 16 * sizeof(uint32_t), st) : hipSuccess;
 	if (e != hipSuccess) return e;
 	const size_t slots = a.adaptive ? (size_t)64 * a.max_waves : (size_t)a.nsub * a.total_segs;
 	const uint32_t per_block = WAVES_PER_BLOCK * ANDI_LISTED_LANES;
@@ -1240,12 +1335,12 @@
 		while ((size_t)L * 8192 < slots) L *= 2;
 		if (L < 64) a.stitch_lanes = L, grid0 = dim3((a.total_segs + WAVES_PER_BLOCK * L - 1) / (WAVES_PER_BLOCK * L), a.nsub);
 	}
-	if (a.exact_equal)
+	if ((parts & ANDI_STITCH_STAGE0) && a.exact_equal)
 		stage(k_lane_stitch<true, 0>, k_lane_stitch<true, 1>, grid0, 8);
-	else
+	else if (parts & ANDI_STITCH_STAGE0)
 		stage(k_lane_stitch<false, 0>, k_lane_stitch<false, 1>, grid0, 8);
 #ifdef ANDI_LANE_STATS
-	if (andi_knob(KNOB_LANE_STATS)) {
+	if ((parts & ANDI_STITCH_STAGE0) && andi_knob(KNOB_LANE_STATS)) {
 		static const char *names[8] = {"entered behind the cold chain's first anchor", "met behind its first anchor", "met at a mark",
 									   "met in phase 2", "position-synced", "left on their own", "steps of those that left on their own", "steps of the others"};
 		unsigned long long h[24];
@@ -1257,16 +1352,17 @@
 		(void)hipMemcpyToSymbol(HIP_SYMBOL(g_lane_stats), h, sizeof h);
 	}
 #endif
-	const bool again = !andi_knob(KNOB_NO_RESTITCH);
+	const bool again = (parts & ANDI_STITCH_ROUNDS) && !andi_knob(KNOB_NO_RESTITCH);
 	for (uint32_t r = 0; again && r < ANDI_RESTITCH_ROUNDS; ++r) {
 		a.restitch_round = r;
 		if (a.exact_equal)
 			stage(k_stitch_heads, k_lane_stitch<true, 2>, grid, 13 + r);
 		else
 			stage(k_stitch_heads, k_lane_stitch<false, 2>, grid, 13 + r);
+		if (rounds) ++*rounds;
 	}
 #ifdef ANDI_LANE_STATS
-	if (andi_knob(KNOB_LANE_STATS)) {
+	if ((parts & ANDI_STITCH_ROUNDS) && andi_knob(KNOB_LANE_STATS)) {
 		static const char *kinds[4] = {"first stage", "first stage, listed", "-", "stretches stitched again (segments)"};
 		unsigned long long h[4][16], st[4];
 		unsigned int mx[4];
diff --git a/andi_amd/lib.py b/andi_amd/lib.py
--- a/andi_amd/lib.py
+++ b/andi_amd/lib.py
@@ -187,6 +187,8 @@
     "andi_hip_test_download_text": (C.c_int, [_P, _P, _P, _P, C.c_size_t, _P, C.c_size_t]),
     "andi_hip_test_pack_text": (C.c_int, [_P, _P, C.c_int]),
     "andi_hip_test_coop_items": (C.c_int, [_P, _P, C.c_size_t, _P, _P, C.c_size_t, _P]),
+    "andi_hip_test_call_edges": (C.c_int, [_P, _P, _P]),
+    "andi_hip_test_pair_layout": (C.c_int, [_P, _P, _P, _P, _P, _P]),
     "andi_hip_test_query_codes": (C.c_int, [_P, _P, C.c_size_t, _P, C.c_size_t]),
     "andi_hip_test_stitch_slots": (C.c_int, [_P, _P, _P, _P, _P, _P, _P, C.c_size_t, _P, _P]),
 }
@@ -562,6 +564,22 @@
         items, cls, cost = np.zeros(int(info[0]), np.uint32), np.zeros(int(info[1]), np.uint8), np.zeros(int(info[1]), np.uint8)
         self._check(hook(self._h, items.ctypes.data, len(items), cls.ctypes.data, cost.ctypes.data, len(cls), info.ctypes.data), "test_coop_items")
         return (items if info[3] else None), cls, cost, int(info[2])
+
+    def call_edges(self):
+        out, count_b = np.zeros(8, np.uint32), np.zeros(16, np.uint32)
+        self._check(_hook("andi_hip_test_call_edges")(self._h, out.ctypes.data, count_b.ctypes.data), "test_call_edges")
+        edges = {name: (bool(out[k]), int(out[3 + k])) for k, name in enumerate(("lanes", "coop", "back"))}
+        edges["ahead"], edges["again"] = bool(out[6]), bool(out[7])
+        return edges, count_b
+
+    def pair_layout(self):
+        hook = _hook("andi_hip_test_pair_layout")
+        info = np.zeros(4, np.uint32)
+        self._check(hook(self._h, None, None, None, None, info.ctypes.data), "test_pair_layout")
+        pairs, nsub = int(info[0]), int(info[1])
+        waves, wave0, order, counts = np.zeros(pairs, np.uint32), np.zeros(pairs + 1, np.uint32), np.zeros(nsub, np.uint32), np.zeros(16, np.uint32)
+        self._check(hook(self._h, waves.ctypes.data, wave0.ctypes.data, order.ctypes.data, counts.ctypes.data, info.ctypes.data), "test_pair_layout")
+        return {"pair_waves": waves, "pair_wave0": wave0 if info[2] else None, "sub_order": order, "counts": counts if info[3] else None}
 
     def stitch_slots(self):
         hook = _hook("andi_hip_test_stitch_slots")
```

After: 167,100, median of 6. +3.0%, better.
